# It4innovations/hyperqueue

Hardware: AMD Instinct MI355X
Metric: tasks_assigned_per_sec (higher is better)
Workload: dtype u64

## Files before the change

hyperqueue_amd/csrc/debug_capi.cpp:

```cpp
#include "../../include/hqtick_debug.h"

#include <algorithm>
#include <cstring>

#include "hb_order.h"
#include "milp.h"
#include "price_emul.h"

static thread_local int g_last_canonical = 0;
static thread_local long g_last_hull[2] = {0, 0};
extern "C" int hqtick_debug_milp_was_canonical(void) { return g_last_canonical; }
extern "C" void hqtick_debug_milp_last_hull(long *solves, long *nonpacking) {
    if (solves) *solves = g_last_hull[0];
    if (nonpacking) *nonpacking = g_last_hull[1];
}

extern "C" int hqtick_debug_milp_solve(int ncols, const double *obj, const uint8_t *col_kind, int nrows, const uint8_t *row_type,
                                       const double *rhs, const int *row_off, const int *row_col, const double *row_coef,
                                       double time_limit_s, int canonical, double *x_out, double *obj_out, int *is_optimal,
                                       long *nodes_out) {
    hqmilp::Model m;
    m.obj.assign(obj, obj + ncols);
    m.kind.assign(col_kind, col_kind + ncols);
    m.rtype.assign(row_type, row_type + nrows);
// ... 13 lines not shown
    return 1;
}

extern "C" void hqtick_debug_map_order_u32(const uint32_t *keys, uint32_t n, uint32_t *out_pos) {
    std::vector<uint32_t> order;
    hqhb::insertion_order_u32(keys, n, order);
    for (uint32_t i = 0; i < n; i++) out_pos[i] = order[i];
}

extern "C" int hqtick_debug_milp_solve_priced(int ncols, const double *obj, const uint8_t *col_kind, const int32_t *col_group, int nrows, const uint8_t *row_type,
                                              const uint8_t *row_implied, const double *rhs, const int *row_off, const int *row_col, const double *row_coef,
                                              double time_limit_s, int use_sweeps, uint32_t min_cols, double *x_out, double *obj_out, int *is_optimal, double *stats_out) {
    hqmilp::Model m;
    m.obj.assign(obj, obj + ncols);
    m.kind.assign(col_kind, col_kind + ncols);
    m.rtype.assign(row_type, row_type + nrows);
    m.rhs.assign(rhs, rhs + nrows);
    m.roff.assign(row_off, row_off + nrows + 1);
    int nnz = nrows ? row_off[nrows] : 0;
    m.rcol.assign(row_col, row_col + nnz);
    m.rcoef.assign(row_coef, row_coef + nnz);
    if (col_group) m.col_group.assign(col_group, col_group + ncols);
    if (row_implied) m.row_implied.assign(row_implied, row_implied + nrows);
    hqprice::EmulatedSweeper emu;
    if (min_cols) emu.min_cols = min_cols;
    hqmilp::Result r = hqmilp::solve(m, time_limit_s, true, hqmilp::REFERENCE_MIP_REL_GAP, use_sweeps ? &emu : nullptr);
    g_last_canonical = r.canonical ? 1 : 0;
    g_last_hull[0] = r.hull_solves; g_last_hull[1] = r.hull_solves_nonpacking;
    if (stats_out) { stats_out[0] = r.price_sweeps; stats_out[1] = r.price_rounds; stats_out[2] = r.price_total_us; stats_out[3] = r.canonical ? 1.0 : 0.0; }
    if (!r.feasible) return 0;
    for (int j = 0; j < ncols; j++) x_out[j] = r.x[j];
    *obj_out = r.objective;
    *is_optimal = r.optimal ? 1 : 0;
    return 1;
}

static thread_local hqmilp::Probe g_block_run_probe;
extern "C" void hqtick_debug_set_block_runs(int on) {
    hqmilp::g_probe = on < 0 ? nullptr : &g_block_run_probe; hqmilp::set_block_runs(on);
    if (on >= 0) { g_block_run_probe.model = g_block_run_probe.tables = g_block_run_probe.runs = g_block_run_probe.covered = 0; }
}
extern "C" void hqtick_debug_corrupt_block_runs(int on) { g_block_run_probe.corrupt_runs = on != 0; }
extern "C" void hqtick_debug_last_coupled_digest(uint64_t out[4]) {
    out[0] = g_block_run_probe.model; out[1] = g_block_run_probe.tables; out[2] = g_block_run_probe.runs; out[3] = g_block_run_probe.covered;
}
extern "C" void hqtick_debug_set_early_sweep(int on) { hqprice::set_early_sweep(on); }
extern "C" uint32_t hqtick_debug_early_sweeps(void) { return hqprice::early_sweeps(); }
extern "C" void hqtick_debug_capture_first_cut(int on) { hqprice::capture_first_cut(on != 0); }
extern "C" uint32_t hqtick_debug_first_cut(unsigned char *out, uint32_t cap) {
    const std::vector<unsigned char> &b = hqprice::first_cut_bytes();
    if (out && cap) memcpy(out, b.data(), std::min<size_t>(cap, b.size()));
    return (uint32_t)b.size();
}
```

hyperqueue_amd/csrc/host_model.cpp:

```cpp
#include "host_model.h"

#include <algorithm>
#include <chrono>
#include <cmath>
#include <cstring>
#include <string>
#include <unordered_map>

#include "hb_order.h"

namespace hqhost {

namespace {

struct OrderEntry { uint64_t hash = 0; bool used = false; std::vector<uint32_t> ids, order; };
thread_local OrderEntry order_cache[32];
thread_local unsigned order_next = 0;
const std::vector<uint32_t> &cached_worker_order(const std::vector<uint32_t> &ids) {
    typedef OrderEntry Entry;
    Entry (&cache)[32] = order_cache;
    unsigned &next = order_next;
    uint64_t h = 0x9E3779B97F4A7C15ull ^ ids.size();
    for (uint32_t v : ids) { h ^= v; h *= 0xFF51AFD7ED558CCDull; h ^= h >> 29; }
    for (Entry &e : cache) if (e.used && e.hash == h && e.ids.size() == ids.size() && (ids.empty() || memcmp(e.ids.data(), ids.data(), ids.size() * 4) == 0)) return e.order;
// ... 1181 lines not shown
                        if (runs_on) for (auto &wg : pm.with_gap) pm.max_excess = std::max(pm.max_excess, (int64_t)bcols_ub[wg.first] - (int64_t)wg.second);
                    }
                    no_gap = pm.whole ? &bcols : &pm.no_gap; no_gap_id = pm.lhs_id;
                    auto gap_rows = [&](const uint32_t w, const uint32_t gap) {
                        const int *wc = bcols.data() + bcols_off[w]; const size_t nwc = bcols_end[w] - bcols_off[w];
                        const uint64_t cols_ub = bcols_ub[w];
                        if (bounded && fl_cached == -2) fl_cached = short_flag(brq, bl.second);
                        const int fl = bounded ? fl_cached : -1;
                        if (cols_ub <= (uint64_t)cut.size + gap) return;
                        if (bounded && fl >= 0) { cols.assign(wc, wc + nwc); emit_plus(hqmilp::ROW_MAX, (double)cut.size + bsize + (double)gap, cols, fl, bsize); }
                        else if (!bounded) { m.begin_row(hqmilp::ROW_MAX, (double)cut.size + (double)gap); for (size_t k = 0; k < nwc; k++) m.term(wc[k], 1.0); m.end_row(); }
                    };
                    if (runs_on && (pm.all_gap || !pm.with_gap.empty()) && pm.max_excess <= (int64_t)cut.size) {
                        if (bounded) fl_cached = short_flag(brq, bl.second);
                        n_decided_once++;
                    } else if (pm.all_gap) for (uint32_t w : solver_workers) gap_rows(w, pm.gap_all);
                    else for (auto &wg : pm.with_gap) gap_rows(wg.first, wg.second);
                }
                if (no_gap->empty()) continue;
                int fl;
                if (bounded && (fl = short_flag(brq, bl.second)) >= 0) list_row(hqmilp::ROW_MAX, bsize + (double)cut.size, no_gap_id, *no_gap, fl, bsize);
                else if (!bounded && std::find(capped_by.begin(), capped_by.end(), brq) == capped_by.end()) {
                    capped_by.push_back(brq);
                    list_row(hqmilp::ROW_MAX, (double)cut.size, no_gap_id, *no_gap, -1, 0.0);
                }
            }
        }
    }

    if (!seq_start.empty()) {
        m.start.assign(m.ncols(), 0.0);
        for (const SeqStart &ss : seq_start) {
            const int pc = place_get(ss.w, batches[ss.batch].rq, ss.variant);
            if (pc < 0) { m.start.clear(); break; }
            m.start[pc] = ss.count;
        }
    }
    m.row_implied.resize(m.nrows(), 0);
    m.row_lhs.resize((size_t)m.nrows(), -1); m.row_lhs_len.resize((size_t)m.nrows(), 0); m.row_block.resize((size_t)m.nrows(), -1);
    m.col_ub = col_ub; m.col_ub.resize((size_t)m.ncols(), UINT32_MAX);
    if (hqmilp::g_probe) {
        using hqmilp::fnv1a_vec;
        uint64_t h = hqmilp::FNV_BASIS;
        h = fnv1a_vec(h, m.obj); h = fnv1a_vec(h, m.kind); h = fnv1a_vec(h, m.rtype); h = fnv1a_vec(h, m.rhs); h = fnv1a_vec(h, m.roff); h = fnv1a_vec(h, m.rcol); h = fnv1a_vec(h, m.rcoef);
        h = fnv1a_vec(h, m.start); h = fnv1a_vec(h, m.col_group); h = fnv1a_vec(h, m.row_implied); h = fnv1a_vec(h, m.row_lhs); h = fnv1a_vec(h, m.row_lhs_len);
        h = fnv1a_vec(h, m.list_off); h = fnv1a_vec(h, m.list_col); h = fnv1a_vec(h, m.row_block); h = fnv1a_vec(h, m.col_ub);
        hqmilp::g_probe->model = h; hqmilp::g_probe->runs = m.block_runs.size(); hqmilp::g_probe->tables = 0; hqmilp::g_probe->covered = 0;
    }
    const double t_model1 = clock_us();
    if (trace_model) {
        size_t run_blocks = 0; for (const auto &br : m.block_runs) run_blocks += (size_t)br.n_blocks;
        fprintf(stderr, "[model] cuts done at %.3f ms: %d columns, %d rows, %zu terms, %zu worker signatures, %zu (batch, cut, blocker) passes over the workers; %zu equal-block runs over %zu blocks, %zu (cut, blocker) passes decided once\n", (t_model1 - t_model0) / 1e3, m.ncols(), m.nrows(), m.rcol.size(), sig_rep.size(), n_triples, m.block_runs.size(), run_blocks, n_decided_once);
    }
    hqmilp::Result sol = hqmilp::solve(m, pb.time_limit_s, !pb.certificate_only, hqmilp::REFERENCE_MIP_REL_GAP, pb.pricer);
    if (trace_model) fprintf(stderr, "[model] solve done %.3f ms after the model\n", (clock_us() - t_model1) / 1e3);
    out.pre_us = t_model0 - t_enter; out.model_us = t_model1 - t_model0; out.milp_us = clock_us() - t_model1; out.price_sweeps = sol.price_sweeps; out.price_rounds = sol.price_rounds; out.price_us = sol.price_total_us;
    out.milp_nodes = sol.nodes; out.milp_cols = m.ncols(); out.milp_rows = m.nrows(); out.milp_components = sol.n_components;
    if (!sol.feasible) return out;
    out.is_optimal = sol.optimal;
    out.is_canonical = sol.canonical && sol.optimal;

    std::vector<uint64_t> key_hash; std::vector<std::pair<uint32_t, uint8_t>> key_list; std::vector<std::vector<std::pair<uint32_t, uint32_t>>> key_counts;
    std::vector<uint64_t> mn_hash; std::vector<uint32_t> mn_list; std::vector<std::vector<std::vector<uint32_t>>> mn_sets;
    std::vector<uint32_t> dec_ids, dec_widx, dec_cnt;
    for (const TaskBatch &batch : batches) {
        const RequestView &rv = pb.rqs[batch.rq];
        if (pb.rq_multi_node(batch.rq)) {
            size_t n_nodes = pb.variants[rv.first_variant].n_nodes;
            std::vector<std::vector<uint32_t>> sets;
            for (uint32_t w : solver_workers) {
                const int pc = place_get(w, batch.rq, 0);
                if (pc < 0 || (uint32_t)std::round(sol.x[pc]) == 0) continue;
                if (!sets.empty() && sets.back().size() < n_nodes) sets.back().push_back(w); else sets.push_back({w});
            }
            if (!sets.empty()) { mn_hash.push_back(hqhb::hash_rq_variant(batch.rq, 0)); mn_list.push_back(batch.rq); mn_sets.push_back(sets); }
        } else {
            for (uint8_t v = 0; v < rv.n_variants; v++) {
                const size_t nsw = solver_workers.size();
                dec_ids.resize(nsw + 1); dec_widx.resize(nsw + 1); dec_cnt.resize(nsw + 1);
                uint32_t *idp = dec_ids.data(), *wxp = dec_widx.data(), *cp = dec_cnt.data(); size_t nk = 0;
                const int *pcol = place_col.data() + rv.first_variant + v;
                const double *xs = sol.x.data();
                for (size_t i = 0; i < nsw; i++) {
                    const uint32_t w = solver_workers[i];
                    const int pc = pcol[(size_t)w * NVS];
                    const double xv = pc >= 0 ? xs[pc] : 0.0;
                    const uint32_t c = xv > 0.0 ? (uint32_t)(xv + 0.5) : 0u;
                    idp[nk] = ws.id[w]; wxp[nk] = w; cp[nk] = c; nk += c > 0 ? 1 : 0;
                }
                if (nk == 0) continue;
                dec_ids.resize(nk);
                const std::vector<uint32_t> &ids = dec_ids, &widx = dec_widx, &cnt = dec_cnt;
                const std::vector<uint32_t> &word = cached_worker_order(ids);
                std::vector<std::pair<uint32_t, uint32_t>> ordered; ordered.reserve(word.size());
                for (uint32_t k : word) ordered.push_back({widx[k], cnt[k]});
                key_hash.push_back(hqhb::hash_rq_variant(batch.rq, v)); key_list.push_back({batch.rq, v}); key_counts.push_back(std::move(ordered));
            }
        }
    }
    std::vector<uint32_t> ord;
    hqhb::insertion_order(key_hash.data(), (uint32_t)key_hash.size(), ord);
    for (uint32_t k : ord) { out.keys.push_back(key_list[k]); out.per_key.push_back(std::move(key_counts[k])); }
    hqhb::insertion_order(mn_hash.data(), (uint32_t)mn_hash.size(), ord);
    for (uint32_t k : ord) { out.mn_rq.push_back(mn_list[k]); out.mn_sets.push_back(std::move(mn_sets[k])); }
    if (trace_model) fprintf(stderr, "[model] decoded %.3f ms after the model, %.3f ms after the solver was entered\n", (clock_us() - t_model1) / 1e3, (clock_us() - t_enter) / 1e3);
    return out;
}

}
```

hyperqueue_amd/csrc/host_model.h:

```cpp
#pragma once
#include <cstdint>
#include <map>
#include <string>
#include <tuple>
#include <vector>

#include "../../include/hqtick.h"
#include "block_core.h"
#include "price.h"
#include "milp.h"

namespace hqhost {

struct VariantView {
    const uint32_t *res;
    const uint8_t *kind;
    const uint64_t *amount;
    uint32_t n_entries, n_nodes, weight;
    uint64_t min_time_ns;
    bool multi_node() const { return n_nodes > 0; }
};

struct RequestView {
    uint32_t first_variant, n_variants;
// ... 26 lines not shown
    const float *min_util = nullptr;
    const uint8_t *flags = nullptr;
    const uint32_t *group = nullptr;
    const uint8_t *vflags = nullptr;
    const uint32_t *vtmc = nullptr;
    uint32_t n_variant_slots = 0;
    std::vector<std::vector<std::pair<uint32_t, uint8_t>>> blocked;
    uint32_t n_blocked_lists = 0;
    const uint32_t *assigned_off = nullptr, *assigned_rq = nullptr; const uint8_t *assigned_variant = nullptr;
    const uint32_t *agg_off = nullptr, *agg_rq = nullptr, *agg_cnt = nullptr; const uint8_t *agg_variant = nullptr;
    uint32_t n_assigned(uint32_t w) const { return assigned_off ? assigned_off[w + 1] - assigned_off[w] : agg_off ? agg_off[w + 1] - agg_off[w] : 0; }
    bool is_sn(uint32_t w) const { return flags ? (flags[w] & HQ_WORKER_SN) != 0 : true; }
    bool stopping(uint32_t w) const { return flags ? (flags[w] & HQ_WORKER_STOPPING) != 0 : false; }
    bool is_free(uint32_t w) const { return is_sn(w) && n_assigned(w) == 0 && !stopping(w); }
    uint8_t vf(uint32_t w, uint32_t slot) const { return vflags[(size_t)w * n_variant_slots + slot]; }
    uint32_t tmc(uint32_t w, uint32_t slot) const { return vtmc[(size_t)w * n_variant_slots + slot]; }
};

struct BlockSolver {
    virtual ~BlockSolver() {}
    virtual bool solve(const hqblock::ColTable &cols, const hqblock::ClassTable &classes, const hqblock::Output &out) = 0;
    virtual bool begin(const hqblock::ColTable &cols, const hqblock::ClassTable &classes, const hqblock::Output &out) { begun_ok = solve(cols, classes, out); return begun_ok; }
    virtual bool finish() { return begun_ok; }
    virtual bool overlaps() const { return false; }
    bool begun_ok = false;
};

void flush_tick_caches();

struct BlockMemo {
    struct Entry { uint64_t hash = 0; std::vector<unsigned char> key; std::vector<double> x; long nodes = 0; int n_components = 0; };
    static constexpr size_t CAP = 64;
    std::vector<Entry> entries;
    size_t next = 0;
    std::vector<unsigned char> scratch;
    uint64_t scratch_hash = 0;
    const Entry *find(const hqmilp::Model &m);
    void put(const hqmilp::Result &r);
};

struct Problem {
    BlockMemo *memo = nullptr;
    BlockSolver *blocks = nullptr;
    hqprice::Sweeper *pricer = nullptr;
    uint32_t block_min_classes = 1;
    uint32_t block_verify = 2;
    uint32_t tick_seq = 0;
    uint32_t R = 0, n_groups = 0;
    std::vector<RequestView> rqs;
    std::vector<VariantView> variants;
    WorkerSet real;
    const WorkerSet *custom = nullptr;
    double time_limit_s = 5.0;
    bool certificate_only = false;
    bool rq_multi_node(uint32_t rq) const { return variants[rqs[rq].first_variant].multi_node(); }
    bool capable_rqv(const WorkerSet &ws, uint32_t w, uint32_t rq) const {
        for (uint32_t v = 0; v < rqs[rq].n_variants; v++) {
            uint32_t slot = rqs[rq].first_variant + v;
            uint8_t f = ws.vf(w, slot);
            if ((f & 4) && (variants[slot].multi_node() || (f & 2))) return true;
        }
        return false;
    }
};

void group_equal_rows(WorkerSet &ws, bool all_solver);

std::vector<TaskBatch> create_task_batches(const Problem &pb, const std::vector<QueueLevels> &queues);

struct Counts {
    std::vector<std::pair<uint32_t, uint8_t>> keys;
    std::vector<std::vector<std::pair<uint32_t, uint32_t>>> per_key;
    std::vector<uint32_t> mn_rq;
    std::vector<std::vector<std::vector<uint32_t>>> mn_sets;
    struct WorkerList { std::vector<uint32_t> widx; };
    bool by_class = false;
    bool one_class = false;
    uint32_t n_cols = 0;
    std::vector<uint32_t> wclass, class_x, key_col, key_list;
    std::vector<WorkerList> lists;
    bool pairs_built = true;
    void pairs() {
        if (pairs_built) return;
        per_key.assign(keys.size(), {});
        for (size_t k = 0; k < keys.size(); k++) {
            const std::vector<uint32_t> &wi = lists[key_list[k]].widx;
            auto &out = per_key[k]; out.resize(wi.size());
            for (size_t i = 0; i < wi.size(); i++) out[i] = {wi[i], class_x[(size_t)wclass[wi[i]] * n_cols + key_col[k]]};
        }
        pairs_built = true;
    }
    size_t key_size(size_t k) const { return pairs_built ? per_key[k].size() : lists[key_list[k]].widx.size(); }
    bool is_optimal = true;
    bool is_canonical = true;
    bool empty() const {
        if (!pairs_built) { for (size_t k = 0; k < keys.size(); k++) if (key_size(k)) return false; }
        for (auto &k : per_key) if (!k.empty()) return false;
        for (auto &k : mn_sets) if (!k.empty()) return false;
        return true;
    }
    uint32_t checksum() const {
        uint32_t h = 2166136261u;
        auto mix = [&](uint32_t v) { for (int i = 0; i < 4; i++) { h ^= (v >> (8 * i)) & 0xFFu; h *= 16777619u; } };
        mix(is_optimal ? 1u : 0u);
        for (size_t k = 0; k < keys.size(); k++) {
            mix(keys[k].first); mix(keys[k].second);
            if (pairs_built) for (auto &wc : per_key[k]) { mix(wc.first); mix(wc.second); }
            else for (uint32_t w : lists[key_list[k]].widx) { mix(w); mix(class_x[(size_t)wclass[w] * n_cols + key_col[k]]); }
        }
        for (size_t k = 0; k < mn_rq.size(); k++) { mix(mn_rq[k]); for (auto &set : mn_sets[k]) { mix(0xFFFFFFFFu); for (uint32_t w : set) mix(w); } }
        return h;
    }
    int error = 0; std::string errmsg;
    long milp_nodes = 0; int milp_cols = 0, milp_rows = 0, milp_components = 0;
    int price_sweeps = 0, price_rounds = 0; double price_us = 0, milp_us = 0, model_us = 0, pre_us = 0;
    uint32_t blocks_device = 0, blocks_host = 0, block_steps_max = 0, n_classes = 0;
    uint32_t blocks_verified = 0, blocks_mismatch = 0, blocks_rejected = 0;
    uint32_t blocks_memo = 0;
    double t_classify_us = 0, t_blocks_us = 0, t_decode_us = 0;
};

Counts run_scheduling_solver(const Problem &pb, const std::vector<TaskBatch> &batches);

}
```

hyperqueue_amd/csrc/hqtick.cpp:

```cpp
#include "../../include/hqtick.h"
#ifdef HQTICK_TEST_HOOKS
#include "../../include/hqtick_debug.h"
#endif

#include <dlfcn.h>
#include <hip/hip_runtime.h>
#include <rccl/rccl.h>

#include <algorithm>
#include <chrono>
#include <cstdio>
#include <cstdlib>
#include <cstring>
#include <functional>
#include <map>
#include <string>
#include <vector>

#include "block_solve.h"
#include "price_dev.h"
#ifdef HQTICK_TEST_HOOKS
#include "price_emul.h"
#endif
#include "devbuf.h"
// ... 43 lines not shown
    uint64_t max_id = 0; bool max_id_valid = false;
    uint32_t n_appends = 0;
    bool consumed_unconfirmed = false;
    hqhost::BlockMemo block_memo;
    uint64_t add_staged_n = 0;
    DevBuf d_set, d_flags, d_levels, d_nlevels, d_wave_tab, d_hist, d_gkey;
    DevBuf d_ord_hist, d_ord_tab, d_perm, d_perm2, d_ord_tiles, d_inv; PinBuf h_ord, h_ordh;
    bool force_ordered = false;
    bool ordered_sticky = false;
    bool last_ordered = false;
    hqk::OrderSelect last_os{};
    uint32_t dbg_order_runs = 0, dbg_order_levels = 0; bool dbg_order = false; double dbg_order_us = 0;
    uint32_t dbg_scan_L = 0, dbg_scan_G = 0, dbg_scan_shape[4] = {0, 0, 0, 0}; bool dbg_scan = false, dbg_census = false;
    uint32_t lv_seq = 0; bool set_clean = false; bool no_spec_scan = getenv("HQTICK_NO_SPEC_SCAN") != nullptr; bool levels_valid = false; uint32_t cached_L = 0; std::vector<uint64_t> h_levels; bool timing = true, timing_k1 = false;
    PinBuf h_up, h_up2, h_q, h_a, h_plan, h_rec, h_sinkhdr, h_add, h_addp, h_retr, h_blk, h_k5a, h_lv;
    PinBuf h_blkprof; uint32_t n_blkprof = 0; bool block_profile = false;
    hqprice::DeviceSweeper *pricer = nullptr;
    uint32_t block_budget = 4096, block_min_classes = 12;
    DevBuf d_up, d_vflags, d_vtmc, d_blk;
    DevBuf d_cluster; PinBuf h_cl, h_cld; bool cluster_valid = false, cluster_check = false, cl_pending = false; uint32_t cl_W = 0, cl_R = 0;
    std::vector<unsigned char> cl_rt;
    hipEvent_t cl_ev = nullptr;
    struct ClusterMirror {
        bool valid = false; uint32_t n_groups = 1;
        std::vector<uint32_t> id, group; std::vector<uint64_t> total, free_; std::vector<int64_t> rem; std::vector<float> min_util; std::vector<uint8_t> flags;
        std::map<uint32_t, std::vector<std::pair<uint32_t, uint8_t>>> blocked;
        std::vector<uint32_t> blk_worker, blk_rq; std::vector<uint8_t> blk_variant; bool blk_dirty = true;
    } mirror;
    DevBuf d_cluster2;
    struct RetrEntry { uint32_t old_id; bool in_queue; bool has_redirect; uint32_t target_id; uint8_t variant; };
    std::map<uint64_t, RetrEntry> retr;
    std::vector<uint64_t> retr_task, resp_task; std::vector<uint32_t> retr_worker, retr_red_worker, resp_worker; std::vector<uint8_t> retr_red_variant, resp_variant;
    bool sweep_inflight = false;
    bool wait_on_kernel = true;
    DevBuf d_sel_task, d_sel_level, d_map, d_rec, d_tsweep, d_bits, d_pre;
    hqhost::Problem pb;
    PlanScratch plan;
    std::vector<uint32_t> b_rq, b_size, b_limit, b_cut_off, c_size, c_bl_off, bl_rq, bl_size; std::vector<uint8_t> b_lr, b_blk;
    std::vector<uint32_t> cnt_rq, cnt_worker, cnt_value; std::vector<uint8_t> cnt_variant;
    std::vector<uint32_t> rec_off, retract_off, red_worker, mn_off, mn_worker, mn_rq; std::vector<uint64_t> rec_task, retract_task, red_task, mn_task, new_free;
    std::vector<uint8_t> rec_variant, rec_kind, red_variant, red_kind, q_loaded;
    hqtick_kernel_stats stats{};
    uint32_t tpw_hint = 0;
    uint32_t shard_index = 0, shard_count = 1;
    void *sink = nullptr; size_t sink_bytes = 0;
    hqk::WaveGeom last_geom{}; uint32_t last_L = 0, last_Q = 0, last_G = 0; size_t last_tb = 0, last_plan_bytes = 0, last_hist_off = 0; bool last_valid = false;
    hqgraph::Graph graph;
    hqasg::Ledger asg;
    hqtick_ctx *qctx = nullptr;
    ncclComm_t comm = nullptr; uint32_t comm_rank = 0, comm_world = 0;
    hqtick_exchange_fn xfn = nullptr; void *xuser = nullptr;
    DevBuf d_xsend, d_xrecv; PinBuf h_xsend, h_xrecv;
    uint32_t shard_min_blocks = 1025, shard_min_classes = 1025; bool shard_solve = true;
    uint32_t block_verify = 2, tick_seq = 0;
    uint64_t x_calls = 0, x_bytes = 0; double x_us = 0;
    double tl[32] = {}; int ntl = 0;
};

namespace {

#define HQ_HIP(call)                                                                                          \
    do {                                                                                                      \
        hipError_t e_ = (call);                                                                               \
        if (e_ != hipSuccess) { ctx->err = std::string(#call) + ": " + hipGetErrorString(e_); return HQTICK_E_DEVICE; } \
    } while (0)

#define HQ_HIP_TIMED(call)                                                                                    \
    do {                                                                                                      \
        hipError_t e_ = (call);                                                                               \
        hqk::take_launch_timer();                                                                             \
        if (e_ != hipSuccess) { ctx->err = std::string(#call) + ": " + hipGetErrorString(e_); return HQTICK_E_DEVICE; } \
    } while (0)

#define HQ_HIP_LAST(call, launched)                                                                           \
    do {                                                                                                      \
        hipError_t e_ = (call);                                                                               \
        (launched) = hqk::take_launch_timer().stop == nullptr && ctx->wait_on_kernel;                        \
        if (e_ != hipSuccess) { ctx->err = std::string(#call) + ": " + hipGetErrorString(e_); return HQTICK_E_DEVICE; } \
    } while (0)

int fail(hqtick_ctx *ctx, int code, const std::string &msg) { ctx->err = msg; return code; }

double elapsed_us(hipEvent_t a, hipEvent_t b) {
    float ms = 0;
    if (hipEventElapsedTime(&ms, a, b) == hipSuccess) return (double)ms * 1000.0;
    (void)hipGetLastError();
    return -1.0;
}

int validate(hqtick_ctx *ctx, const hqtick_snapshot *s, bool need_tasks) {
    if (!s) return fail(ctx, HQTICK_E_INVALID, "null snapshot");
    if (s->n_workers && (!s->worker_id || !s->worker_total || !s->worker_free)) return fail(ctx, HQTICK_E_INVALID, "worker arrays missing");
    for (uint32_t w = 1; w < s->n_workers; w++) if (s->worker_id[w - 1] >= s->worker_id[w]) return fail(ctx, HQTICK_E_INVALID, "worker ids not ascending");
    if (s->n_requests && (!s->rq_variant_off || !s->variant_entry_off)) return fail(ctx, HQTICK_E_INVALID, "request arrays missing");
    for (uint32_t q = 0; q < s->n_requests; q++) {
        if (s->rq_variant_off[q + 1] <= s->rq_variant_off[q]) return fail(ctx, HQTICK_E_INVALID, "request without variants");
        if (s->rq_variant_off[q + 1] - s->rq_variant_off[q] > 32) return fail(ctx, HQTICK_E_INVALID, "more than 32 variants");
    }
    uint32_t nv = s->n_requests ? s->rq_variant_off[s->n_requests] : 0;
    for (uint32_t e = 0; e < (nv ? s->variant_entry_off[nv] : 0); e++) {
        if (s->entry_resource[e] >= s->n_resources) return fail(ctx, HQTICK_E_INVALID, "entry resource id out of range");
        if (s->entry_kind[e] == HQ_ENTRY_AMOUNT && s->entry_amount[e] == 0) return fail(ctx, HQTICK_E_INVALID, "zero amount request");
    }
    if (need_tasks && s->n_ready) {
        if (!s->task_id || !s->task_priority || !s->task_rq) return fail(ctx, HQTICK_E_INVALID, "ready-set columns missing");
        for (uint64_t i = 1; i < s->n_ready; i++) if (s->task_id[i - 1] >= s->task_id[i]) return fail(ctx, HQTICK_E_INVALID, "ready set not sorted by task id");
// ... 493 lines not shown
    bool allgather(const void *send, void *recv, size_t bytes) override {
        if (ctx->xfn) return ctx->xfn(ctx->xuser, send, recv, bytes) == 0;
        return rccl_allgather_host(ctx, send, recv, bytes);
    }
    ~CtxExchange() override { ctx->x_calls += n_calls; ctx->x_bytes += n_bytes; ctx->x_us += us; }
};

struct ShardedBlocks : hqhost::BlockSolver {
    hqhost::BlockSolver &inner; hqprice::Exchange &ex; uint32_t min_classes;
    hqblock::Output p_out{}; uint32_t p_nd = 0, p_nc = 0, p_nm = 0; bool p_pass = false, p_inner_ok = false, p_pending = false;
    std::vector<uint64_t> cfree, ctot, celig; std::vector<uint32_t> dx, dst, dsteps; std::vector<unsigned char> send, recv;
    ShardedBlocks(hqhost::BlockSolver &in, hqprice::Exchange &e, uint32_t mc) : inner(in), ex(e), min_classes(mc) {}
    bool overlaps() const override { return inner.overlaps(); }
    bool solve(const hqblock::ColTable &ct, const hqblock::ClassTable &cl, const hqblock::Output &out) override { return begin(ct, cl, out) && finish(); }
    bool begin(const hqblock::ColTable &ct, const hqblock::ClassTable &cl, const hqblock::Output &out) override {
        p_pass = ex.world <= 1 || cl.n_classes < min_classes;
        if (p_pass) return inner.begin(ct, cl, out);
        const uint32_t nd = cl.n_classes, R = ct.R, NC = ct.n_cols, W = ex.world, me = ex.rank;
        const uint32_t nm = nd > me ? (nd - me + W - 1) / W : 0;
        cfree.resize((size_t)nm * R); ctot.resize((size_t)nm * R); celig.resize(nm);
        for (uint32_t j = 0; j < nm; j++) {
            const size_t i = (size_t)me + (size_t)j * W;
            memcpy(cfree.data() + (size_t)j * R, cl.free_ + i * R, (size_t)R * 8); memcpy(ctot.data() + (size_t)j * R, cl.total + i * R, (size_t)R * 8); celig[j] = cl.elig[i];
        }
        dx.assign((size_t)nm * NC, 0); dst.assign(nm, hqblock::ST_UNSUPPORTED); dsteps.assign(nm, 0);
        p_out = out; p_nd = nd; p_nc = NC; p_nm = nm; p_pending = true;
        p_inner_ok = nm == 0 || inner.begin(ct, hqblock::ClassTable{nm, cfree.data(), ctot.data(), celig.data()}, hqblock::Output{dx.data(), dst.data(), dsteps.data(), nullptr});
        return true;
    }
    bool finish() override {
        if (p_pass) return inner.finish();
        if (!p_pending) return false;
        p_pending = false;
        if (p_nm && !(p_inner_ok && inner.finish())) { std::fill(dst.begin(), dst.end(), (uint32_t)hqblock::ST_UNSUPPORTED); std::fill(dx.begin(), dx.end(), 0u); }
        const uint32_t W = ex.world, NC = p_nc, mx = (p_nd + W - 1) / W;
        const size_t o_st = (size_t)mx * NC * 4, o_steps = o_st + (size_t)mx * 4, bytes = (o_steps + (size_t)mx * 4 + 7) & ~(size_t)7;
        send.assign(bytes, 0); recv.resize(bytes * W);
        if (p_nm) { memcpy(send.data(), dx.data(), (size_t)p_nm * NC * 4); memcpy(send.data() + o_st, dst.data(), (size_t)p_nm * 4); memcpy(send.data() + o_steps, dsteps.data(), (size_t)p_nm * 4); }
        const double t0 = now_us();
        if (!ex.allgather(send.data(), recv.data(), bytes)) return false;
        ex.us += now_us() - t0; ex.n_calls++; ex.n_bytes += bytes * W;
        for (uint32_t r = 0; r < W; r++) {
            const unsigned char *b = recv.data() + (size_t)r * bytes;
            const uint32_t nr = p_nd > r ? (p_nd - r + W - 1) / W : 0;
            for (uint32_t j = 0; j < nr; j++) {
                const size_t i = (size_t)r + (size_t)j * W;
                memcpy(p_out.x + i * NC, b + (size_t)j * NC * 4, (size_t)NC * 4); memcpy(p_out.status + i, b + o_st + (size_t)j * 4, 4); memcpy(p_out.steps + i, b + o_steps + (size_t)j * 4, 4);
            }
        }
        return true;
    }
};

struct TickRun {
    hqtick_ctx *ctx; const hqtick_snapshot *s; hqtick_result *out; const bool use_resident;
    PlanScratch &ps; hqhost::Problem &pb;
    const uint32_t W, R, Q;
    static constexpr uint32_t NONE = 0xFFFFFFFFu;
    WorkerEval ev; Scan sc; hqhost::Counts cnt;
    uint64_t N = 0; uint32_t L = 0; int status = HQTICK_DONE;
    uint32_t nkeys = 0, max_count = 0, max_nk = 0, n_bit_words = 0, n_sel = 0, n_pfq = 0, n_rec = 0, max_items = 0;
    std::vector<uint32_t> pfq_rq;
    std::vector<std::pair<uint32_t, uint32_t>> retr_pos;
    std::vector<std::vector<uint32_t>> key_T;
    size_t o_rv = 0, o_rk = 0, o_mn = 0, o_fl = 0;
    bool sweep_launched = false;
    uint32_t n_tr = 0;
    const bool transpose_on = !(getenv("HQTICK_TRANSPOSE") && atoi(getenv("HQTICK_TRANSPOSE")) == 0);
    bool may_reorder = false;
    bool compact = false, delta16 = false; size_t o_rs = 0, o_rf = 0; uint32_t max_out = 0;
    uint64_t *h_rec_task = nullptr, *mn_ids = nullptr; uint8_t *h_rec_var = nullptr, *h_rec_kind = nullptr;
    bool assembled = false;
    double t0 = 0;

    TickRun(hqtick_ctx *c, const hqtick_snapshot *snap, hqtick_result *o, bool resident)
        : ctx(c), s(snap), out(o), use_resident(resident), ps(c->plan), pb(c->pb), W(snap->n_workers), R(snap->n_resources), Q(snap->n_requests) {}

    void mark() { if (ctx->ntl < 32) ctx->tl[ctx->ntl++] = now_us() - t0; }
    uint32_t n_groups() const { return sc.ordered ? (uint32_t)sc.run_cnt.size() : sc.G; }

    uint32_t worker_of(uint32_t k, uint32_t idx) {
        cnt.pairs();
        const auto &pk = cnt.per_key[k];
        std::vector<uint32_t> &T = key_T[k];
        if (T.empty()) {
            uint32_t maxc = 0; for (auto &wc : pk) maxc = std::max(maxc, wc.second);
            std::vector<uint32_t> ge(maxc + 2, 0);
            for (auto &wc : pk) ge[wc.second]++;
            uint32_t more = (uint32_t)pk.size(), acc = 0;
            for (uint32_t sw = 0; sw <= maxc; sw++) { T.push_back(acc); more -= ge[sw]; acc += more; }
        }
        uint32_t sw = (uint32_t)(std::upper_bound(T.begin(), T.end(), idx) - T.begin()) - 1, nth = idx - T[sw];
        for (auto &wc : pk) if (wc.second > sw) { if (nth == 0) return wc.first; nth--; }
        return HQ_NO_WORKER;
    }

    int load_ready_set() {
        if (!use_resident) {
            uint64_t N = s->n_ready;
            if (!ctx->d_tid.ensure(N * 8 + 8) || !ctx->d_tprio.ensure(N * 8 + 8) || !ctx->d_trq.ensure(N * 4 + 8)) return fail(ctx, HQTICK_E_DEVICE, "hipMalloc ready set");
            if (N) {
                HQ_HIP(hipMemcpyAsync(ctx->d_tid.p, s->task_id, N * 8, hipMemcpyHostToDevice, ctx->stream));
                HQ_HIP(hipMemcpyAsync(ctx->d_tprio.p, s->task_priority, N * 8, hipMemcpyHostToDevice, ctx->stream));
                HQ_HIP(hipMemcpyAsync(ctx->d_trq.p, s->task_rq, N * 4, hipMemcpyHostToDevice, ctx->stream));
            }
            ctx->n_ready = N; ctx->resident = false; ctx->levels_valid = false;
        } else if (!ctx->resident) return fail(ctx, HQTICK_E_INVALID, "hqtick_run_resident without hqtick_upload_ready");
        N = ctx->n_ready;
        return 0;
    }

    int plan_keys() {
        L = sc.L;
        ps.q_total.assign(Q, 0); ps.pf_n.assign(Q, 0); ps.pf_start.assign(Q, 0); ps.seq_taken.assign(Q, 0);
        for (uint32_t q = 0; q < Q; q++) {
            const uint32_t r0 = sc.run_off[q], r1 = sc.run_off[q + 1];
            for (uint32_t r = r0; r < r1; r++) ps.q_total[q] += sc.run_cnt[r];
            ps.pf_n[q] = s->prefill_off ? s->prefill_off[q + 1] - s->prefill_off[q] : 0;
            if (ps.pf_n[q]) ps.pf_start[q] = (r0 < r1 && sc.run_prio[r0] == s->prefill_priority[q]) ? sc.run_cnt[r0] : 0;
        }
        nkeys = (uint32_t)cnt.keys.size();
        ps.key_seg.assign(nkeys, 0); ps.key_sum.assign(nkeys, 0); ps.key_rq.assign(nkeys, 0); ps.key_var_w.assign((nkeys + 3) / 4 + 1, 0);
        ps.key_ord_off.assign(nkeys + 1, 0); ps.key_t_off.assign(nkeys + 1, 0); ps.key_bits_off.assign(nkeys + 1, 0);
        const bool by_class = cnt.by_class && cnt.wclass.size() == W && cnt.key_col.size() == nkeys;
        ctx->last_valid = false;
// ... 257 lines not shown
        ctx->rec_off = ps.out_off;
        ctx->retract_off.assign(W + 1, 0); ctx->retract_task.assign(ps.retract_pairs.size(), 0);
        {
            for (auto &rp : ps.retract_pairs) if (rp.first < W) ctx->retract_off[rp.first + 1]++;
            for (uint32_t w = 0; w < W; w++) ctx->retract_off[w + 1] += ctx->retract_off[w];
            std::vector<uint32_t> cur(ctx->retract_off.begin(), ctx->retract_off.end() - 1);
            for (auto &rp : ps.retract_pairs) if (rp.first < W) ctx->retract_task[cur[rp.first]++] = rp.second;
        }
        ctx->new_free.assign(s->worker_free, s->worker_free + (size_t)W * R);
        for (uint32_t k = 0; k < nkeys; k++) {
            const hqhost::VariantView &vv = pb.variants[pb.rqs[cnt.keys[k].first].first_variant + cnt.keys[k].second];
            const uint32_t *wcn = ps.wcnt + (size_t)k * W;
            for (uint32_t w = 0; w < W; w++) {
                const uint32_t c = wcn[w];
                if (!c) continue;
                for (uint32_t e = 0; e < vv.n_entries; e++) {
                    uint64_t &f = ctx->new_free[(size_t)w * R + vv.res[e]];
                    if (vv.kind[e] == HQ_ENTRY_ALL) f = 0; else { uint64_t d = vv.amount[e] * (uint64_t)c; f = f > d ? f - d : 0; }
                }
            }
        }
        for (auto &fr : ps.freed) {
            const hqhost::VariantView &vv = pb.variants[fr.second];
            for (uint32_t e = 0; e < vv.n_entries; e++) {
                uint64_t &f = ctx->new_free[(size_t)fr.first * R + vv.res[e]];
                f = vv.kind[e] == HQ_ENTRY_ALL ? s->worker_total[(size_t)fr.first * R + vv.res[e]] : f + vv.amount[e];
            }
        }
    }

    int launch_sweep_early() {
        sweep_launched = false;
        if (nkeys == 0 || n_bit_words == 0 || max_nk > hqk::SWEEP_MAX_WORKERS) return 0;
        if (n_tr == nkeys) { sweep_launched = true; return 0; }
        if (ctx->sweep_inflight) { HQ_HIP(hipStreamSynchronize(ctx->stream)); ctx->sweep_inflight = false; }
        const size_t n_ord = ps.ord_cnt.size(), words = 4 * (size_t)(nkeys + 1) + n_ord;
        if (!ctx->h_k5a.ensure(words * 4 + 64) || !ctx->d_tsweep.ensure((size_t)ps.key_t_off[nkeys] * 4 + 16) || !ctx->d_bits.ensure((size_t)n_bit_words * 8 + 16) ||
            !ctx->d_pre.ensure((size_t)n_bit_words * 4 + 16))
            return fail(ctx, HQTICK_E_DEVICE, "hipMalloc mapping");
        uint32_t *h = ctx->h_k5a.as<uint32_t>();
        const uint32_t *d = ctx->h_k5a.dev<uint32_t>();
        const size_t o_toff = 0, o_ordoff = nkeys + 1, o_boff = 2 * (size_t)(nkeys + 1), o_tr = 3 * (size_t)(nkeys + 1), o_ord = 4 * (size_t)(nkeys + 1);
        memcpy(h + o_toff, ps.key_t_off.data(), (size_t)(nkeys + 1) * 4); memcpy(h + o_ordoff, ps.key_ord_off.data(), (size_t)(nkeys + 1) * 4);
        memcpy(h + o_boff, ps.key_bits_off.data(), (size_t)(nkeys + 1) * 4); memcpy(h + o_tr, ps.key_tr.data(), (size_t)nkeys * 4); if (n_ord) memcpy(h + o_ord, ps.ord_cnt.data(), n_ord * 4);
        hqk::MapKeys mk{};
        mk.n_keys = nkeys; mk.key_t_off = d + o_toff; mk.key_ord_off = d + o_ordoff; mk.key_bits_off = d + o_boff; mk.ord_cnt = d + o_ord; mk.key_tr = d + o_tr;
        mk.t_sweep = ctx->d_tsweep.as<uint32_t>(); mk.bits = ctx->d_bits.as<uint64_t>(); mk.pre = ctx->d_pre.as<uint32_t>();
        if (ctx->timing) hqk::time_next_launch(ctx->ev[1], ctx->ev[6]);
        HQ_HIP_TIMED(hqk::sweep_bits(mk, max_count, max_nk, ctx->stream));
        sweep_launched = true; ctx->sweep_inflight = true;
        return 0;
    }

    int phase_c() {
        size_t n_mn_ids = 0; for (auto &sets : cnt.mn_sets) n_mn_ids += sets.size();
        delta16 = compact && (ctx->cfg.flags & HQTICK_FLAG_COMPACT_DELTA16) != 0;
        if (compact) {
            o_rs = delta16 ? (size_t)n_rec * 8 : (((size_t)n_rec * 4 + 7) & ~(size_t)7); o_rf = o_rs + (size_t)W * 8;
            o_rv = o_rk = 0; o_mn = (o_rf + (size_t)n_rec * (delta16 ? 16 : 12) + 7) & ~(size_t)7;
        } else { o_rv = (size_t)n_rec * 8; o_rk = o_rv + n_rec; o_mn = (o_rk + n_rec + 7) & ~(size_t)7; }
        o_fl = o_mn + n_mn_ids * 8;
        const size_t rec_bytes = o_fl + 64;
        if (!ctx->h_rec.ensure(rec_bytes)) return fail(ctx, HQTICK_E_DEVICE, "hipHostMalloc records");
        h_rec_task = ctx->h_rec.as<uint64_t>(); h_rec_var = ctx->h_rec.as<uint8_t>() + o_rv; h_rec_kind = ctx->h_rec.as<uint8_t>() + o_rk;
        mn_ids = reinterpret_cast<uint64_t *>(ctx->h_rec.as<uint8_t>() + o_mn);
        if (n_sel) {
            if (!ctx->d_sel_task.ensure((size_t)n_sel * 8) || !ctx->d_sel_level.ensure((size_t)n_sel * (sc.ordered ? 4 : 2) + 4))
                return fail(ctx, HQTICK_E_DEVICE, "hipMalloc selection");
            uint32_t *hp = ctx->h_plan.as<uint32_t>();
            size_t cur = ps.plan_head_words;
            auto put = [&](const std::vector<uint32_t> &v) { const size_t o = cur; if (!v.empty()) memcpy(hp + cur, v.data(), v.size() * 4); cur += v.size(); if (v.empty()) hp[cur++] = 0; return o; };
            const size_t o_wpos = 0, o_wcnt = (size_t)nkeys * W, o_pflj = (size_t)2 * nkeys * W;
            size_t o_rq = put(ps.key_rq), o_var = put(ps.key_var_w), o_seg = put(ps.key_seg), o_ordoff = put(ps.key_ord_off), o_ord = put(ps.ord_cnt), o_toff = put(ps.key_t_off),
                   o_boff = put(ps.key_bits_off), o_tr = put(ps.key_tr), o_base = put(ps.rq_sel_base), o_pfs = put(ps.pf_start), o_pfn = put(ps.pf_n),
                   o_pqs = put(ps.pfq_src), o_pqz = put(ps.pfq_size), o_out = put(ps.out_off);
            const size_t o_pqr = ctx->asg.on ? put(pfq_rq) : 0;
            size_t o_tb = put(ps.take_base);
            size_t o_roff = 0, o_qtnc = 0, o_rst = 0, o_rrk = 0;
            if (sc.ordered) { o_roff = put(sc.run_off); o_qtnc = put(ps.q_tnc); o_rst = put(sc.run_start); o_rrk = put(sc.run_level); }
            if (cur & 1) hp[cur++] = 0;
            const size_t o_holes = cur;
            for (uint64_t hk : ps.holes) { hp[cur++] = (uint32_t)(hk & 0xFFFFFFFFu); hp[cur++] = (uint32_t)(hk >> 32); }
            if (ps.holes.empty()) { hp[cur++] = 0; hp[cur++] = 0; }
            const size_t plan_words = cur;
            if (plan_words * 4 + 16 > ctx->h_plan.cap) return fail(ctx, HQTICK_E_DEVICE, "mapping plan larger than its buffer");
            if (!ctx->d_map.ensure(plan_words * 4 + 16) ||
                !ctx->d_tsweep.ensure((size_t)ps.key_t_off[nkeys] * 4 + 16) || !ctx->d_bits.ensure((size_t)n_bit_words * 8 + 16) || !ctx->d_pre.ensure((size_t)n_bit_words * 4 + 16))
                return fail(ctx, HQTICK_E_DEVICE, "hipMalloc mapping");
            mark();
            const uint32_t *d = ctx->d_map.as<uint32_t>();
            hqk::MapKeys mk{};
            mk.n_keys = nkeys; mk.key_rq = d + o_rq; mk.key_variant = reinterpret_cast<const uint8_t *>(d + o_var); mk.key_seg_start = d + o_seg;
            mk.key_ord_off = d + o_ordoff; mk.ord_cnt = d + o_ord; mk.key_t_off = d + o_toff; mk.key_bits_off = d + o_boff; mk.key_tr = d + o_tr;
            mk.t_sweep = ctx->d_tsweep.as<uint32_t>(); mk.bits = ctx->d_bits.as<uint64_t>(); mk.pre = ctx->d_pre.as<uint32_t>();
            mk.wpos = d + o_wpos; mk.wcnt = d + o_wcnt; mk.rq_sel_base = d + o_base; mk.rq_pf_start = d + o_pfs; mk.rq_pf_n = d + o_pfn;
            mk.n_holes = (uint32_t)ps.holes.size(); mk.holes = reinterpret_cast<const uint64_t *>(d + o_holes);
            mk.n_pfq = n_pfq; mk.pfq_src = d + o_pqs; mk.pfq_size = d + o_pqz; mk.pfl_j = d + o_pflj; mk.out_off = d + o_out;
            uint32_t *flags = reinterpret_cast<uint32_t *>(ctx->h_rec.as<uint8_t>() + o_fl);
            flags[0] = 0;
            ctx->last_n_sel = n_sel; ctx->last_consumed = false;
            const bool consume_in_tick = use_resident && (ctx->cfg.flags & HQTICK_FLAG_CONSUME_IN_TICK) != 0;
            if (consume_in_tick && ctx->asg.on && s->n_retracting) {
                uint32_t *saved = ctx->asg.saved_rq(N);
                if (!saved) return fail(ctx, HQTICK_E_DEVICE, "hipMalloc ledger request ids");
                HQ_HIP(hipMemcpyAsync(saved, ctx->d_trq.p, N * 4, hipMemcpyDeviceToDevice, ctx->stream));
            }
            ctx->last_geom = sc.geom; ctx->last_L = L; ctx->last_Q = Q; ctx->last_G = sc.G; ctx->last_tb = o_tb; ctx->last_plan_bytes = plan_words * 4; ctx->last_valid = true;
// ... 15 lines not shown
                                consume_in_tick ? ctx->d_trq.as<uint32_t>() : nullptr, ctx->stream, consume_in_tick ? 1u : 0u));
            }
            if (consume_in_tick) { ctx->n_live -= n_sel; ctx->last_consumed = true; ctx->consumed_unconfirmed = true; }
            if (!sweep_launched && n_tr < nkeys) {
                if (ctx->timing) hqk::time_next_launch(ctx->ev[1], ctx->ev[6]);
                HQ_HIP_TIMED(hqk::sweep_bits(mk, max_count, max_nk, ctx->stream));
            }
            uint8_t *drec = ctx->h_rec.dev<uint8_t>();
            uint64_t *k_task = reinterpret_cast<uint64_t *>(drec); uint8_t *k_var = drec + o_rv, *k_kind = drec + o_rk;
            if (ctx->sink) {
                const uint32_t cap = hqtick_sink_capacity_records(W, ctx->sink_bytes);
                if (n_rec > cap || hqtick_sink_bytes(W, cap) > ctx->sink_bytes) return fail(ctx, HQTICK_E_CAPACITY, "record sink too small for this tick");
                uint8_t *sk = reinterpret_cast<uint8_t *>(ctx->sink);
                const size_t so_off = 16, so_task = (so_off + (size_t)(W + 1) * 4 + 7) & ~(size_t)7, so_var = so_task + (size_t)cap * 8, so_kind = so_var + cap;
                std::vector<uint32_t> &hdr = ps.sink_hdr; hdr.assign(4 + W + 1, 0);
                hdr[0] = n_rec; hdr[1] = cnt.checksum(); hdr[2] = HQTICK_SINK_MAGIC; hdr[3] = cap;
                memcpy(hdr.data() + 4, ps.out_off.data(), (size_t)(W + 1) * 4);
                if (!ctx->h_sinkhdr.ensure(hdr.size() * 4)) return fail(ctx, HQTICK_E_DEVICE, "hipHostMalloc sink header");
                memcpy(ctx->h_sinkhdr.p, hdr.data(), hdr.size() * 4);
                HQ_HIP(hipMemcpyAsync(sk, ctx->h_sinkhdr.p, hdr.size() * 4, hipMemcpyHostToDevice, ctx->stream));
                k_task = reinterpret_cast<uint64_t *>(sk + so_task); k_var = sk + so_var; k_kind = sk + so_kind;
            }
            hqk::time_next_launch(ctx->timing ? ctx->ev[7] : nullptr, ctx->ev[11]);
            hqk::CompactOut co{};
            if (compact) co = hqk::CompactOut{reinterpret_cast<uint32_t *>(drec), reinterpret_cast<uint2 *>(drec + o_rs), reinterpret_cast<uint32_t *>(drec + o_rf),
                                              delta16 ? reinterpret_cast<uint16_t *>(drec) : nullptr};
            hqk::Stage stg{};
            if (ctx->asg.on && n_rec) {
                hqasg::StageCols c{};
                if (!ctx->asg.stage_for(n_rec, sc.ordered, sc.L, &c)) return fail(ctx, HQTICK_E_DEVICE, "hipMalloc ledger staging");
                stg = hqk::Stage{c.task, c.rq, c.row, c.level, c.meta};
                stg.pfq_rq = ctx->d_map.as<uint32_t>() + o_pqr;
            }
            bool expand_is_last = false;
            if (sc.ordered) HQ_HIP_LAST(hqk::expand_mapping_wide(mk, W, ctx->d_sel_task.as<uint64_t>(), ctx->d_sel_level.as<uint32_t>(), max_items, k_task, k_var, k_kind,
                                                           reinterpret_cast<uint32_t *>(drec + o_fl), co, max_out, may_reorder, ctx->stream, stg), expand_is_last);
            else HQ_HIP_LAST(hqk::expand_mapping(mk, W, ctx->d_sel_task.as<uint64_t>(), ctx->d_sel_level.as<uint16_t>(), Q, max_items, k_task, k_var, k_kind,
                                reinterpret_cast<uint32_t *>(drec + o_fl), co, max_out, may_reorder, ctx->stream, stg), expand_is_last);
            if (!cnt.mn_rq.empty()) expand_is_last = false;
            if (sc.ordered) {
                HQ_HIP(hipMemcpyAsync(ctx->h_ordh.as<uint32_t>() + hqk::ORDER_DIGITS * 256 + 2, ctx->d_ord_hist.as<uint32_t>() + hqk::ORDER_DIGITS * 256 + 2, 4, hipMemcpyDeviceToHost, ctx->stream));
                expand_is_last = false;
            }
            {
                size_t pos = 0;
                for (size_t i = 0; i < cnt.mn_rq.size(); i++) {
                    size_t n = cnt.mn_sets[i].size();
                    HQ_HIP(hipMemcpyAsync(mn_ids + pos, ctx->d_sel_task.as<uint64_t>() + ps.rq_sel_base[cnt.mn_rq[i]] + ps.mn_first[i], n * 8, hipMemcpyDeviceToHost, ctx->stream));
                    pos += n;
                }
            }
            mark();
            assemble_host_part();
            if (expand_is_last) HQ_HIP(hipEventSynchronize(ctx->ev[11])); else HQ_HIP(hipStreamSynchronize(ctx->stream));
            ctx->sweep_inflight = false;
            if (flags[0]) return fail(ctx, HQTICK_E_CAPACITY, "mapping kernel capacity exceeded");
            if (sc.ordered && ctx->h_ordh.as<uint32_t>()[hqk::ORDER_DIGITS * 256 + 2]) return fail(ctx, HQTICK_E_DEVICE, "ordered view: the selection left its request's segment");
            if (ctx->timing) { const double us_ = elapsed_us(ctx->ev[4], ctx->ev[5]); if (us_ >= 0) ctx->stats.select_us = us_; }
            if (ctx->timing) { const double us_ = elapsed_us(ctx->ev[1], ctx->ev[6]); if (us_ >= 0) ctx->stats.sweep_us = us_; }
            if (ctx->timing) { const double us_ = elapsed_us(ctx->ev[7], ctx->ev[11]); if (us_ >= 0) ctx->stats.other_us = us_; }
        }
        if (!n_sel) { ctx->last_n_sel = 0; ctx->last_consumed = true; }
        if (!n_sel && ctx->sink) {
            if (hqtick_sink_bytes(W, 0) > ctx->sink_bytes) return fail(ctx, HQTICK_E_CAPACITY, "record sink too small for this tick");
            std::vector<uint32_t> &hdr = ps.sink_hdr; hdr.assign(4 + W + 1, 0);
            hdr[1] = cnt.checksum(); hdr[2] = HQTICK_SINK_MAGIC; hdr[3] = hqtick_sink_capacity_records(W, ctx->sink_bytes);
            HQ_HIP(hipMemcpy(ctx->sink, hdr.data(), hdr.size() * 4, hipMemcpyHostToDevice));
        }
        return 0;
    }

    void finish(double t1, double t2, double t3) {
        if (!assembled) assemble_host_part();
        ctx->mn_task.clear(); ctx->mn_off.assign(1, 0); ctx->mn_worker.clear(); ctx->mn_rq.clear();
        {
            size_t pos = 0;
            for (size_t i = 0; i < cnt.mn_rq.size(); i++) for (auto &set : cnt.mn_sets[i]) {
                ctx->mn_task.push_back(mn_ids[pos++]); ctx->mn_rq.push_back(cnt.mn_rq[i]);
                for (uint32_t w : set) ctx->mn_worker.push_back(w);
                ctx->mn_off.push_back((uint32_t)ctx->mn_worker.size());
            }
        }
        out->status = status;
        out->n_counts = (uint32_t)ctx->cnt_rq.size(); out->count_rq = ctx->cnt_rq.data(); out->count_variant = ctx->cnt_variant.data();
        out->count_worker = ctx->cnt_worker.data(); out->count_value = ctx->cnt_value.data();
        out->rec_off = ctx->rec_off.data();
        if (compact && n_sel) {
            const uint8_t *hb = ctx->h_rec.as<uint8_t>();
            out->run_span = reinterpret_cast<const hqtick_run_span *>(hb + o_rs);
            if (delta16) { out->rec_delta16 = reinterpret_cast<const uint16_t *>(hb); out->runs16 = reinterpret_cast<const hqtick_rec_run16 *>(hb + o_rf); }
            else { out->rec_task_lo = reinterpret_cast<const uint32_t *>(hb); out->runs = reinterpret_cast<const hqtick_rec_run *>(hb + o_rf); }
        } else if (!ctx->sink) { out->rec_task = h_rec_task; out->rec_variant = h_rec_var; out->rec_kind = h_rec_kind; }
        out->retract_off = ctx->retract_off.data(); out->retract_task = ctx->retract_task.data();
        out->n_redirects = (uint32_t)ctx->red_task.size(); out->redirect_task = ctx->red_task.data(); out->redirect_worker = ctx->red_worker.data(); out->redirect_variant = ctx->red_variant.data(); out->redirect_kind = ctx->red_kind.data();
        out->n_mn = (uint32_t)ctx->mn_task.size(); out->mn_task = ctx->mn_task.data(); out->mn_worker_off = ctx->mn_off.data(); out->mn_worker = ctx->mn_worker.data();
        out->new_free = ctx->new_free.data();
        mark();
        double t5 = now_us();
        out->t_total_us = t5 - t0; out->t_scan_us = t1 - t0; out->t_batches_us = t2 - t1; out->t_solve_us = t3 - t2; out->t_mapping_us = t5 - t3;
        uint64_t n_pref = 0; for (uint32_t q = 0; q < Q; q++) n_pref += ps.new_pf_total[q];
        uint64_t n_asg = 0; for (uint32_t w = 0; w < W; w++) n_asg += ps.n_assign[w];
        uint32_t nv = Q ? s->rq_variant_off[Q] : 0;
        ctx->stats.n_assigned = n_asg; ctx->stats.n_prefilled = n_pref;
        ctx->stats.algorithmic_bytes = N * 20 + (uint64_t)W * R * 16 + (uint64_t)nv * R * 9 + n_asg * 13 + n_pref * 12;
        ctx->stats.tick_gpu_us = ctx->stats.distinct_us + ctx->stats.level_hist_us + ctx->stats.scan_us + ctx->stats.block_solve_us + ctx->stats.select_us + ctx->stats.sweep_us + ctx->stats.other_us;
    }

    int run() {
        t0 = now_us();
        ctx->ntl = 0;
        if (ctx->cfg.flags & HQTICK_FLAG_NO_TICK_CACHES) { ctx->levels_valid = false; hqhost::flush_tick_caches(); }
        memset(out, 0, sizeof(*out));
        ctx->stats = hqtick_kernel_stats{};
        int rc = validate(ctx, s, !use_resident);
        if (rc) return rc;
        HQ_HIP(hipSetDevice(ctx->device));
        if ((rc = load_ready_set())) return rc;
        const std::function<void()> prep = [&]() {
            fill_problem(pb, s, ctx->cfg, ev);
            if (ctx->asg.on && !s->assigned_off) {
                const hqasg::Agg g = ctx->asg.agg();
                pb.real.agg_off = g.off; pb.real.agg_rq = g.rq; pb.real.agg_cnt = g.cnt; pb.real.agg_variant = g.var;
            }
            if (pb.certificate_only && (ctx->shard_count > 1 || ctx->sink || ctx->xfn || ctx->comm)) pb.certificate_only = false;
        };
        if ((rc = phase_a(ctx, s, &ev, &sc, &prep))) return rc;
        mark();
        const double t1 = now_us();
        std::vector<hqhost::QueueLevels> qlv = queue_levels(sc, s);
        std::vector<hqhost::TaskBatch> batches = hqhost::create_task_batches(pb, qlv);
        export_batches(ctx, batches, out);
        mark();
        const double t2 = now_us();
        DeviceBlocks dev_blocks(ctx);
        pb.blocks = &dev_blocks; pb.block_min_classes = ctx->block_min_classes; pb.pricer = ctx->pricer;
        pb.block_verify = ctx->block_verify; pb.tick_seq = ctx->tick_seq++;
        pb.memo = (ctx->cfg.flags & (HQTICK_FLAG_NO_BLOCK_MEMO | HQTICK_FLAG_NO_TICK_CACHES)) ? nullptr : &ctx->block_memo;
        double shard_sweep_us = -1.0;
        ctx->x_calls = 0; ctx->x_bytes = 0; ctx->x_us = 0;
        if (CtxExchange::available(ctx)) {
            CtxExchange xch(ctx);
            ShardedBlocks sh_blocks(dev_blocks, xch, ctx->shard_min_classes);
            pb.blocks = &sh_blocks;
            if (ctx->pricer) {
                hqprice::ShardedSweeper sh_sweeps(*ctx->pricer, xch, ctx->shard_min_blocks);
                pb.pricer = &sh_sweeps;
                cnt = hqhost::run_scheduling_solver(pb, batches);
                shard_sweep_us = sh_sweeps.stat_sweep_us;
            } else cnt = hqhost::run_scheduling_solver(pb, batches);
        } else cnt = hqhost::run_scheduling_solver(pb, batches);
        pb.blocks = nullptr; pb.pricer = nullptr;
        ctx->stats.price_sweeps = (uint32_t)cnt.price_sweeps; ctx->stats.price_rounds = (uint32_t)cnt.price_rounds; ctx->stats.price_us = cnt.price_us; ctx->stats.milp_us = cnt.milp_us; ctx->stats.model_us = cnt.model_us; ctx->stats.solve_pre_us = cnt.pre_us;
        ctx->stats.price_sweep_us = shard_sweep_us >= 0.0 ? shard_sweep_us : (ctx->pricer ? ctx->pricer->stat_sweep_us : 0.0); ctx->stats.milp_cols = (uint32_t)cnt.milp_cols; ctx->stats.milp_rows = (uint32_t)cnt.milp_rows;
        ctx->stats.n_classes_verified = cnt.blocks_verified; ctx->stats.n_classes_mismatch = cnt.blocks_mismatch; ctx->stats.n_classes_rejected = cnt.blocks_rejected; ctx->stats.n_classes_memo = cnt.blocks_memo;
        ctx->stats.exchange_calls = (uint32_t)ctx->x_calls; ctx->stats.exchange_bytes = ctx->x_bytes; ctx->stats.exchange_us = ctx->x_us;
        if (cnt.error) return fail(ctx, cnt.error, cnt.errmsg);
        ctx->stats.n_classes_device = cnt.blocks_device; ctx->stats.n_classes_host = cnt.blocks_host; ctx->stats.block_steps_max = cnt.block_steps_max; ctx->stats.n_classes = cnt.n_classes;
        ctx->stats.solve_classify_us = cnt.t_classify_us; ctx->stats.solve_blocks_us = cnt.t_blocks_us; ctx->stats.solve_decode_us = cnt.t_decode_us;
        mark();
        const double t3 = now_us();
        out->is_optimal = cnt.is_optimal;
        out->is_canonical = cnt.is_canonical && cnt.is_optimal;
        status = HQTICK_DONE;
        if (!cnt.is_optimal) status = cnt.empty() ? HQTICK_NO_PROGRESS : HQTICK_NEED_MORE_COMPUTE;
        if ((rc = plan_keys())) return rc;
        if ((rc = launch_sweep_early())) return rc;
        if ((rc = plan_redirects())) return rc;
        mark();
        if ((rc = plan_prefill())) return rc;
        mark();
        if ((rc = plan_outputs())) return rc;
        mark();
        if ((rc = phase_c())) return rc;
        mark();
        finish(t1, t2, t3);
        return status;
    }
};

bool ledger_replica(const hqtick_ctx *ctx) { return ctx->shard_count > 1 || ctx->xfn || ctx->comm; }
hqasg::Env ledger_env(hqtick_ctx *ctx) {
    return hqasg::Env{ctx->device, ctx->stream, ctx->d_cluster.as<unsigned char>(), ctx->cl_W, ctx->cl_R, ctx->d_tid.as<uint64_t>(), ctx->d_tprio.as<uint64_t>(), ctx->d_trq.as<uint32_t>(), ctx->n_ready,
                      ctx->d_levels.as<uint64_t>(), &ctx->mirror.id, &ctx->mirror.flags, &ctx->mirror.free_};
}
int ledger_fail(hqtick_ctx *ctx, int rc) { if (rc < 0) ctx->err = ctx->asg.err; return rc; }
bool ledger_pending_live(hqtick_ctx *ctx) { return ctx->asg.pending_live(ctx->last_valid && !ctx->last_consumed); }
int ledger_guard(hqtick_ctx *ctx) {
    if (ctx->asg.on && ledger_pending_live(ctx)) return fail(ctx, HQTICK_E_INVALID, "assignment ledger: the last tick's placement is pending (hqtick_ready_consume_last first)");
    return 0;
}

int run_tick(hqtick_ctx *ctx, const hqtick_snapshot *s, hqtick_result *out, bool use_resident) {
    hqtick_snapshot full;
    bool copied = false;
    if (ctx->asg.on && s) {
        if (ledger_replica(ctx)) return fail(ctx, HQTICK_E_UNSUPPORTED, "assignment ledger on a sharded or replica context");
        if (s->worker_id || !(ctx->cluster_valid && ctx->mirror.valid)) return fail(ctx, HQTICK_E_INVALID, "assignment ledger on: the tick runs on the resident worker set (HQ_WORKERS_RESIDENT, no worker arrays)");
        if (s->assigned_off) return fail(ctx, HQTICK_E_INVALID, "assignment ledger on: the snapshot must not carry an assigned CSR as well");
        if (ctx->asg.tracking() && s->prefilled_off) return fail(ctx, HQTICK_E_INVALID, "prefilled tracking on: the snapshot must not carry a prefilled CSR as well");
        HQ_HIP(hipSetDevice(ctx->device));
        ctx->asg.abandon_tick();
        ctx->asg.take_requests(s);
        if (ctx->asg.tracking() && ctx->asg.max_variants() >= hqasg::PF_VARIANT) return fail(ctx, HQTICK_E_UNSUPPORTED, "prefilled tracking: a request has 254 or more variants");
        if (int rc = ctx->asg.sync_mirror(ledger_env(ctx))) return ledger_fail(ctx, rc);
    }
    if (s && s->n_workers == HQ_WORKERS_RESIDENT && !(s->worker_id == nullptr && ctx->cluster_valid && ctx->mirror.valid))
        return fail(ctx, HQTICK_E_INVALID, s->worker_id ? "n_workers == HQ_WORKERS_RESIDENT with worker arrays in the snapshot"
                                                         : "n_workers == HQ_WORKERS_RESIDENT without a resident worker set (hqtick_cluster_upload; dropped by hqtick_cluster_drop)");
    if (s && s->worker_id == nullptr && ctx->cluster_valid && ctx->mirror.valid) {
        hqtick_ctx::ClusterMirror &m = ctx->mirror;
        const uint32_t W = (uint32_t)m.id.size();
        if (s->n_workers != 0 && s->n_workers != HQ_WORKERS_RESIDENT && s->n_workers != W) return fail(ctx, HQTICK_E_INVALID, "snapshot without worker arrays: n_workers must be HQ_WORKERS_RESIDENT, 0 or the resident worker count");
        if (s->n_resources != ctx->cl_R) return fail(ctx, HQTICK_E_INVALID, "snapshot without worker arrays: n_resources differs from the resident tables");
        if (m.blk_dirty) {
            m.blk_worker.clear(); m.blk_rq.clear(); m.blk_variant.clear();
            for (uint32_t w = 0; w < W; w++) { auto it = m.blocked.find(m.id[w]); if (it == m.blocked.end()) continue; for (auto &p : it->second) { m.blk_worker.push_back(w); m.blk_rq.push_back(p.first); m.blk_variant.push_back(p.second); } }
            m.blk_dirty = false;
        }
        full = *s; copied = true;
        full.n_workers = W; full.worker_id = m.id.data(); full.worker_total = m.total.data(); full.worker_free = m.free_.data(); full.worker_remaining_ns = m.rem.data();
        full.worker_min_utilization = m.min_util.data(); full.worker_flags = m.flags.data(); full.worker_group = m.group.data(); full.n_groups = m.n_groups; full.worker_map_rank = nullptr;
        full.n_blocked = (uint32_t)m.blk_worker.size(); full.blocked_worker = m.blk_worker.data(); full.blocked_rq = m.blk_rq.data(); full.blocked_variant = m.blk_variant.data();
        s = &full;
    }
    const bool retr_resident = s && s->n_retracting == HQ_RETRACTING_RESIDENT;
    if (retr_resident) {
        if (!s->worker_id) return fail(ctx, HQTICK_E_INVALID, "resident retracting table without worker ids (hqtick_cluster_upload, or worker arrays in the snapshot)");
        const uint32_t W = s->n_workers;
        auto index_of = [&](uint32_t id) -> uint32_t { const uint32_t *b = s->worker_id, *e = b + W, *it = std::lower_bound(b, e, id); return (it != e && *it == id) ? (uint32_t)(it - b) : HQ_NO_WORKER; };
        ctx->retr_task.clear(); ctx->retr_worker.clear(); ctx->retr_red_worker.clear(); ctx->retr_red_variant.clear();
        for (auto &kv : ctx->retr) {
            if (!kv.second.in_queue) continue;
            const uint32_t oi = index_of(kv.second.old_id);
            if (oi == HQ_NO_WORKER) return fail(ctx, HQTICK_E_INVALID, "a Retracting task's worker is not in the worker set");
            ctx->retr_task.push_back(kv.first); ctx->retr_worker.push_back(oi);
            ctx->retr_red_worker.push_back(kv.second.has_redirect ? index_of(kv.second.target_id) : HQ_NO_WORKER); ctx->retr_red_variant.push_back(kv.second.variant);
        }
        if (!copied) { full = *s; copied = true; s = &full; }
        full.n_retracting = (uint32_t)ctx->retr_task.size();
        full.retracting_task = ctx->retr_task.data(); full.retracting_worker = ctx->retr_worker.data();
        full.retracting_redirect_worker = ctx->retr_red_worker.data(); full.retracting_redirect_variant = ctx->retr_red_variant.data();
    }
    int rc;
    {
        TickRun run(ctx, s, out, use_resident);
        rc = run.run();
    }
    if (ctx->consumed_unconfirmed) {
        ctx->consumed_unconfirmed = false;
        if (rc < 0) {
            const std::string why = ctx->err;
            bool restored = false;
            const bool synced = hipStreamSynchronize(ctx->stream) == hipSuccess;
            if (synced && ctx->last_valid && ctx->last_ordered) {
                hqk::OrderSelect os = ctx->last_os;
                os.mark_rq = ctx->d_trq.as<uint32_t>(); os.mark_value = 0; os.mark_and_select = 0;
                if (hqk::order_select(os, ctx->last_n_sel, ctx->stream) == hipSuccess && hipStreamSynchronize(ctx->stream) == hipSuccess) { ctx->n_live += ctx->last_n_sel; restored = true; }
            } else if (synced && ctx->last_valid && !ctx->last_ordered && ctx->last_Q && ctx->h_q.ensure(64)) {
                uint32_t *cntp = ctx->h_q.as<uint32_t>();
                cntp[0] = 0;
                if (hqk::ready_restore_consumed(ctx->d_gkey.as<uint16_t>(), ctx->d_trq.as<uint32_t>(), ctx->n_ready, ctx->last_Q, ctx->h_q.dev<uint32_t>(), ctx->stream) == hipSuccess &&
                    hipStreamSynchronize(ctx->stream) == hipSuccess && cntp[0] <= ctx->last_n_sel) {
                    ctx->n_live += ctx->last_n_sel;
                    restored = true;
                }
            }
            ctx->last_valid = false; ctx->last_consumed = true; ctx->last_n_sel = 0;
            ctx->err = why;
            if (restored) ctx->err += " (HQTICK_FLAG_CONSUME_IN_TICK: what the tick had taken is back in the resident ready set)";
            else { ctx->resident = false; ctx->err += " (HQTICK_FLAG_CONSUME_IN_TICK: the tick had already taken its tasks and they could not be put back; the resident ready set is dropped, upload it again)"; }
        }
    }
    if (rc >= 0 && retr_resident) {
        const uint32_t W = s->n_workers;
        for (uint32_t w = 0; w < W && w + 1 < ctx->retract_off.size(); w++)
            for (uint32_t i = ctx->retract_off[w]; i < ctx->retract_off[w + 1]; i++) ctx->retr[ctx->retract_task[i]] = hqtick_ctx::RetrEntry{s->worker_id[w], false, false, 0, 0};
        for (size_t i = 0; i < ctx->red_task.size(); i++) {
            auto it = ctx->retr.find(ctx->red_task[i]);
            if (it == ctx->retr.end()) continue;
            hqtick_ctx::RetrEntry &e = it->second;
            const uint8_t kind = i < ctx->red_kind.size() ? ctx->red_kind[i] : (uint8_t)HQ_REDIRECT_FROM_PREFILL;
            e.in_queue = false;
            if (kind == HQ_REDIRECT_SAME_WORKER) continue;
            if (ctx->red_worker[i] < W) { e.has_redirect = true; e.target_id = s->worker_id[ctx->red_worker[i]]; e.variant = ctx->red_variant[i]; }
        }
    }
    if (rc >= 0 && ctx->asg.on) {
        const bool in_tick = use_resident && (ctx->cfg.flags & HQTICK_FLAG_CONSUME_IN_TICK) != 0;
        ctx->asg.collect_tick(s, out, ctx->new_free, ctx->mn_rq, in_tick && s->n_retracting != 0);
        if (!use_resident || in_tick) {
            if (int r2 = ledger_fail(ctx, ctx->asg.apply_tick(ledger_env(ctx)))) {
                ctx->asg.on = false; ctx->asg.pending = false;
                ctx->err += " (the assignment ledger is switched off: upload the worker set and enable it again)";
                return r2;
            }
        }
    }
    return rc;
}

}

extern "C" {

uint32_t hqtick_abi_version(void) { return HQTICK_ABI_VERSION; }
const char *hqtick_build_arch(void) { return "gfx950"; }

int hqtick_create(const hqtick_config *config, hqtick_ctx **out_ctx) {
    if (!config || !out_ctx || (config->abi_version != HQTICK_ABI_VERSION && config->abi_version != 10u && config->abi_version != 11u)) return HQTICK_E_INVALID;
    int n = 0;
    if (hipGetDeviceCount(&n) != hipSuccess || n <= 0 || config->device_index < 0 || config->device_index >= n) return HQTICK_E_NO_DEVICE;
    hipDeviceProp_t prop;
    if (hipGetDeviceProperties(&prop, config->device_index) != hipSuccess) return HQTICK_E_NO_DEVICE;
    if (std::string(prop.gcnArchName).rfind("gfx950", 0) != 0) return HQTICK_E_NO_DEVICE;
    if (hipSetDevice(config->device_index) != hipSuccess) return HQTICK_E_NO_DEVICE;
    hqtick_ctx *ctx = new hqtick_ctx();
    ctx->cfg = *config; ctx->device = config->device_index;
    ctx->timing = (config->flags & HQTICK_FLAG_NO_KERNEL_TIMING) == 0;
    if (const char *e = getenv("HQTICK_TPW")) { long v = atol(e); if (v >= 256 && v <= (1 << 20) && v % 256 == 0) ctx->tpw_hint = (uint32_t)v; }
    if (const char *e = getenv("HQTICK_BLOCK_PROFILE")) ctx->block_profile = atoi(e) != 0;
// ... 936 lines not shown
    for (auto &k : cnt.per_key) for (auto &wc : k) if (wc.second > 0) q->q_loaded[wc.first] = 1;
    out->n_workers = fake->n_workers; out->is_loaded = q->q_loaded.data(); out->is_optimal = cnt.is_optimal;
    return 0;
}

#ifdef HQTICK_TEST_HOOKS
namespace {
struct EmulatedBlocks : hqhost::BlockSolver {
    uint32_t budget;
    explicit EmulatedBlocks(uint32_t b) : budget(b) {}
    bool solve(const hqblock::ColTable &ct, const hqblock::ClassTable &cl, const hqblock::Output &out) override {
        static thread_local hqblock::Shared *S = new hqblock::Shared();
        hqblock::HostWave wv;
        const uint32_t NC = ct.n_cols, R = ct.R, ne = ct.ent_off[NC];
        auto al8 = [](size_t v) { return (v + 7) & ~(size_t)7; };
        const size_t o_res = al8((size_t)(NC + 1) * 4), o_w = al8(o_res + (size_t)ne * 4), o_kind = al8(o_w + (size_t)NC * 4), o_amt = al8(o_kind + ne), o_pool = o_amt + (size_t)ne * 8,
                     bytes = (o_pool + (size_t)R * 8 + 15) & ~(size_t)15;
        std::vector<hqblock::V16> store(bytes / 16 + 1);
        unsigned char *b = reinterpret_cast<unsigned char *>(store.data());
        memcpy(b, ct.ent_off, (size_t)(NC + 1) * 4); memcpy(b + o_res, ct.ent_res, (size_t)ne * 4); memcpy(b + o_w, ct.weight, (size_t)NC * 4);
        memcpy(b + o_kind, ct.ent_kind, ne); memcpy(b + o_amt, ct.ent_amount, (size_t)ne * 8); memcpy(b + o_pool, ct.pool, (size_t)R * 8);
        hqblock::ColTable bt{NC, R, (const uint32_t *)b, (const uint32_t *)(b + o_res), b + o_kind, (const uint64_t *)(b + o_amt), (const uint32_t *)(b + o_w), (const double *)(b + o_pool), b, (uint32_t)bytes};
        for (uint32_t c = 0; c < cl.n_classes; c++) hqblock::solve_block(wv, *S, (c & 1) ? ct : bt, cl, c, out, budget);
        if (corrupt_mode && corrupt_class < cl.n_classes && out.status[corrupt_class] == hqblock::ST_OK) {
            uint32_t *x = out.x + (size_t)corrupt_class * NC;
            if (corrupt_mode == 1) { for (uint32_t g = 0; g < NC; g++) if (x[g]) { x[g]--; break; } }
            else if (corrupt_mode == 2) { for (uint32_t g = NC; g-- > 0;) if (x[g]) { x[g] += 1000; break; } }
            else if (corrupt_mode == 3) {
                const uint32_t col = corrupt_fill >> 16, n = corrupt_fill & 0xFFFFu;
                if (col < NC) { for (uint32_t g = 0; g < NC; g++) x[g] = 0; x[col] = n; }
            }
        }
        return true;
    }
    int corrupt_mode = 0; uint32_t corrupt_class = 0, corrupt_fill = 0;
};
thread_local int g_block_emulation = 0, g_price_emulation = 0; thread_local uint32_t g_price_min_cols = 0, g_last_price_sweeps = 0, g_last_price_rounds = 0;
thread_local uint32_t g_block_budget = 4096, g_last_blocks_device = 0, g_last_blocks_host = 0;
thread_local uint32_t g_block_verify = 2, g_tick_seq = 0, g_last_guard[3] = {0, 0, 0}; thread_local int g_corrupt_mode = 0; thread_local uint32_t g_corrupt_class = 0, g_corrupt_fill = 0;
thread_local double g_last_stage_us[3] = {0, 0, 0};
}

void hqtick_debug_set_block_guard(uint32_t verify, uint32_t tick_seq, int corrupt_mode, uint32_t corrupt_class, uint32_t corrupt_fill) {
    g_block_verify = verify; g_tick_seq = tick_seq; g_corrupt_mode = corrupt_mode; g_corrupt_class = corrupt_class; g_corrupt_fill = corrupt_fill;
}
void hqtick_debug_last_block_guard(uint32_t *verified, uint32_t *mismatch, uint32_t *rejected) {
    if (verified) *verified = g_last_guard[0]; if (mismatch) *mismatch = g_last_guard[1]; if (rejected) *rejected = g_last_guard[2];
}
thread_local hqhost::BlockMemo *g_memo = nullptr; thread_local uint32_t g_last_memo = 0;
void hqtick_debug_set_block_memo(int on) { if (on && !g_memo) g_memo = new hqhost::BlockMemo(); if (!on) { delete g_memo; g_memo = nullptr; } }
uint32_t hqtick_debug_last_block_memo(void) { return g_last_memo; }
void hqtick_debug_set_price_emulation(int on, uint32_t min_cols) { g_price_emulation = on; g_price_min_cols = min_cols; }
void hqtick_debug_set_fast_path(int on) { hqmilp::set_fast_path(on); }
void hqtick_debug_check_model_hints(int on) { hqprice::set_check_hints(on != 0); }
int hqtick_debug_model_hint_mismatches(void) { return hqprice::hint_mismatches(); }
thread_local int g_price_fault = -1;
void hqtick_debug_set_price_fault(int fail_at) { g_price_fault = fail_at; }
thread_local hqtick_exchange_fn g_xfn = nullptr; thread_local void *g_xuser = nullptr; thread_local uint32_t g_xrank = 0, g_xworld = 1, g_xmin_blocks = 1, g_xmin_classes = 1, g_xcalls = 0;
void hqtick_debug_set_exchange(hqtick_exchange_fn fn, void *user, uint32_t rank, uint32_t world, uint32_t min_blocks, uint32_t min_classes) {
    g_xfn = fn; g_xuser = user; g_xrank = rank; g_xworld = world ? world : 1; g_xmin_blocks = min_blocks; g_xmin_classes = min_classes;
}
uint32_t hqtick_debug_last_exchange_calls(void) { return g_xcalls; }
void hqtick_debug_last_stage_us(double *out3) { if (out3) for (int i = 0; i < 3; i++) out3[i] = g_last_stage_us[i]; }
void hqtick_debug_last_price(uint32_t *sweeps, uint32_t *rounds) { if (sweeps) *sweeps = g_last_price_sweeps; if (rounds) *rounds = g_last_price_rounds; }
static thread_local std::vector<uint32_t> g_last_mn_rq, g_last_mn_off{0}, g_last_mn_worker;
uint32_t hqtick_debug_last_mn(const uint32_t **rq, const uint32_t **off, const uint32_t **worker) {
    if (rq) *rq = g_last_mn_rq.data();
    if (off) *off = g_last_mn_off.data();
    if (worker) *worker = g_last_mn_worker.data();
    return (uint32_t)g_last_mn_rq.size();
}
int hqtick_debug_last_order(const hqtick_ctx *ctx, uint32_t *n_runs, uint32_t *n_levels, double *order_us) {
    if (!ctx) return HQTICK_E_INVALID;
    if (n_runs) *n_runs = ctx->dbg_order ? ctx->dbg_order_runs : 0;
    if (n_levels) *n_levels = ctx->dbg_order ? ctx->dbg_order_levels : 0;
    if (order_us) *order_us = ctx->dbg_order ? ctx->dbg_order_us : 0.0;
    return ctx->dbg_order ? 1 : 0;
}
int hqtick_debug_last_scan(const hqtick_ctx *ctx, int which, uint32_t *n_levels, uint32_t *n_groups, uint32_t shape[4], uint64_t *levels, uint32_t cap_levels, uint32_t *hist,
                           uint32_t cap_groups) {
    if (!ctx || (which != 0 && which != 1)) return HQTICK_E_INVALID;
    const hqtick_ctx *c = which == 0 ? ctx : ctx->qctx;
    if (!c || !(which == 0 ? c->dbg_scan : c->dbg_census)) return 0;
    const uint32_t L = c->dbg_scan_L, G = c->dbg_scan_G;
    const uint64_t *lv = which == 0 ? c->h_levels.data() : c->h_lv.as<uint64_t>() + 2;
    const uint32_t *hs = reinterpret_cast<const uint32_t *>(c->h_a.as<unsigned char>() + 16);
    if (n_levels) *n_levels = L;
    if (n_groups) *n_groups = G;
    if (shape) for (int i = 0; i < 4; i++) shape[i] = which == 0 ? c->dbg_scan_shape[i] : 0u;
    if (levels) for (uint32_t i = 0; i < L && i < cap_levels; i++) levels[i] = lv[i];
    if (hist) for (uint32_t i = 0; i < G && i < cap_groups; i++) hist[i] = hs[i];
    return 1;
}
void hqtick_debug_set_block_emulation(int on, uint32_t budget) { g_block_emulation = on; if (budget) g_block_budget = budget; }
void hqtick_debug_last_blocks(uint32_t *n_emulated, uint32_t *n_host) { if (n_emulated) *n_emulated = g_last_blocks_device; if (n_host) *n_host = g_last_blocks_host; }

int hqtick_debug_block_solve_host(uint32_t n_cols, uint32_t n_resources, const uint32_t *ent_off, const uint32_t *ent_res, const uint8_t *ent_kind, const uint64_t *ent_amount,
                                  const uint32_t *weight, const double *pool, uint32_t n_classes, const uint64_t *free_, const uint64_t *total, const uint64_t *elig,
                                  uint32_t budget, uint32_t *x, uint32_t *status, uint32_t *steps) {
    hqblock::ColTable ct{n_cols, n_resources, ent_off, ent_res, ent_kind, ent_amount, weight, pool, nullptr, 0};
    hqblock::ClassTable cl{n_classes, free_, total, elig};
    hqblock::Output out{x, status, steps, nullptr};
    EmulatedBlocks emu(budget ? budget : 4096);
    return emu.solve(ct, cl, out) ? 0 : HQTICK_E_DEVICE;
}

int hqtick_debug_host_stages(const hqtick_config *config, const hqtick_snapshot *s, const uint8_t *vflags, const uint32_t *vtmc, uint32_t n_levels,
                             const uint64_t *levels, const uint32_t *hist, hqtick_result *out) {
    if (!config || !s || !out) return HQTICK_E_INVALID;
    static thread_local hqtick_ctx *holder = nullptr;
    if (!holder) holder = new hqtick_ctx();
    hqtick_ctx *ctx = holder;
    ctx->cfg = *config;
    if (int rc = validate(ctx, s, false)) return rc;
    WorkerEval ev; ev.flags = vflags; ev.tmc = vtmc;
    hqhost::Problem pb;
    fill_problem(pb, s, ctx->cfg, ev);
    Scan sc; sc.Q = s->n_requests; sc.L = n_levels; sc.G = n_levels * s->n_requests;
    sc.levels.assign(levels, levels + n_levels); sc.hist.assign(hist, hist + (size_t)n_levels * s->n_requests);
    runs_from_hist(sc);
    std::vector<hqhost::QueueLevels> qlv = queue_levels(sc, s);
    std::vector<hqhost::TaskBatch> batches = hqhost::create_task_batches(pb, qlv);
    memset(out, 0, sizeof(*out));
    g_last_mn_rq.clear(); g_last_mn_off.assign(1, 0); g_last_mn_worker.clear();
    export_batches(ctx, batches, out);
    EmulatedBlocks emu(g_block_budget);
    emu.corrupt_mode = g_corrupt_mode; emu.corrupt_class = g_corrupt_class; emu.corrupt_fill = g_corrupt_fill;
    if (g_block_emulation) { pb.blocks = &emu; pb.block_min_classes = 1; }
    pb.block_verify = g_block_verify; pb.tick_seq = g_tick_seq; pb.memo = g_memo;
    hqprice::EmulatedSweeper pemu;
    if (g_price_emulation) { pemu.fail_at = g_price_fault; pemu.budget = g_block_budget; if (g_price_min_cols) pemu.min_cols = g_price_min_cols; pb.pricer = &pemu; }
    hqhost::Counts cnt;
    if (g_xfn && g_xworld > 1) {
        struct FnExchange : hqprice::Exchange { bool allgather(const void *snd, void *rcv, size_t bytes) override { return g_xfn(g_xuser, snd, rcv, bytes) == 0; } } xch;
        xch.rank = g_xrank; xch.world = g_xworld;
        ShardedBlocks sh_blocks(emu, xch, g_xmin_classes);
        hqprice::ShardedSweeper sh_sweeps(pemu, xch, g_xmin_blocks);
        if (pb.blocks) pb.blocks = &sh_blocks;
        if (pb.pricer) pb.pricer = &sh_sweeps;
        cnt = hqhost::run_scheduling_solver(pb, batches);
        g_xcalls = (uint32_t)xch.n_calls;
    } else cnt = hqhost::run_scheduling_solver(pb, batches);
    if (cnt.error) return fail(ctx, cnt.error, cnt.errmsg);
    g_last_guard[0] = cnt.blocks_verified; g_last_guard[1] = cnt.blocks_mismatch; g_last_guard[2] = cnt.blocks_rejected;
    g_last_memo = cnt.blocks_memo;
    g_last_blocks_device = cnt.blocks_device; g_last_blocks_host = cnt.blocks_host; g_last_price_sweeps = (uint32_t)cnt.price_sweeps; g_last_price_rounds = (uint32_t)cnt.price_rounds;
    g_last_stage_us[0] = cnt.t_classify_us; g_last_stage_us[1] = cnt.t_blocks_us; g_last_stage_us[2] = cnt.t_decode_us;
    for (size_t i = 0; i < cnt.mn_rq.size(); i++)
        for (auto &set : cnt.mn_sets[i]) { g_last_mn_rq.push_back(cnt.mn_rq[i]); g_last_mn_worker.insert(g_last_mn_worker.end(), set.begin(), set.end()); g_last_mn_off.push_back((uint32_t)g_last_mn_worker.size()); }
    ctx->cnt_rq.clear(); ctx->cnt_variant.clear(); ctx->cnt_worker.clear(); ctx->cnt_value.clear();
    cnt.pairs();
    for (size_t k = 0; k < cnt.keys.size(); k++)
        for (auto &wc : cnt.per_key[k]) { ctx->cnt_rq.push_back(cnt.keys[k].first); ctx->cnt_variant.push_back(cnt.keys[k].second); ctx->cnt_worker.push_back(wc.first); ctx->cnt_value.push_back(wc.second); }
    out->n_counts = (uint32_t)ctx->cnt_rq.size(); out->count_rq = ctx->cnt_rq.data(); out->count_variant = ctx->cnt_variant.data();
    out->count_worker = ctx->cnt_worker.data(); out->count_value = ctx->cnt_value.data();
    out->is_optimal = cnt.is_optimal; out->is_canonical = cnt.is_canonical && cnt.is_optimal;
    out->status = cnt.is_optimal ? HQTICK_DONE : (cnt.empty() ? HQTICK_NO_PROGRESS : HQTICK_NEED_MORE_COMPUTE);
    return out->status;
}

int hqtick_debug_host_query(const hqtick_config *config, const hqtick_snapshot *s, const hqtick_query_workers *fake, const uint8_t *vflags, const uint32_t *vtmc,
                            const uint8_t *fake_vflags, const uint32_t *fake_vtmc, uint32_t n_levels, const uint64_t *levels, const uint32_t *hist,
                            hqtick_query_result *out) {
    if (!config || !s || !fake || !out) return HQTICK_E_INVALID;
    static thread_local hqtick_ctx *holder = nullptr;
    if (!holder) holder = new hqtick_ctx();
    hqtick_ctx *ctx = holder;
    ctx->cfg = *config;
    if (int rc = validate(ctx, s, false)) return rc;
    const uint32_t R = s->n_resources, Q = s->n_requests;
    WorkerEval ev; ev.flags = vflags; ev.tmc = vtmc;
    hqhost::Problem pb;
    fill_problem(pb, s, ctx->cfg, ev);
    hqhost::WorkerSet fw;
    fw.n = fake->n_workers; fw.R = R; fw.id = fake->worker_id; fw.total = fake->worker_total; fw.free_ = fake->worker_total;
    fw.remaining_ns = fake->worker_remaining_ns; fw.min_util = fake->worker_min_utilization; fw.flags = nullptr; fw.group = nullptr;
    fw.vflags = fake_vflags; fw.vtmc = fake_vtmc; fw.n_variant_slots = Q ? s->rq_variant_off[Q] : 0;
    fw.blocked.assign(fw.n, {});
    hqhost::group_equal_rows(fw, true);
    pb.custom = &fw;
    Scan sc; sc.Q = Q; sc.L = n_levels; sc.G = n_levels * Q;
    sc.levels.assign(levels, levels + n_levels); sc.hist.assign(hist, hist + (size_t)n_levels * Q);
    runs_from_hist(sc);
    std::vector<hqhost::QueueLevels> qlv = queue_levels(sc, s);
    std::vector<hqhost::TaskBatch> batches = hqhost::create_task_batches(pb, qlv);
    EmulatedBlocks emu(g_block_budget);
    if (g_block_emulation) { pb.blocks = &emu; pb.block_min_classes = 1; }
    hqhost::Counts cnt = hqhost::run_scheduling_solver(pb, batches);
    if (cnt.error) return fail(ctx, cnt.error, cnt.errmsg);
    ctx->q_loaded.assign(fake->n_workers, 0);
    for (auto &k : cnt.per_key) for (auto &wc : k) if (wc.second > 0) ctx->q_loaded[wc.first] = 1;
    out->n_workers = fake->n_workers; out->is_loaded = ctx->q_loaded.data(); out->is_optimal = cnt.is_optimal;
    return 0;
}

#endif

int hqtick_set_shard(hqtick_ctx *ctx, uint32_t shard_index, uint32_t shard_count) {
    if (!ctx) return HQTICK_E_INVALID;
    if (shard_count > 1 && shard_index >= shard_count) return fail(ctx, HQTICK_E_INVALID, "shard_index >= shard_count");
    if (shard_count > 1 && ctx->asg.on) return fail(ctx, HQTICK_E_UNSUPPORTED, "hqtick_set_shard: the assignment ledger is on (hqtick_assigned_disable first)");
    ctx->shard_index = shard_count > 1 ? shard_index : 0; ctx->shard_count = shard_count > 1 ? shard_count : 1;
    return 0;
}

int hqtick_set_exchange(hqtick_ctx *ctx, hqtick_exchange_fn fn, void *user) {
    if (!ctx) return HQTICK_E_INVALID;
    ctx->xfn = fn; ctx->xuser = fn ? user : nullptr;
    return 0;
}

// ... 201 lines not shown
```

hyperqueue_amd/csrc/milp.cpp:

```cpp
#include "milp.h"
#include "lp_tab.h"
#include "price.h"

#include <algorithm>
#include <chrono>
#include <cstdio>
#include <cstdlib>
#include <cmath>
#include <climits>
#include <cstring>
#include <functional>
#include <numeric>
#include <string>
#include <unordered_map>

namespace hqmilp {
namespace {

using namespace lp;

struct DSUlite {
    std::vector<int> p;
    explicit DSUlite(int n) : p(n) { std::iota(p.begin(), p.end(), 0); }
    int find(int a) { while (p[a] != a) { p[a] = p[p[a]]; a = p[a]; } return a; }
// ... 1252 lines not shown
    auto row_ok = [&](int i, double a) {
        const double tol = 1e-7 * (1.0 + std::fabs(mdl.rhs[i]));
        return mdl.rtype[i] == ROW_MAX ? a <= mdl.rhs[i] + tol : (mdl.rtype[i] == ROW_MIN ? a >= mdl.rhs[i] - tol : std::fabs(a - mdl.rhs[i]) <= tol);
    };
    for (int i = 0; i < m; i++) if (!row_ok(i, act[i])) return false;
    std::vector<int> order;
    order_by_cost_desc(mdl.obj.data(), n, order);
    for (int pass = 0; pass < 64; pass++) {
        bool changed = false;
        for (int j : order) {
            if (mdl.obj[j] <= 0.0) break;
            double step = ub[j] - x[j];
            for (int k = coff[j]; k < coff[j + 1] && step >= 1.0; k++) {
                const int i = crow[k]; const double a = ccoef[k];
                if (mdl.rtype[i] == ROW_EQ) { step = 0.0; break; }
                if (a > 0.0 && mdl.rtype[i] == ROW_MAX) { const double room = mdl.rhs[i] - act[i]; if (room < 0.5 * a) { step = 0.0; break; } step = std::min(step, std::floor(room / a + 1e-9)); }
                else if (a < 0.0 && mdl.rtype[i] == ROW_MIN) { const double room = act[i] - mdl.rhs[i]; if (room < -0.5 * a) { step = 0.0; break; } step = std::min(step, std::floor(room / -a + 1e-9)); }
            }
            if (step < 1.0) continue;
            x[j] += step; changed = true;
            for (int k = coff[j]; k < coff[j + 1]; k++) act[crow[k]] += ccoef[k] * step;
        }
        bool dropped = false;
        for (int j = 0; j < n; j++) {
            if (mdl.kind[j] != COL_BOOL || mdl.obj[j] != 0.0 || x[j] != 1.0) continue;
            bool ok = true;
            for (int k = coff[j]; k < coff[j + 1] && ok; k++) ok = row_ok(crow[k], act[crow[k]] - ccoef[k]);
            if (!ok) continue;
            x[j] = 0.0; dropped = true;
            for (int k = coff[j]; k < coff[j + 1]; k++) act[crow[k]] -= ccoef[k];
        }
        if (!changed && !dropped) break;
        if (!dropped) break;
    }
    return true;
}

}

void columns_by_cost_desc(const double *c, int n, std::vector<int> &out) { order_by_cost_desc(c, n, out); }

thread_local int g_fast_path = -1;
void set_fast_path(int on) { g_fast_path = on; }
thread_local int g_block_runs = -1;
thread_local Probe *g_probe = nullptr;
void set_block_runs(int on) { g_block_runs = on; }
bool block_runs_on() {
    static const bool env_on = !(getenv("HQMILP_BLOCK_RUNS") && atoi(getenv("HQMILP_BLOCK_RUNS")) == 0);
    return g_block_runs < 0 ? env_on : g_block_runs != 0;
}

const double ROW_TOL = 1e-6;

namespace {
bool solve_fast(const Model &mdl_in, double time_limit_s, double rel_gap, hqprice::Sweeper *sweeper, const double ts0, Result &res_out) {
    static const bool tracing_solve = getenv("HQMILP_TRACE") != nullptr;
    auto tmark = [&](const char *what) { if (tracing_solve && mdl_in.ncols() > 1000) fprintf(stderr, "[milp] solve(): %s at %.3f ms\n", what, (wall() - ts0) * 1e3); };
    static const bool fast_env = !(getenv("HQMILP_FAST") && atoi(getenv("HQMILP_FAST")) == 0);
    const bool fast_on = g_fast_path < 0 ? fast_env : g_fast_path != 0;
    const int FAST_MIN_COLS = 2048;
    const bool hints_there = (int)mdl_in.col_group.size() == mdl_in.ncols() && (int)mdl_in.row_lhs.size() == mdl_in.nrows() && (int)mdl_in.row_lhs_len.size() == mdl_in.nrows();
    const bool takes_it = fast_on && sweeper && rel_gap > 0.0 && mdl_in.ncols() >= FAST_MIN_COLS && mdl_in.ncols() >= (int)sweeper->min_cols && hints_there && (int)mdl_in.start.size() != mdl_in.ncols();
    if (takes_it || (g_probe && hints_there)) {
        const int n = mdl_in.ncols(), m = mdl_in.nrows();
        hqprice::ModelView mv;
        mv.n = n; mv.m = m; mv.obj = mdl_in.obj.data(); mv.kind = mdl_in.kind.data(); mv.rtype = mdl_in.rtype.data(); mv.rhs = mdl_in.rhs.data();
        mv.roff = mdl_in.roff.data(); mv.rcol = mdl_in.rcol.data(); mv.rcoef = mdl_in.rcoef.data(); mv.col_group = mdl_in.col_group.data();
        mv.row_implied = (int)mdl_in.row_implied.size() == m ? mdl_in.row_implied.data() : nullptr; mv.row_lhs = mdl_in.row_lhs.data(); mv.row_lhs_len = mdl_in.row_lhs_len.data(); mv.list_off = mdl_in.list_off.data(); mv.list_col = mdl_in.list_col.data(); mv.n_lists = (int)mdl_in.list_off.size() - 1;
        if ((int)mdl_in.row_block.size() == m && (int)mdl_in.col_ub.size() == n) { mv.row_block = mdl_in.row_block.data(); mv.col_ub = mdl_in.col_ub.data(); }
        static_assert(sizeof(Model::BlockRun) == 7 * sizeof(int32_t), "ModelView::block_runs reads seven int32 per run");
        if (!mdl_in.block_runs.empty()) { mv.block_runs = &mdl_in.block_runs[0].col0; mv.n_block_runs = (int)mdl_in.block_runs.size(); }
        mv.run_stats = g_probe ? &g_probe->covered : nullptr; mv.tables_digest = g_probe ? &g_probe->tables : nullptr;
        if (!takes_it) { hqprice::flatten_for_probe(mv, tracing_solve); return false; }
        double cost_scale = 1.0;
        const double tf0 = wall();
        hqprice::Answer pa = hqprice::solve_model(mv, rel_gap, time_limit_s, ts0 + (time_limit_s > 0 ? time_limit_s : 1e18), tracing_solve, *sweeper, &cost_scale);
        if (tracing_solve) fprintf(stderr, "[milp] fast path: ran %d (%s) sweeps %u rounds %u bound %.9f point %.9f, %.3f ms of which %.3f ms inside the sweeps\n", (int)pa.ran, pa.why, pa.sweeps, pa.rounds, pa.ran ? pa.bound : -1.0, pa.x.empty() ? -1.0 : pa.x_value, (wall() - tf0) * 1e3, sweeper->stat_sweep_us / 1e3);
        if (pa.ran && (int)pa.x.size() == n && pa.bound * (1.0 + 1e-9) + 1e-12 <= pa.x_value + rel_gap * std::fabs(pa.x_value)) {
            bool ok = true;
            for (int j = 0; j < n && ok; j++) { const double v = pa.x[(size_t)j]; if (v < -1e-9 || std::fabs(v - std::floor(v + 0.5)) > 1e-9 || (mdl_in.kind[j] == COL_BOOL && v > 1.0 + 1e-9)) ok = false; }
            std::vector<double> lhs_act; std::vector<uint8_t> lhs_seen;
            for (int i = 0; i < m && ok; i++) {
                double a = 0.0;
                int k0 = mdl_in.roff[i];
                const int L = mdl_in.row_lhs[i];
                if (L >= 0) {
                    if ((size_t)L >= lhs_seen.size()) { lhs_seen.resize((size_t)L + 1, 0); lhs_act.resize((size_t)L + 1, 0.0); }
                    if (!lhs_seen[(size_t)L]) { double s = 0.0; for (int k = mdl_in.list_off[L]; k < mdl_in.list_off[L + 1]; k++) s += pa.x[(size_t)mdl_in.list_col[k]]; lhs_act[(size_t)L] = s; lhs_seen[(size_t)L] = 1; }
                    a = lhs_act[(size_t)L];
                }
                for (int k = k0; k < mdl_in.roff[i + 1]; k++) a += mdl_in.rcoef[k] * pa.x[(size_t)mdl_in.rcol[k]];
                const double tol = std::max(ROW_TOL, 1e-9 * std::max(1.0, std::fabs(mdl_in.rhs[i])));
                if (mdl_in.rtype[i] != ROW_MIN && a > mdl_in.rhs[i] + tol) ok = false;
                if (mdl_in.rtype[i] != ROW_MAX && a < mdl_in.rhs[i] - tol) ok = false;
            }
            double z_pt = 0.0;
            if (ok) {
                for (int j = 0; j < n; j++) z_pt += mdl_in.obj[j] * std::floor(pa.x[(size_t)j] + 0.5);
                const double zs = cost_scale > 0.0 ? z_pt / cost_scale : z_pt;
                if (!(pa.bound * (1.0 + 1e-9) + 1e-12 <= zs + rel_gap * std::fabs(zs))) ok = false;
            }
            if (ok) {
                Result res;
                res.x = std::move(pa.x);
                for (double &v : res.x) v = std::floor(v + 0.5);
                res.feasible = true; res.optimal = true; res.canonical = false;
                res.n_components = 1; res.nodes = pa.sweeps; res.price_sweeps = (int)pa.sweeps; res.price_rounds = (int)pa.rounds; res.price_total_us = (wall() - tf0) * 1e6;
                res.objective = z_pt;
                tmark("fast path certified");
                res_out = std::move(res);
                return true;
            }
            if (tracing_solve) fprintf(stderr, "[milp] fast path: the certified point fails a row of the model (or its own objective misses the certificate): classic path\n");
        }
    }
    return false;
}
}

static Result solve_classic(const Model &mdl_in, double time_limit_s, bool canonical, double rel_gap, hqprice::Sweeper *sweeper, const double ts0);

Result solve(const Model &mdl_arg, double time_limit_s, bool canonical, double rel_gap, hqprice::Sweeper *sweeper) {
    const double ts_entry = wall();
    { Result r; if (solve_fast(mdl_arg, time_limit_s, rel_gap, sweeper, ts_entry, r)) return r; }
    if (mdl_arg.has_lists()) {
        Model plain = mdl_arg;
        plain.expand_lists();
        return solve_classic(plain, time_limit_s, canonical, rel_gap, sweeper, ts_entry);
    }
    return solve_classic(mdl_arg, time_limit_s, canonical, rel_gap, sweeper, ts_entry);
}

static Result solve_classic(const Model &mdl_in, double time_limit_s, bool canonical, double rel_gap, hqprice::Sweeper *sweeper, const double ts0) {
    static const bool tracing_solve = getenv("HQMILP_TRACE") != nullptr;
    auto tmark = [&](const char *what) { if (tracing_solve && mdl_in.ncols() > 1000) fprintf(stderr, "[milp] solve(): %s at %.3f ms\n", what, (wall() - ts0) * 1e3); };
    Model snapped;
    bool need_snap = false;
    for (size_t k = 0; k < mdl_in.rcoef.size() && !need_snap; k++) {
        if (mdl_in.kind[mdl_in.rcol[k]] != COL_BOOL) continue;
        const double c = mdl_in.rcoef[k], g = std::round(c * 10000.0) / 10000.0;
        if (g != c && std::fabs(g - c) <= ROW_TOL) need_snap = true;
    }
    if (need_snap) {
        snapped = mdl_in;
        for (size_t k = 0; k < snapped.rcoef.size(); k++) {
            if (snapped.kind[snapped.rcol[k]] != COL_BOOL) continue;
            const double c = snapped.rcoef[k], g = std::round(c * 10000.0) / 10000.0;
            if (g != c && std::fabs(g - c) <= ROW_TOL) snapped.rcoef[k] = g;
        }
    }
    {
        const Model &src = need_snap ? snapped : mdl_in;
        const double GRID = 10000.0;
        std::vector<long long> ci;
        std::vector<uint8_t> reach;
        struct Seen { std::vector<long long> ci; double rhs, new_rhs; };
        std::vector<Seen> seen_rows; size_t seen_next = 0; const size_t SEEN_CAP = 8;
        struct Cut { int row; long long d, rhs; };
        std::vector<Cut> cuts; std::vector<long long> cut_d;
        for (int i = 0; i < src.nrows(); i++) {
            if (src.rtype[i] != ROW_MAX) continue;
            const int a = src.roff[i], b = src.roff[i + 1];
            if (b - a < 1 || !(src.rhs[i] > 0.0) || src.rhs[i] > 1e11) continue;
            ci.clear();
            bool ok = true;
            for (int k = a; k < b && ok; k++) {
                const double c = src.rcoef[k] * GRID, r = std::round(c);
                if (!(src.rcoef[k] > 0.0) || r < 1.0 || std::fabs(c - r) > 1e-6 * std::max(1.0, r) || r > 9e15) ok = false; else ci.push_back((long long)r);
            }
            if (!ok) continue;
            double new_rhs;
            const Seen *hit = nullptr;
            for (const Seen &sr : seen_rows) if (sr.rhs == src.rhs[i] && sr.ci == ci) { hit = &sr; break; }
            if (hit) new_rhs = hit->new_rhs;
            else {
                long long g = 0;
                for (long long c : ci) { long long x = c, y = g; while (y) { const long long t = x % y; x = y; y = t; } g = x; }
// ... 228 lines not shown
```

hyperqueue_amd/csrc/milp.h:

```cpp
#pragma once
#include <cstddef>
#include <cstdint>
#include <algorithm>
#include <vector>

namespace hqprice { struct Sweeper; }

namespace hqmilp {

enum { COL_NAT = 0, COL_BOOL = 1 };
enum { ROW_MIN = 0, ROW_MAX = 1, ROW_EQ = 2 };

struct Model {
    std::vector<double> obj;
    std::vector<uint8_t> kind;
    std::vector<uint8_t> rtype;
    std::vector<double> rhs;
    std::vector<int> roff{0};
    std::vector<int> rcol;
    std::vector<double> rcoef;
    std::vector<double> start;
    std::vector<int32_t> col_group;
    std::vector<uint8_t> row_implied;
    std::vector<int32_t> row_lhs, row_lhs_len;
// ... 4 lines not shown
        if (!has_lists()) return;
        const int m = nrows();
        std::vector<int> noff; noff.reserve((size_t)m + 1); noff.push_back(0);
        size_t total = rcol.size();
        for (int i = 0; i < m; i++) if (i < (int)row_lhs.size() && row_lhs[i] >= 0) total += (size_t)(list_off[row_lhs[i] + 1] - list_off[row_lhs[i]]);
        std::vector<int> ncol; std::vector<double> ncoef; ncol.reserve(total); ncoef.reserve(total);
        for (int i = 0; i < m; i++) {
            if (i < (int)row_lhs.size() && row_lhs[i] >= 0) {
                const int l = row_lhs[i];
                ncol.insert(ncol.end(), list_col.begin() + list_off[l], list_col.begin() + list_off[l + 1]);
                ncoef.resize(ncol.size(), 1.0);
            }
            ncol.insert(ncol.end(), rcol.begin() + roff[i], rcol.begin() + roff[i + 1]);
            ncoef.insert(ncoef.end(), rcoef.begin() + roff[i], rcoef.begin() + roff[i + 1]);
            noff.push_back((int)ncol.size());
        }
        roff.swap(noff); rcol.swap(ncol); rcoef.swap(ncoef);
        list_off.assign(1, 0); list_col.clear();
        std::fill(row_lhs.begin(), row_lhs.end(), -1); std::fill(row_lhs_len.begin(), row_lhs_len.end(), 0);
    }
    std::vector<int32_t> row_block;
    std::vector<uint32_t> col_ub;
    struct BlockRun { int32_t col0, row0, term0, n_blocks, n_cols, n_rows, n_terms; };
    std::vector<BlockRun> block_runs;
    int ncols() const { return (int)obj.size(); }
    int nrows() const { return (int)rhs.size(); }
    int add_col(double w, uint8_t k) {
        obj.push_back(w);
        kind.push_back(k);
        return (int)obj.size() - 1;
    }
    void begin_row(uint8_t t, double b) {
        rtype.push_back(t);
        rhs.push_back(b);
    }
    void term(int c, double v) {
        rcol.push_back(c);
        rcoef.push_back(v);
    }
    void end_row() { roff.push_back((int)rcol.size()); }
};

struct Result {
    std::vector<double> x;
    double objective = 0.0;
    bool feasible = false;
    bool optimal = false;
    bool canonical = true;
    long nodes = 0, lp_iters = 0;
    int n_components = 0;
    int price_sweeps = 0, price_rounds = 0;
    double price_bound_us = 0, price_total_us = 0;
    long hull_solves = 0, hull_solves_nonpacking = 0;
};

const double REFERENCE_MIP_REL_GAP = 1e-4;

Result solve(const Model &m, double time_limit_s, bool canonical = true, double rel_gap = REFERENCE_MIP_REL_GAP, hqprice::Sweeper *sweeper = nullptr);

void columns_by_cost_desc(const double *c, int n, std::vector<int> &out);
void set_fast_path(int on);
void set_block_runs(int on);
bool block_runs_on();
struct Probe { uint64_t model = 0, tables = 0, runs = 0, covered = 0; bool corrupt_runs = false; };
extern thread_local Probe *g_probe;
inline uint64_t fnv1a(uint64_t h, const void *p, size_t bytes) { const unsigned char *b = (const unsigned char *)p; for (size_t i = 0; i < bytes; i++) h = (h ^ b[i]) * 1099511628211ull; return h; }
template <class T> inline uint64_t fnv1a_vec(uint64_t h, const std::vector<T> &v) { const uint64_t n = v.size(); h = fnv1a(h, &n, 8); return v.empty() ? h : fnv1a(h, v.data(), v.size() * sizeof(T)); }
const uint64_t FNV_BASIS = 1469598103934665603ull;

}
```

hyperqueue_amd/csrc/price.hip:

```cpp
#include <hip/hip_runtime.h>

#include <algorithm>
#include <chrono>
#include <cstdio>
#include <cstdlib>
#include <cstring>
#include <type_traits>
#include <vector>

#include "dev_wave.h"
#include "price_core.h"
#include "price_dev.h"

namespace hqprice {

static_assert(PARTS == ASLOTS, "the master's parts are the kernel's activity slots");
constexpr int ASUB = 4;

namespace {

struct SweepResult {
    double cx, rc, bnd;
    uint32_t n_budget, max_steps;
    long long act[KMAX];
    double part_cx[ASLOTS];
    long long part_act[ASLOTS * KMAX];
    uint32_t seq;
};

struct PartVal { uint32_t nbud, mx; };

struct SweepArgs {
    Tables t;
    SweepOut out;
    uint32_t budget, seq;
    uint32_t *tickets;
    long long *tact;
    PartVal *pval;
    SweepResult *res;
    uint32_t first, local;
    double *lv_cx, *lv_rc, *lv_bnd; uint32_t *lv_steps;
    double pi[KMAX];
};

__device__ __forceinline__ double ld_dev(const double *p) { return __longlong_as_double((long long)__hip_atomic_load(reinterpret_cast<const unsigned long long *>(p), __ATOMIC_RELAXED, __HIP_MEMORY_SCOPE_AGENT)); }
__device__ __forceinline__ long long ld_dev(const long long *p) { return (long long)__hip_atomic_load(reinterpret_cast<const unsigned long long *>(p), __ATOMIC_RELAXED, __HIP_MEMORY_SCOPE_AGENT); }
__device__ __forceinline__ uint32_t ld_dev(const uint32_t *p) { return __hip_atomic_load(p, __ATOMIC_RELAXED, __HIP_MEMORY_SCOPE_AGENT); }
__device__ __forceinline__ void st_dev(long long *p, long long v) { __hip_atomic_store(reinterpret_cast<unsigned long long *>(p), (unsigned long long)v, __ATOMIC_RELAXED, __HIP_MEMORY_SCOPE_AGENT); }
__device__ __forceinline__ void st_dev(uint32_t *p, uint32_t v) { __hip_atomic_store(p, v, __ATOMIC_RELAXED, __HIP_MEMORY_SCOPE_AGENT); }
__device__ __forceinline__ void st_host(double *p, double v) { __hip_atomic_store(reinterpret_cast<unsigned long long *>(p), (unsigned long long)__double_as_longlong(v), __ATOMIC_RELAXED, __HIP_MEMORY_SCOPE_SYSTEM); }
__device__ __forceinline__ void st_host(long long *p, long long v) { __hip_atomic_store(reinterpret_cast<unsigned long long *>(p), (unsigned long long)v, __ATOMIC_RELAXED, __HIP_MEMORY_SCOPE_SYSTEM); }
__device__ __forceinline__ void st_host(uint32_t *p, uint32_t v) { __hip_atomic_store(p, v, __ATOMIC_RELAXED, __HIP_MEMORY_SCOPE_SYSTEM); }
__device__ __forceinline__ void acked() { __builtin_amdgcn_fence(__ATOMIC_RELEASE, "workgroup"); }

template <class SH, int NW>
__global__ __launch_bounds__(WAVE * NW) void k_price_sweep(const SweepArgs a) {
    __shared__ SH S;
    using WV = typename std::conditional<NW == 1, hqblock::DevWave, hqblock::DevGroup<NW>>::type;
    WV wv;
    if (NW > 1 && threadIdx.x >= WAVE) { hqblock::pool_helper(wv, S); return; }
    const uint32_t lane = threadIdx.x;
    const uint32_t nb = a.t.n_blocks, K = a.t.K, per = part_size(nb), b = a.first + blockIdx.x, p = b / per;
    solve_priced_block(wv, S, a.t, a.pi, b, a.out, a.budget);
    uint64_t *prof = a.out.prof ? a.out.prof + (size_t)b * PSLOTS : nullptr;
    const uint32_t r0 = a.first, r1 = a.first + gridDim.x;
    const uint32_t pb0 = p * per > r0 ? p * per : r0, pe = p * per + per < nb ? p * per + per : nb, pb1 = pe < r1 ? pe : r1;
    acked();
    if (prof && lane == 0) prof[11] = wv.now();
    uint32_t last = 0;
    if (lane == 0) last = __hip_atomic_fetch_add(&a.tickets[1 + p], 1u, __ATOMIC_RELAXED, __HIP_MEMORY_SCOPE_AGENT) == pb1 - pb0 - 1 ? 1u : 0u;
    last = (uint32_t)__builtin_amdgcn_readfirstlane((int)last);
    if (prof && lane == 0) prof[12] = wv.now();
    if (!last) return;
    {
        long long vs[2][ASUB];
#pragma unroll
        for (int u = 0; u < 2; u++) {
            const uint32_t k = lane + (uint32_t)u * WAVE;
#pragma unroll
            for (int sub = 0; sub < ASUB; sub++) vs[u][sub] = k < K ? ld_dev(&a.out.act[((size_t)p * ASUB + sub) * K + k]) : 0;
        }
        double *scr = &S.py[0][0];
        static_assert(sizeof(S.py) >= 256 * sizeof(double), "a round of the part's c.x values is staged in the dual pool's storage");
        uint32_t nbud = 0, mx = 0;
        double s4 = 0.0;
        for (uint32_t c0 = p * per; c0 < pe; c0 += 256) {
            double v[4]; uint32_t vst[4];
#pragma unroll
            for (int u = 0; u < 4; u++) { const uint32_t q = c0 + lane + (uint32_t)u * WAVE; v[u] = (q < pe && !a.local) ? ld_dev(&a.out.blk_cx[q]) : 0.0; vst[u] = (q >= pb0 && q < pb1) ? ld_dev(&a.out.blk_steps[q]) : 0u; }
#pragma unroll
            for (int u = 0; u < 4; u++) { scr[lane + (uint32_t)u * WAVE] = v[u]; nbud += vst[u] >> 31; const uint32_t st = vst[u] & 0x7FFFFFFFu; mx = st > mx ? st : mx; }
            wv.sync();
            const uint32_t cnt = pe - c0 < 256u ? pe - c0 : 256u;
            if (lane < 4 && !a.local) for (uint32_t i = lane; i < cnt; i += 4) s4 += scr[i];
            wv.sync();
        }
#pragma unroll
        for (int off = 32; off >= 1; off >>= 1) { nbud += __shfl_xor(nbud, off, 64); const uint32_t om = __shfl_xor(mx, off, 64); mx = om > mx ? om : mx; }
        const double s1 = __shfl(s4, 1, 64), s2 = __shfl(s4, 2, 64), s3 = __shfl(s4, 3, 64);
        const double pcx = ((s4 + s1) + s2) + s3;
#pragma unroll
        for (int u = 0; u < 2; u++) {
            const uint32_t k = lane + (uint32_t)u * WAVE;
            if (k >= K) continue;
            long long v = 0;
#pragma unroll
            for (int sub = 0; sub < ASUB; sub++) { v += vs[u][sub]; st_dev(&a.out.act[((size_t)p * ASUB + sub) * K + k], 0); }
            st_host(&a.res->part_act[(size_t)p * K + k], v);
            if (v != 0 && !a.local) atomicAdd(reinterpret_cast<unsigned long long *>(&a.tact[k]), (unsigned long long)v);
        }
        if (lane == 0) {
            st_dev(&a.pval[p].nbud, nbud); st_dev(&a.pval[p].mx, mx);
            if (!a.local) st_host(&a.res->part_cx[p], pcx);
            st_dev(&a.tickets[1 + p], 0u);
        }
        __threadfence_system();
    }
    const uint32_t p_first = r0 / per, p_last = (r1 - 1) / per;
    if (lane == 0) last = __hip_atomic_fetch_add(&a.tickets[0], 1u, __ATOMIC_RELAXED, __HIP_MEMORY_SCOPE_AGENT) == p_last - p_first ? 1u : 0u;
    last = (uint32_t)__builtin_amdgcn_readfirstlane((int)last);
    if (!last) return;
    if (a.local) {
        for (uint32_t b0 = r0 + lane; b0 < r1; b0 += WAVE * 8) {
            double vcx[8], vrc[8], vbd[8]; uint32_t vst[8];
#pragma unroll
            for (int u = 0; u < 8; u++) { const uint32_t q = b0 + (uint32_t)u * WAVE; const bool in = q < r1; vcx[u] = in ? ld_dev(&a.out.blk_cx[q]) : 0.0; vrc[u] = in ? ld_dev(&a.out.blk_rc[q]) : 0.0; vbd[u] = in ? ld_dev(&a.out.blk_bnd[q]) : 0.0; vst[u] = in ? ld_dev(&a.out.blk_steps[q]) : 0u; }
#pragma unroll
            for (int u = 0; u < 8; u++) { const uint32_t q = b0 + (uint32_t)u * WAVE; if (q < r1) { st_host(&a.lv_cx[q], vcx[u]); st_host(&a.lv_rc[q], vrc[u]); st_host(&a.lv_bnd[q], vbd[u]); st_host(&a.lv_steps[q], vst[u]); } }
        }
    } else {
        const uint32_t n_parts = (nb + per - 1) / per;
        long long ta[2] = {0, 0};
#pragma unroll
        for (int u = 0; u < 2; u++) { const uint32_t k = lane + (uint32_t)u * WAVE; if (k < K) ta[u] = ld_dev(&a.tact[k]); }
        uint32_t pn = 0, pm = 0;
        if (lane < n_parts) { pn = ld_dev(&a.pval[lane].nbud); pm = ld_dev(&a.pval[lane].mx); }
        double cx = 0.0, rc = 0.0, bnd = 0.0;
        for (uint32_t b0 = lane; b0 < nb; b0 += WAVE * 8) {
            double vcx[8], vrc[8], vbd[8];
#pragma unroll
            for (int u = 0; u < 8; u++) { const uint32_t q = b0 + (uint32_t)u * WAVE; const bool in = q < nb; vcx[u] = in ? ld_dev(&a.out.blk_cx[q]) : 0.0; vrc[u] = in ? ld_dev(&a.out.blk_rc[q]) : 0.0; vbd[u] = in ? ld_dev(&a.out.blk_bnd[q]) : 0.0; }
#pragma unroll
            for (int u = 0; u < 8; u++) { if (b0 + (uint32_t)u * WAVE >= nb) break; cx += vcx[u]; rc += vrc[u]; bnd += vbd[u]; }
        }
        double *red = &S.py[0][0];
        red[lane] = cx; red[WAVE + lane] = rc; red[2 * WAVE + lane] = bnd;
#pragma unroll
        for (int off = 8; off >= 1; off >>= 1) { pn += __shfl_xor(pn, off, 64); const uint32_t om = __shfl_xor(pm, off, 64); pm = om > pm ? om : pm; }
        wv.sync();
        double tcx = 0.0, trc = 0.0, tb = 0.0;
        if (lane == 0) for (int l = 0; l < WAVE; l++) { tcx += red[l]; trc += red[WAVE + l]; tb += red[2 * WAVE + l]; }
#pragma unroll
        for (int u = 0; u < 2; u++) {
            const uint32_t k = lane + (uint32_t)u * WAVE;
            if (k >= K) continue;
            st_dev(&a.tact[k], 0);
            st_host(&a.res->act[k], ta[u]);
            for (uint32_t i = n_parts; i < (uint32_t)ASLOTS; i++) st_host(&a.res->part_act[(size_t)i * K + k], 0);
        }
        if (lane >= n_parts && lane < (uint32_t)ASLOTS) st_host(&a.res->part_cx[lane], 0.0);
        if (lane == 0) { st_host(&a.res->cx, tcx); st_host(&a.res->rc, trc); st_host(&a.res->bnd, tb); st_host(&a.res->n_budget, pn); st_host(&a.res->max_steps, pm); }
    }
    if (lane == 0) st_dev(&a.tickets[0], 0u);
    if (prof && lane == 0) prof[13] = wv.now();
    __threadfence_system();
    wv.sync();
    if (prof && lane == 0) prof[14] = wv.now();
    if (lane == 0) __hip_atomic_store(&a.res->seq, a.seq, __ATOMIC_RELEASE, __HIP_MEMORY_SCOPE_SYSTEM);
}

constexpr size_t SYNC_ACT = 128, SYNC_PACT = SYNC_ACT + (size_t)ASLOTS * ASUB * KMAX * 8, SYNC_PVAL = SYNC_PACT + (size_t)KMAX * 8, SYNC_BYTES = SYNC_PVAL + (size_t)ASLOTS * sizeof(PartVal);

constexpr int NPROF = 13;
const int PROF_FROM[NPROF] = {0, 1, 3, 4, 5, 5, 8, 9, 10, 6, 11, 12, 13};
const int PROF_TO[NPROF]   = {1, 2, 4, 5, 6, 8, 9, 10, 6, 11, 12, 13, 14};
const char *const PROF_NAME[NPROF] = {"reduced costs + compaction", "dual pool + order + greedy fills", "level lists + root bound", "walk", "results + activities", "[results: zero the sums", "pattern + sums in LDS", "atomics + cost loads", "values]",
                                      "acknowledgements before the ticket", "part ticket", "part sums + sweep ticket + totals (last block)", "system fence (last block)"};

size_t al16(size_t v) { return (v + 15) & ~(size_t)15; }
double now_us() { return std::chrono::duration<double, std::micro>(std::chrono::steady_clock::now().time_since_epoch()).count(); }

}

DeviceSweeper::~DeviceSweeper() { h_stage.release(); h_res.release(); h_pats.release(); h_pin.release(); h_blkv.release(); d_tab.release(); d_pats.release(); d_blk.release(); d_sync.release(); d_prof.release(); }

bool DeviceSweeper::size_buffers(const HostTables &t, uint32_t max_sweeps) {
    if (profile && (!h_prof.ensure((size_t)t.n_blocks * PSLOTS * 8 + 64) || !d_prof.ensure((size_t)t.n_blocks * PSLOTS * 8 + 64))) return false;
    T = &t; n_sweeps = 0; cap_sweeps = max_sweeps; blocks_only = false;
    max_block_cols = 0;
    for (uint32_t b = 0; b < t.n_blocks; b++) max_block_cols = std::max(max_block_cols, t.blk_off[b + 1] - t.blk_off[b]);
    if (force_nmax) max_block_cols = (uint32_t)hqblock::NMAX;
    o_off = 0; o_m = al16(o_off + (size_t)(t.n_blocks + 1) * 4); o_cap = al16(o_m + t.n_blocks); o_cost = al16(o_cap + (size_t)t.n_blocks * MMAX * 8);
    o_a = al16(o_cost + (size_t)t.n_cols * 8); o_ccap = al16(o_a + (size_t)t.n_cols * MMAX * 8); o_woff = al16(o_ccap + (size_t)t.n_cols * 4);
    o_wrow = al16(o_woff + (size_t)(t.n_cols + 1) * 4);
    if (!h_res.ensure(sizeof(SweepResult) + 64)) return false;
    if (!h_pin.ensure((size_t)std::min<uint32_t>(max_sweeps, PIN_SWEEPS) * t.n_cols * 2 + 64)) return false;
    in_flight = false;
    return d_pats.ensure((size_t)max_sweeps * t.n_cols * 2) && d_blk.ensure((size_t)t.n_blocks * 28 + 64) && d_sync.ensure(SYNC_BYTES);
}

void DeviceSweeper::stage_blocks(const HostTables &t) {
    unsigned char *h = h_stage.as<unsigned char>();
    memcpy(h + o_off, t.blk_off.data(), (size_t)(t.n_blocks + 1) * 4); memcpy(h + o_m, t.blk_m.data(), t.n_blocks); memcpy(h + o_cap, t.blk_cap.data(), (size_t)t.n_blocks * MMAX * 8);
    memcpy(h + o_cost, t.col_cost.data(), (size_t)t.n_cols * 8); memcpy(h + o_a, t.col_a.data(), (size_t)t.n_cols * MMAX * 8); memcpy(h + o_ccap, t.col_cap.data(), (size_t)t.n_cols * 4);
}

bool DeviceSweeper::begin(const HostTables &t, uint32_t max_sweeps) {
    if (t.K > (uint32_t)KMAX || t.n_blocks == 0) return false;
    if (!size_buffers(t, max_sweeps)) return false;
    const size_t nw = t.w_row.size();
    wide_room = std::max(wide_room, nw);
    o_wcoef = al16(o_wrow + nw * 2); tab_bytes = al16(o_wcoef + nw * 4);
    if (!h_stage.ensure(tab_bytes) || !d_tab.ensure(tab_bytes)) return false;
    unsigned char *h = h_stage.as<unsigned char>();
    stage_blocks(t);
    memcpy(h + o_woff, t.col_woff.data(), (size_t)(t.n_cols + 1) * 4);
    if (nw) { memcpy(h + o_wrow, t.w_row.data(), nw * 2); memcpy(h + o_wcoef, t.w_coef.data(), nw * 4); }
    if (hipMemcpyAsync(d_tab.p, h, tab_bytes, hipMemcpyHostToDevice, stream) != hipSuccess) return false;
    if (!sync_clean) { if (hipMemsetAsync(d_sync.p, 0, SYNC_BYTES, stream) != hipSuccess) return false; }
    SweepResult *r = h_res.as<SweepResult>();
    seq = r->seq;
    return true;
}

int DeviceSweeper::begin_blocks(const HostTables &t, uint32_t max_sweeps) {
    if (t.n_blocks == 0 || !size_buffers(t, max_sweeps)) return 0;
    const size_t room = std::max(wide_room, (size_t)t.n_cols * 4);
    o_wcoef = o_wrow; tab_bytes = o_wrow;
    const size_t dev_bytes = al16(al16(o_wrow + room * 2) + room * 4);
    if (!h_stage.ensure(o_wrow + (dev_bytes - o_woff)) || !d_tab.ensure(dev_bytes)) return 0;
    unsigned char *h = h_stage.as<unsigned char>();
    stage_blocks(t);
    memset(h + o_woff, 0, o_wrow - o_woff);
    if (hipMemcpyAsync(d_tab.p, h, o_wrow, hipMemcpyHostToDevice, stream) != hipSuccess) return 0;
    if (!sync_clean) { if (hipMemsetAsync(d_sync.p, 0, SYNC_BYTES, stream) != hipSuccess) return 0; }
    seq = h_res.as<SweepResult>()->seq;
    blocks_only = true;
    return 1;
}

bool DeviceSweeper::begin_wide() {
    if (!T || !blocks_only) return false;
    const HostTables &t = *T;
    if (t.K > (uint32_t)KMAX || t.col_woff.size() != (size_t)t.n_cols + 1) return false;
    const size_t nw = t.w_row.size();
    wide_room = std::max(wide_room, nw);
    o_wcoef = al16(o_wrow + nw * 2); tab_bytes = al16(o_wcoef + nw * 4);
    const size_t wide_bytes = tab_bytes - o_woff;
    if (o_wrow + wide_bytes > h_stage.cap || tab_bytes > d_tab.cap) {
        if (hipStreamSynchronize(stream) != hipSuccess) return false;
        if (!h_stage.ensure(o_wrow + wide_bytes) || !d_tab.ensure(tab_bytes)) return false;
        unsigned char *h = h_stage.as<unsigned char>();
        stage_blocks(t);
        memcpy(h + o_woff, t.col_woff.data(), (size_t)(t.n_cols + 1) * 4);
        if (nw) { memcpy(h + o_wrow, t.w_row.data(), nw * 2); memcpy(h + o_wcoef, t.w_coef.data(), nw * 4); }
        if (hipMemcpyAsync(d_tab.p, h, tab_bytes, hipMemcpyHostToDevice, stream) != hipSuccess) return false;
    } else {
        unsigned char *h = h_stage.as<unsigned char>() + o_wrow;
        memcpy(h, t.col_woff.data(), (size_t)(t.n_cols + 1) * 4);
        if (nw) { memcpy(h + (o_wrow - o_woff), t.w_row.data(), nw * 2); memcpy(h + (o_wcoef - o_woff), t.w_coef.data(), nw * 4); }
        if (hipMemcpyAsync(d_tab.as<unsigned char>() + o_woff, h, wide_bytes, hipMemcpyHostToDevice, stream) != hipSuccess) return false;
    }
    blocks_only = false;
    return true;
}

bool DeviceSweeper::set_caps(const int32_t *col_cap) {
    if (!T) return false;
    memcpy(h_stage.as<unsigned char>() + o_ccap, col_cap, (size_t)T->n_cols * 4);
    return hipMemcpyAsync(d_tab.as<unsigned char>() + o_ccap, h_stage.as<unsigned char>() + o_ccap, (size_t)T->n_cols * 4, hipMemcpyHostToDevice, stream) == hipSuccess;
}

bool DeviceSweeper::set_block_caps(const double *blk_cap) {
    if (!T) return false;
    const size_t bytes = (size_t)T->n_blocks * MMAX * 8;
    memcpy(h_stage.as<unsigned char>() + o_cap, blk_cap, bytes);
    return hipMemcpyAsync(d_tab.as<unsigned char>() + o_cap, h_stage.as<unsigned char>() + o_cap, bytes, hipMemcpyHostToDevice, stream) == hipSuccess;
}

bool DeviceSweeper::sweep(const double *pi, SweepTotals &out) { return launch(pi, 0, T ? T->n_blocks : 0, false, &out); }

bool DeviceSweeper::sweep_range(const double *pi, uint32_t b0, uint32_t b1, RangeValues &rv) {
    if (!T || b1 > T->n_blocks || b0 > b1) return false;
    const uint32_t nb = T->n_blocks;
    if (!h_blkv.ensure((size_t)nb * 28 + 64)) return false;
    if (b1 > b0) { if (!launch(pi, b0, b1, true, nullptr)) return false; }
    else {
        if (n_sweeps >= cap_sweeps) return false;
        SweepResult *r = h_res.as<SweepResult>();
        memset(r->part_act, 0, sizeof(r->part_act));
        n_sweeps++;
    }
    unsigned char *h = h_blkv.as<unsigned char>();
    rv = RangeValues{(const double *)h, (const double *)(h + (size_t)nb * 8), (const double *)(h + (size_t)nb * 16), (const uint32_t *)(h + (size_t)nb * 24), h_res.as<SweepResult>()->part_act};
    return true;
}

bool DeviceSweeper::launch(const double *pi, uint32_t b0, uint32_t b1, bool local, SweepTotals *outp) { return launch_only(pi, b0, b1, local) && wait_done(outp); }
bool DeviceSweeper::sweep_launch(const double *pi) { return launch_only(pi, 0, T ? T->n_blocks : 0, false); }
bool DeviceSweeper::sweep_finish(SweepTotals &out) { return wait_done(&out); }

bool DeviceSweeper::launch_only(const double *pi, uint32_t b0, uint32_t b1, bool local) {
    if (!T || n_sweeps >= cap_sweeps || b1 <= b0 || in_flight) return false;
    if (blocks_only && (n_sweeps != 0 || local)) return false;
    const HostTables &t = *T;
    const uint32_t K = blocks_only ? 0u : t.K;
    unsigned char *d = d_tab.as<unsigned char>();
    SweepArgs a;
    a.t = Tables{t.n_blocks, t.n_cols, K, (const uint32_t *)(d + o_off), (const uint8_t *)(d + o_m), (const double *)(d + o_cap), (const double *)(d + o_cost), (const double *)(d + o_a),
                 (const int32_t *)(d + o_ccap), (const uint32_t *)(d + o_woff), (const uint16_t *)(d + o_wrow), (const int32_t *)(d + o_wcoef)};
    unsigned char *blk = d_blk.as<unsigned char>();
    uint16_t *xdst = n_sweeps < PIN_SWEEPS ? h_pin.dev<uint16_t>() + (size_t)n_sweeps * t.n_cols : d_pats.as<uint16_t>() + (size_t)n_sweeps * t.n_cols;
    a.out = SweepOut{xdst, (double *)blk, (double *)(blk + (size_t)t.n_blocks * 8), (double *)(blk + (size_t)t.n_blocks * 16),
                     (long long *)(d_sync.as<unsigned char>() + SYNC_ACT), (uint32_t *)(blk + (size_t)t.n_blocks * 24), profile ? d_prof.as<uint64_t>() : nullptr, (uint32_t)ASUB, dbg};
    a.budget = budget; a.seq = ++seq; a.tickets = d_sync.as<uint32_t>(); a.tact = (long long *)(d_sync.as<unsigned char>() + SYNC_PACT); a.pval = (PartVal *)(d_sync.as<unsigned char>() + SYNC_PVAL); a.res = h_res.dev<SweepResult>();
    a.first = b0; a.local = local ? 1u : 0u;
    if (local) { unsigned char *lv = h_blkv.dev<unsigned char>(); a.lv_cx = (double *)lv; a.lv_rc = (double *)(lv + (size_t)t.n_blocks * 8); a.lv_bnd = (double *)(lv + (size_t)t.n_blocks * 16); a.lv_steps = (uint32_t *)(lv + (size_t)t.n_blocks * 24); }
    else { a.lv_cx = a.lv_rc = a.lv_bnd = nullptr; a.lv_steps = nullptr; }
    memset(a.pi, 0, sizeof(a.pi));
    if (K) memcpy(a.pi, pi, (size_t)K * 8);
    const double t0 = now_us();
    const uint32_t nblk = b1 - b0;
    const int nw = force_waves == 1 || force_waves == 2 ? force_waves : 4;
#define HQ_SWEEP(SH_, NW_) hipLaunchKernelGGL((k_price_sweep<SH_, NW_>), dim3(nblk), dim3(WAVE * NW_), 0, stream, a)
#define HQ_SWEEP_N(SH_) do { if (nw == 4) HQ_SWEEP(SH_, 4); else if (nw == 2) HQ_SWEEP(SH_, 2); else HQ_SWEEP(SH_, 1); } while (0)
    if (max_block_cols <= 8) HQ_SWEEP_N(hqblock::SharedN<8>);
    else if (max_block_cols <= 16) HQ_SWEEP_N(hqblock::SharedN<16>);
    else HQ_SWEEP_N(hqblock::SharedN<hqblock::NMAX>);
#undef HQ_SWEEP_N
#undef HQ_SWEEP
    if (hipGetLastError() != hipSuccess) return false;
    in_flight = true; sync_clean = false; flight_t0 = t0; flight_blocks = b1 - b0; flight_k = K;
    return true;
}

bool DeviceSweeper::wait_done(SweepTotals *outp) {
    if (!T || !in_flight) return false;
    in_flight = false;
    const HostTables &t = *T;
    const double t0 = flight_t0;
    volatile SweepResult *r = h_res.as<SweepResult>();
    for (uint64_t spins = 0;; spins++) {
        if (__atomic_load_n(&r->seq, __ATOMIC_ACQUIRE) == seq) break;
        if ((spins & 0xFFFF) == 0xFFFF && now_us() - t0 > 2.0e6) {
            if (hipStreamSynchronize(stream) != hipSuccess) return false;
            if (__atomic_load_n(&r->seq, __ATOMIC_ACQUIRE) != seq) return false;
            break;
        }
    }
    last_kernel_us = now_us() - t0;
    sync_clean = true;
    if (profile) {
        if (hipMemcpyAsync(h_prof.p, d_prof.p, (size_t)t.n_blocks * PSLOTS * 8, hipMemcpyDeviceToHost, stream) != hipSuccess || hipStreamSynchronize(stream) != hipSuccess) return false;
        const uint64_t *pr = h_prof.as<uint64_t>();
        for (int st = 0; st < NPROF; st++) {
            const int from = PROF_FROM[st], to = PROF_TO[st];
            std::vector<double> v; v.reserve(t.n_blocks);
            for (uint32_t b = 0; b < t.n_blocks; b++) { const uint64_t t0s = pr[(size_t)b * PSLOTS + from], t1s = pr[(size_t)b * PSLOTS + to]; if (t0s && t1s >= t0s) v.push_back((double)(t1s - t0s) / 100.0); }
            if (v.empty()) continue;
            std::sort(v.begin(), v.end()); prof_med[st] += v[v.size() / 2]; prof_max[st] += v.back();
        }
        uint64_t first = ~0ull, last_done = 0, seq_at = 0;
        for (uint32_t b = 0; b < t.n_blocks; b++) { const uint64_t *q = pr + (size_t)b * PSLOTS; if (q[0] && q[0] < first) first = q[0]; if (q[6] > last_done) last_done = q[6]; if (q[14] > seq_at) seq_at = q[14]; }
        if (first != ~0ull) { prof_span += (double)(last_done - first) / 100.0; if (seq_at) prof_tail += (double)(seq_at - last_done) / 100.0; }
        double smax = 0; for (uint32_t b = 0; b < t.n_blocks; b++) smax = std::max(smax, (double)pr[(size_t)b * PSLOTS + 7]);
        prof_steps += smax; prof_n++;
    }
    total_sweeps++; total_block_solves += flight_blocks; total_us += last_kernel_us;
    n_sweeps++;
    if (!outp) return true;
    SweepTotals &out = *outp;
    out.cx = r->cx; out.rc = r->rc; out.bnd = r->bnd; out.n_budget = r->n_budget; out.max_steps = r->max_steps;
    const uint32_t K = flight_k;
    out.act.resize(K);
    for (uint32_t k = 0; k < K; k++) out.act[k] = r->act[k];
    out.part_cx.assign(r->part_cx, r->part_cx + ASLOTS);
    out.part_act.resize((size_t)ASLOTS * K);
    for (size_t i = 0; i < (size_t)ASLOTS * K; i++) out.part_act[i] = r->part_act[i];
    return true;
}

const uint16_t *DeviceSweeper::patterns(uint32_t first, uint32_t count) {
    if (!T || first + count > n_sweeps || in_flight) return nullptr;
    const size_t nc = T->n_cols, bytes = (size_t)count * nc * 2;
    if (first + count <= PIN_SWEEPS) return h_pin.as<uint16_t>() + (size_t)first * nc;
    if (!h_pats.ensure(bytes + 64)) return nullptr;
    if (count == 0) return h_pats.as<uint16_t>();
    const uint32_t n_pin = first < PIN_SWEEPS ? PIN_SWEEPS - first : 0;
    if (n_pin) memcpy(h_pats.p, h_pin.as<uint16_t>() + (size_t)first * nc, (size_t)n_pin * nc * 2);
    if (hipMemcpyAsync(h_pats.as<uint16_t>() + (size_t)n_pin * nc, d_pats.as<uint16_t>() + (size_t)(first + n_pin) * nc, bytes - (size_t)n_pin * nc * 2, hipMemcpyDeviceToHost, stream) != hipSuccess) return nullptr;
    if (hipStreamSynchronize(stream) != hipSuccess) return nullptr;
    return h_pats.as<uint16_t>();
}

void DeviceSweeper::end() {
    if (in_flight) { hipStreamSynchronize(stream); in_flight = false; }
    if (profile && prof_n) {
        fprintf(stderr, "[price profile] %d sweeps, per block and sweep (us; median over blocks / slowest block, averaged over the sweeps):", prof_n);
        for (int st = 0; st < NPROF; st++) fprintf(stderr, "  %s %.1f / %.1f;", PROF_NAME[st], prof_med[st] / prof_n, prof_max[st] / prof_n);
        fprintf(stderr, "  first block's start -> last block's results %.1f, -> completion word stored %.1f more;", prof_span / prof_n, prof_tail / prof_n);
        fprintf(stderr, "  most search steps of a block %.0f; sweep as the host saw it %.1f us\n", prof_steps / prof_n, total_us / (double)std::max<uint64_t>(1, total_sweeps));
        for (int st = 0; st < NPROF; st++) prof_med[st] = prof_max[st] = 0; prof_steps = 0; prof_span = prof_tail = 0; prof_n = 0;
    }
    T = nullptr; blocks_only = false;
}

}
```

hyperqueue_amd/csrc/price_dev.h:

```cpp
#pragma once
#include <hip/hip_runtime.h>

#include <cstdlib>

#include "devbuf.h"
#include "price.h"

namespace hqprice {

struct DeviceSweeper : Sweeper {
    hipStream_t stream = nullptr;
    hqbuf::PinBuf h_stage, h_res, h_pats, h_pin, h_prof, h_blkv;
    static constexpr uint32_t PIN_SWEEPS = 64;
    bool sync_clean = false;
    bool in_flight = false; double flight_t0 = 0; uint32_t flight_blocks = 0;
    bool profile = getenv("HQTICK_PRICE_PROFILE") != nullptr; double prof_med[16] = {0}, prof_max[16] = {0}, prof_steps = 0, prof_span = 0, prof_tail = 0; int prof_n = 0;
    hqbuf::DevBuf d_tab, d_pats, d_blk, d_sync, d_prof;
    const HostTables *T = nullptr;
    size_t o_off = 0, o_m = 0, o_cap = 0, o_cost = 0, o_a = 0, o_ccap = 0, o_woff = 0, o_wrow = 0, o_wcoef = 0, tab_bytes = 0;
    bool blocks_only = false;
    uint32_t flight_k = 0;
    size_t wide_room = 0;
    uint32_t n_sweeps = 0, cap_sweeps = 0, seq = 0;
    uint32_t max_block_cols = 0;
    bool force_nmax = getenv("HQTICK_PRICE_NMAX") != nullptr;
    int force_waves = getenv("HQTICK_PRICE_WAVES") ? atoi(getenv("HQTICK_PRICE_WAVES")) : 0;
    uint32_t dbg = getenv("HQTICK_PRICE_DBG") ? (uint32_t)atoi(getenv("HQTICK_PRICE_DBG")) : 0u;
    double last_kernel_us = 0;
    uint64_t total_sweeps = 0, total_block_solves = 0; double total_us = 0;
    explicit DeviceSweeper(hipStream_t s) : stream(s) {}
    ~DeviceSweeper() override;
    bool begin(const HostTables &t, uint32_t max_sweeps) override;
    int begin_blocks(const HostTables &t, uint32_t max_sweeps) override;
    bool begin_wide() override;
    bool size_buffers(const HostTables &t, uint32_t max_sweeps);
    void stage_blocks(const HostTables &t);
    bool set_caps(const int32_t *col_cap) override;
    bool set_block_caps(const double *blk_cap) override;
    bool sweep(const double *pi, SweepTotals &out) override;
    bool sweep_range(const double *pi, uint32_t b0, uint32_t b1, RangeValues &out) override;
    bool launch(const double *pi, uint32_t b0, uint32_t b1, bool local, SweepTotals *out);
    bool launch_only(const double *pi, uint32_t b0, uint32_t b1, bool local);
    bool wait_done(SweepTotals *out);
    bool sweep_launch(const double *pi) override;
    bool sweep_finish(SweepTotals &out) override;
    const uint16_t *patterns(uint32_t first, uint32_t count) override;
    void end() override;
};

}
```

include/hqtick_debug.h:

```cpp
#ifndef HQTICK_DEBUG_H
#define HQTICK_DEBUG_H
#include <stdint.h>
#include "hqtick.h"
#ifdef __cplusplus
extern "C" {
#endif
#if defined(__GNUC__)
#pragma GCC visibility push(default)
#endif

int hqtick_debug_milp_solve(int ncols, const double *obj, const uint8_t *col_kind, int nrows, const uint8_t *row_type,
                            const double *rhs, const int *row_off, const int *row_col, const double *row_coef,
                            double time_limit_s, int canonical, double *x_out, double *obj_out, int *is_optimal,
                            long *nodes_out);

int hqtick_debug_last_order(const hqtick_ctx *ctx, uint32_t *n_runs, uint32_t *n_levels, double *order_us);

int hqtick_debug_last_scan(const hqtick_ctx *ctx, int which, uint32_t *n_levels, uint32_t *n_groups, uint32_t shape[4],
                           uint64_t *levels, uint32_t cap_levels, uint32_t *hist, uint32_t cap_groups);

int hqtick_debug_host_stages(const hqtick_config *config, const hqtick_snapshot *snapshot, const uint8_t *vflags, const uint32_t *vtmc,
                             uint32_t n_levels, const uint64_t *levels, const uint32_t *hist, hqtick_result *out);

int hqtick_debug_host_query(const hqtick_config *config, const hqtick_snapshot *snapshot, const hqtick_query_workers *fake,
                            const uint8_t *vflags, const uint32_t *vtmc, const uint8_t *fake_vflags, const uint32_t *fake_vtmc,
                            uint32_t n_levels, const uint64_t *levels, const uint32_t *hist, hqtick_query_result *out);

int hqtick_debug_milp_was_canonical(void);
void hqtick_debug_milp_last_hull(long *solves, long *nonpacking);

void hqtick_debug_map_order_u32(const uint32_t *keys, uint32_t n, uint32_t *out_pos);

int hqtick_debug_block_solve_host(uint32_t n_cols, uint32_t n_resources, const uint32_t *ent_off, const uint32_t *ent_res, const uint8_t *ent_kind,
                                  const uint64_t *ent_amount, const uint32_t *weight, const double *pool, uint32_t n_classes, const uint64_t *free_,
                                  const uint64_t *total, const uint64_t *elig, uint32_t budget, uint32_t *x, uint32_t *status, uint32_t *steps);
void hqtick_debug_set_block_emulation(int on, uint32_t budget);
void hqtick_debug_last_stage_us(double *out3);
void hqtick_debug_last_blocks(uint32_t *n_emulated, uint32_t *n_host);

int hqtick_time_kernel(hqtick_ctx *ctx, int which, int iters, double *avg_us);
int hqtick_timeline(const hqtick_ctx *ctx, double *out, int cap);
const uint64_t *hqtick_block_profile_last(const hqtick_ctx *ctx, uint32_t *n_classes);


void hqtick_debug_set_price_emulation(int on, uint32_t min_cols);
void hqtick_debug_set_price_fault(int fail_at);
void hqtick_debug_set_fast_path(int on);
void hqtick_debug_check_model_hints(int on);
int hqtick_debug_model_hint_mismatches(void);
void hqtick_debug_set_block_runs(int on);
void hqtick_debug_last_coupled_digest(uint64_t out[4]);
void hqtick_debug_set_early_sweep(int on);
uint32_t hqtick_debug_early_sweeps(void);
void hqtick_debug_capture_first_cut(int on);
uint32_t hqtick_debug_first_cut(unsigned char *out, uint32_t cap);
void hqtick_debug_corrupt_block_runs(int on);
void hqtick_debug_last_price(uint32_t *sweeps, uint32_t *rounds);
uint32_t hqtick_debug_last_mn(const uint32_t **rq, const uint32_t **off, const uint32_t **worker);
int hqtick_debug_milp_solve_priced(int ncols, const double *obj, const uint8_t *col_kind, const int32_t *col_group, int nrows, const uint8_t *row_type,
                                   const uint8_t *row_implied, const double *rhs, const int *row_off, const int *row_col, const double *row_coef,
                                   double time_limit_s, int use_sweeps, uint32_t min_cols, double *x_out, double *obj_out, int *is_optimal, double *stats_out);

struct hqwire_tables;
struct hqwire_records;
struct hqwire_output;
int hqwire_debug_encode_host(const struct hqwire_tables *tables, const struct hqwire_records *records, const struct hqwire_output *out);
int hqwire_debug_encode_host_order(const struct hqwire_tables *tables, const struct hqwire_records *records, const struct hqwire_output *out, int order);

void hqtick_debug_set_block_guard(uint32_t verify, uint32_t tick_seq, int corrupt_mode, uint32_t corrupt_class, uint32_t corrupt_fill);
void hqtick_debug_last_block_guard(uint32_t *verified, uint32_t *mismatch, uint32_t *rejected);
void hqtick_debug_set_block_memo(int on);
uint32_t hqtick_debug_last_block_memo(void);
void hqtick_debug_set_exchange(hqtick_exchange_fn fn, void *user, uint32_t rank, uint32_t world, uint32_t min_blocks, uint32_t min_classes);
uint32_t hqtick_debug_last_exchange_calls(void);
int hqtick_debug_exchange(hqtick_ctx *ctx, const void *send, void *recv, size_t bytes_per_rank);
#if defined(__GNUC__)
#pragma GCC visibility pop
#endif
#ifdef __cplusplus
}
#endif
#endif
```

Before: 70.00 million.

## Defer MILP solution row check to overlap with device work; host-side sweep totals

The row-feasibility check of the coupled MILP solution is moved out of the solver critical path into a pending check. That check runs while the device selection/expansion work is in flight, and the tick is retried without the fast path if it fails, including restoring consumed tasks. Separately, the device sweeper drops the last-block cross-part reduction. It now polls per-part sequence numbers and computes the totals on the host from per-block values. This adds retry complexity and rollback risk in exchange for overlapping the check with GPU work and shortening the kernel tail.

```diff
diff --git a/hyperqueue_amd/csrc/debug_capi.cpp b/hyperqueue_amd/csrc/debug_capi.cpp
--- a/hyperqueue_amd/csrc/debug_capi.cpp
+++ b/hyperqueue_amd/csrc/debug_capi.cpp
@@ -89,3 +89,5 @@
     if (out && cap) memcpy(out, b.data(), std::min<size_t>(cap, b.size()));
     return (uint32_t)b.size();
 }
+extern "C" void hqtick_debug_set_deferred_check(int on) { hqmilp::set_defer_check(on); }
+extern "C" void hqtick_debug_fail_deferred_checks(uint32_t n) { hqmilp::fail_next_deferred_checks(n); }
diff --git a/hyperqueue_amd/csrc/host_model.cpp b/hyperqueue_amd/csrc/host_model.cpp
--- a/hyperqueue_amd/csrc/host_model.cpp
+++ b/hyperqueue_amd/csrc/host_model.cpp
@@ -1257,7 +1257,8 @@
         size_t run_blocks = 0; for (const auto &br : m.block_runs) run_blocks += (size_t)br.n_blocks;
         fprintf(stderr, "[model] cuts done at %.3f ms: %d columns, %d rows, %zu terms, %zu worker signatures, %zu (batch, cut, blocker) passes over the workers; %zu equal-block runs over %zu blocks, %zu (cut, blocker) passes decided once\n", (t_model1 - t_model0) / 1e3, m.ncols(), m.nrows(), m.rcol.size(), sig_rep.size(), n_triples, m.block_runs.size(), run_blocks, n_decided_once);
     }
-    hqmilp::Result sol = hqmilp::solve(m, pb.time_limit_s, !pb.certificate_only, hqmilp::REFERENCE_MIP_REL_GAP, pb.pricer);
+    const unsigned solve_flags = (pb.deferred ? hqmilp::SOLVE_DEFER_CHECK : 0u) | (pb.no_fast_path ? hqmilp::SOLVE_NO_FAST_PATH : 0u);
+    hqmilp::Result sol = hqmilp::solve(m, pb.time_limit_s, !pb.certificate_only, hqmilp::REFERENCE_MIP_REL_GAP, pb.pricer, solve_flags);
     if (trace_model) fprintf(stderr, "[model] solve done %.3f ms after the model\n", (clock_us() - t_model1) / 1e3);
     out.pre_us = t_model0 - t_enter; out.model_us = t_model1 - t_model0; out.milp_us = clock_us() - t_model1; out.price_sweeps = sol.price_sweeps; out.price_rounds = sol.price_rounds; out.price_us = sol.price_total_us;
     out.milp_nodes = sol.nodes; out.milp_cols = m.ncols(); out.milp_rows = m.nrows(); out.milp_components = sol.n_components;
@@ -1309,6 +1310,11 @@
     hqhb::insertion_order(mn_hash.data(), (uint32_t)mn_hash.size(), ord);
     for (uint32_t k : ord) { out.mn_rq.push_back(mn_list[k]); out.mn_sets.push_back(std::move(mn_sets[k])); }
     if (trace_model) fprintf(stderr, "[model] decoded %.3f ms after the model, %.3f ms after the solver was entered\n", (clock_us() - t_model1) / 1e3, (clock_us() - t_enter) / 1e3);
+    if (sol.check_pending) {
+        hqmilp::PendingCheck &pc = *pb.deferred;
+        pc.model = std::move(m); pc.x = std::move(sol.x); pc.bound = sol.check_bound; pc.cost_scale = sol.check_cost_scale; pc.rel_gap = hqmilp::REFERENCE_MIP_REL_GAP; pc.pending = true;
+        out.check_pending = true;
+    }
     return out;
 }
 
diff --git a/hyperqueue_amd/csrc/host_model.h b/hyperqueue_amd/csrc/host_model.h
--- a/hyperqueue_amd/csrc/host_model.h
+++ b/hyperqueue_amd/csrc/host_model.h
@@ -102,6 +102,8 @@
     WorkerSet real;
     const WorkerSet *custom = nullptr;
     double time_limit_s = 5.0;
+    hqmilp::PendingCheck *deferred = nullptr;
+    bool no_fast_path = false;
     bool certificate_only = false;
     bool rq_multi_node(uint32_t rq) const { return variants[rqs[rq].first_variant].multi_node(); }
     bool capable_rqv(const WorkerSet &ws, uint32_t w, uint32_t rq) const {
@@ -143,6 +145,7 @@
     size_t key_size(size_t k) const { return pairs_built ? per_key[k].size() : lists[key_list[k]].widx.size(); }
     bool is_optimal = true;
     bool is_canonical = true;
+    bool check_pending = false;
     bool empty() const {
         if (!pairs_built) { for (size_t k = 0; k < keys.size(); k++) if (key_size(k)) return false; }
         for (auto &k : per_key) if (!k.empty()) return false;
diff --git a/hyperqueue_amd/csrc/hqtick.cpp b/hyperqueue_amd/csrc/hqtick.cpp
--- a/hyperqueue_amd/csrc/hqtick.cpp
+++ b/hyperqueue_amd/csrc/hqtick.cpp
@@ -119,6 +119,7 @@
     hqtick_exchange_fn xfn = nullptr; void *xuser = nullptr;
     DevBuf d_xsend, d_xrecv; PinBuf h_xsend, h_xrecv;
     uint32_t shard_min_blocks = 1025, shard_min_classes = 1025; bool shard_solve = true;
+    hqmilp::PendingCheck pending_check; uint32_t check_retries = 0;
     uint32_t block_verify = 2, tick_seq = 0;
     uint64_t x_calls = 0, x_bytes = 0; double x_us = 0;
     double tl[32] = {}; int ntl = 0;
@@ -718,6 +719,8 @@
     }
 };
 
+constexpr int CHECK_FAILED = -0x7fff0001;
+
 struct TickRun {
     hqtick_ctx *ctx; const hqtick_snapshot *s; hqtick_result *out; const bool use_resident;
     PlanScratch &ps; hqhost::Problem &pb;
@@ -737,6 +740,8 @@
     bool compact = false, delta16 = false; size_t o_rs = 0, o_rf = 0; uint32_t max_out = 0;
     uint64_t *h_rec_task = nullptr, *mn_ids = nullptr; uint8_t *h_rec_var = nullptr, *h_rec_kind = nullptr;
     bool assembled = false;
+    bool no_fast_path = false;
+    bool check_failed = false;
     double t0 = 0;
 
     TickRun(hqtick_ctx *c, const hqtick_snapshot *snap, hqtick_result *o, bool resident)
@@ -1100,7 +1105,13 @@
         return 0;
     }
 
+    bool settle_check() {
+        if (ctx->pending_check.pending && !ctx->pending_check.run()) check_failed = true;
+        return !check_failed;
+    }
+
     int phase_c() {
+        if (!n_sel && !settle_check()) return CHECK_FAILED;
         size_t n_mn_ids = 0; for (auto &sets : cnt.mn_sets) n_mn_ids += sets.size();
         delta16 = compact && (ctx->cfg.flags & HQTICK_FLAG_COMPACT_DELTA16) != 0;
         if (compact) {
@@ -1222,8 +1233,10 @@
             }
             mark();
             assemble_host_part();
+            settle_check();
             if (expand_is_last) HQ_HIP(hipEventSynchronize(ctx->ev[11])); else HQ_HIP(hipStreamSynchronize(ctx->stream));
             ctx->sweep_inflight = false;
+            if (check_failed) return CHECK_FAILED;
             if (flags[0]) return fail(ctx, HQTICK_E_CAPACITY, "mapping kernel capacity exceeded");
             if (sc.ordered && ctx->h_ordh.as<uint32_t>()[hqk::ORDER_DIGITS * 256 + 2]) return fail(ctx, HQTICK_E_DEVICE, "ordered view: the selection left its request's segment");
             if (ctx->timing) { const double us_ = elapsed_us(ctx->ev[4], ctx->ev[5]); if (us_ >= 0) ctx->stats.select_us = us_; }
@@ -1306,6 +1319,9 @@
         pb.blocks = &dev_blocks; pb.block_min_classes = ctx->block_min_classes; pb.pricer = ctx->pricer;
         pb.block_verify = ctx->block_verify; pb.tick_seq = ctx->tick_seq++;
         pb.memo = (ctx->cfg.flags & (HQTICK_FLAG_NO_BLOCK_MEMO | HQTICK_FLAG_NO_TICK_CACHES)) ? nullptr : &ctx->block_memo;
+        ctx->pending_check.pending = false;
+        pb.no_fast_path = no_fast_path;
+        pb.deferred = (!no_fast_path && !ctx->sink && !CtxExchange::available(ctx) && hqmilp::defer_check_on()) ? &ctx->pending_check : nullptr;
         double shard_sweep_us = -1.0;
         ctx->x_calls = 0; ctx->x_bytes = 0; ctx->x_us = 0;
         if (CtxExchange::available(ctx)) {
@@ -1319,7 +1335,7 @@
                 shard_sweep_us = sh_sweeps.stat_sweep_us;
             } else cnt = hqhost::run_scheduling_solver(pb, batches);
         } else cnt = hqhost::run_scheduling_solver(pb, batches);
-        pb.blocks = nullptr; pb.pricer = nullptr;
+        pb.blocks = nullptr; pb.pricer = nullptr; pb.deferred = nullptr; pb.no_fast_path = false;
         ctx->stats.price_sweeps = (uint32_t)cnt.price_sweeps; ctx->stats.price_rounds = (uint32_t)cnt.price_rounds; ctx->stats.price_us = cnt.price_us; ctx->stats.milp_us = cnt.milp_us; ctx->stats.model_us = cnt.model_us; ctx->stats.solve_pre_us = cnt.pre_us;
         ctx->stats.price_sweep_us = shard_sweep_us >= 0.0 ? shard_sweep_us : (ctx->pricer ? ctx->pricer->stat_sweep_us : 0.0); ctx->stats.milp_cols = (uint32_t)cnt.milp_cols; ctx->stats.milp_rows = (uint32_t)cnt.milp_rows;
         ctx->stats.n_classes_verified = cnt.blocks_verified; ctx->stats.n_classes_mismatch = cnt.blocks_mismatch; ctx->stats.n_classes_rejected = cnt.blocks_rejected; ctx->stats.n_classes_memo = cnt.blocks_memo;
@@ -1412,30 +1428,55 @@
         full.retracting_redirect_worker = ctx->retr_red_worker.data(); full.retracting_redirect_variant = ctx->retr_red_variant.data();
     }
     int rc;
+    bool check_failed = false;
     {
         TickRun run(ctx, s, out, use_resident);
         rc = run.run();
+        run.settle_check();
+        check_failed = run.check_failed;
+    }
+    auto restore_consumed = [&]() -> bool {
+        bool restored = false;
+        const bool synced = hipStreamSynchronize(ctx->stream) == hipSuccess;
+        if (synced && ctx->last_valid && ctx->last_ordered) {
+            hqk::OrderSelect os = ctx->last_os;
+            os.mark_rq = ctx->d_trq.as<uint32_t>(); os.mark_value = 0; os.mark_and_select = 0;
+            if (hqk::order_select(os, ctx->last_n_sel, ctx->stream) == hipSuccess && hipStreamSynchronize(ctx->stream) == hipSuccess) { ctx->n_live += ctx->last_n_sel; restored = true; }
+        } else if (synced && ctx->last_valid && !ctx->last_ordered && ctx->last_Q && ctx->h_q.ensure(64)) {
+            uint32_t *cntp = ctx->h_q.as<uint32_t>();
+            cntp[0] = 0;
+            if (hqk::ready_restore_consumed(ctx->d_gkey.as<uint16_t>(), ctx->d_trq.as<uint32_t>(), ctx->n_ready, ctx->last_Q, ctx->h_q.dev<uint32_t>(), ctx->stream) == hipSuccess &&
+                hipStreamSynchronize(ctx->stream) == hipSuccess && cntp[0] <= ctx->last_n_sel) {
+                ctx->n_live += ctx->last_n_sel;
+                restored = true;
+            }
+        }
+        ctx->last_valid = false; ctx->last_consumed = true; ctx->last_n_sel = 0;
+        return restored;
+    };
+    if (check_failed) {
+        ctx->check_retries++;
+        bool clean = hipStreamSynchronize(ctx->stream) == hipSuccess;
+        ctx->sweep_inflight = false;
+        if (clean && ctx->consumed_unconfirmed) clean = restore_consumed();
+        else { ctx->last_valid = false; ctx->last_consumed = true; ctx->last_n_sel = 0; }
+        if (ctx->asg.on) ctx->asg.abandon_tick();
+        if (!clean) {
+            if (ctx->consumed_unconfirmed) ctx->resident = false;
+            ctx->consumed_unconfirmed = false;
+            return fail(ctx, HQTICK_E_DEVICE, "the coupled solve's point failed its row check after the tick had taken its tasks, and they could not be put back; upload the ready set again");
+        }
+        ctx->consumed_unconfirmed = false;
+        ctx->tick_seq--;
+        TickRun again(ctx, s, out, use_resident);
+        again.no_fast_path = true;
+        rc = again.run();
     }
     if (ctx->consumed_unconfirmed) {
         ctx->consumed_unconfirmed = false;
         if (rc < 0) {
             const std::string why = ctx->err;
-            bool restored = false;
-            const bool synced = hipStreamSynchronize(ctx->stream) == hipSuccess;
-            if (synced && ctx->last_valid && ctx->last_ordered) {
-                hqk::OrderSelect os = ctx->last_os;
-                os.mark_rq = ctx->d_trq.as<uint32_t>(); os.mark_value = 0; os.mark_and_select = 0;
-                if (hqk::order_select(os, ctx->last_n_sel, ctx->stream) == hipSuccess && hipStreamSynchronize(ctx->stream) == hipSuccess) { ctx->n_live += ctx->last_n_sel; restored = true; }
-            } else if (synced && ctx->last_valid && !ctx->last_ordered && ctx->last_Q && ctx->h_q.ensure(64)) {
-                uint32_t *cntp = ctx->h_q.as<uint32_t>();
-                cntp[0] = 0;
-                if (hqk::ready_restore_consumed(ctx->d_gkey.as<uint16_t>(), ctx->d_trq.as<uint32_t>(), ctx->n_ready, ctx->last_Q, ctx->h_q.dev<uint32_t>(), ctx->stream) == hipSuccess &&
-                    hipStreamSynchronize(ctx->stream) == hipSuccess && cntp[0] <= ctx->last_n_sel) {
-                    ctx->n_live += ctx->last_n_sel;
-                    restored = true;
-                }
-            }
-            ctx->last_valid = false; ctx->last_consumed = true; ctx->last_n_sel = 0;
+            const bool restored = restore_consumed();
             ctx->err = why;
             if (restored) ctx->err += " (HQTICK_FLAG_CONSUME_IN_TICK: what the tick had taken is back in the resident ready set)";
             else { ctx->resident = false; ctx->err += " (HQTICK_FLAG_CONSUME_IN_TICK: the tick had already taken its tasks and they could not be put back; the resident ready set is dropped, upload it again)"; }
@@ -2478,6 +2519,8 @@
 uint32_t hqtick_debug_last_block_memo(void) { return g_last_memo; }
 void hqtick_debug_set_price_emulation(int on, uint32_t min_cols) { g_price_emulation = on; g_price_min_cols = min_cols; }
 void hqtick_debug_set_fast_path(int on) { hqmilp::set_fast_path(on); }
+thread_local uint32_t g_stage_retries = 0;
+uint32_t hqtick_debug_deferred_check_retries(const hqtick_ctx *ctx) { return ctx ? ctx->check_retries : g_stage_retries; }
 void hqtick_debug_check_model_hints(int on) { hqprice::set_check_hints(on != 0); }
 int hqtick_debug_model_hint_mismatches(void) { return hqprice::hint_mismatches(); }
 thread_local int g_price_fault = -1;
@@ -2557,6 +2600,9 @@
     hqprice::EmulatedSweeper pemu;
     if (g_price_emulation) { pemu.fail_at = g_price_fault; pemu.budget = g_block_budget; if (g_price_min_cols) pemu.min_cols = g_price_min_cols; pb.pricer = &pemu; }
     hqhost::Counts cnt;
+    hqmilp::PendingCheck pend;
+    g_stage_retries = 0;
+    if (!(g_xfn && g_xworld > 1) && hqmilp::defer_check_setting() == 1) pb.deferred = &pend;
     if (g_xfn && g_xworld > 1) {
         struct FnExchange : hqprice::Exchange { bool allgather(const void *snd, void *rcv, size_t bytes) override { return g_xfn(g_xuser, snd, rcv, bytes) == 0; } } xch;
         xch.rank = g_xrank; xch.world = g_xworld;
@@ -2566,7 +2612,10 @@
         if (pb.pricer) pb.pricer = &sh_sweeps;
         cnt = hqhost::run_scheduling_solver(pb, batches);
         g_xcalls = (uint32_t)xch.n_calls;
-    } else cnt = hqhost::run_scheduling_solver(pb, batches);
+    } else {
+        cnt = hqhost::run_scheduling_solver(pb, batches);
+        if (cnt.check_pending && !pend.run()) { g_stage_retries++; pb.deferred = nullptr; pb.no_fast_path = true; cnt = hqhost::run_scheduling_solver(pb, batches); }
+    }
     if (cnt.error) return fail(ctx, cnt.error, cnt.errmsg);
     g_last_guard[0] = cnt.blocks_verified; g_last_guard[1] = cnt.blocks_mismatch; g_last_guard[2] = cnt.blocks_rejected;
     g_last_memo = cnt.blocks_memo;
@@ -2583,6 +2632,66 @@
     out->is_optimal = cnt.is_optimal; out->is_canonical = cnt.is_canonical && cnt.is_optimal;
     out->status = cnt.is_optimal ? HQTICK_DONE : (cnt.empty() ? HQTICK_NO_PROGRESS : HQTICK_NEED_MORE_COMPUTE);
     return out->status;
+}
+
+int hqtick_debug_run_sweeps(hqtick_ctx *ctx, uint32_t n_blocks, uint32_t seed, int early, int abandon, uint32_t n_sweeps, double *out, uint32_t cap) {
+    const uint32_t K = 3, NC = 8, ROW = 5 + K + hqprice::PARTS + hqprice::PARTS * K;
+    if (!out || !n_blocks || (size_t)n_sweeps * ROW > cap) return HQTICK_E_INVALID;
+    if (ctx && !ctx->pricer) return fail(ctx, HQTICK_E_UNSUPPORTED, "no device sweeper on this context");
+    uint64_t state = 0x9E3779B97F4A7C15ull ^ ((uint64_t)seed << 17);
+    auto rnd = [&](uint32_t n) { state = state * 6364136223846793005ull + 1442695040888963407ull; return (uint32_t)((state >> 33) % n); };
+    hqprice::HostTables t;
+    t.n_blocks = n_blocks; t.n_cols = n_blocks * NC; t.K = K;
+    t.blk_off.resize((size_t)n_blocks + 1); t.blk_m.assign(n_blocks, 2); t.blk_cap.assign((size_t)n_blocks * hqblock::MMAX, 0.0);
+    t.col_cost.resize(t.n_cols); t.col_a.assign((size_t)t.n_cols * hqblock::MMAX, 0.0); t.col_cap.resize(t.n_cols); t.col_woff.assign(1, 0);
+    for (uint32_t b = 0; b <= n_blocks; b++) t.blk_off[b] = b * NC;
+    for (uint32_t b = 0; b < n_blocks; b++) {
+        t.blk_cap[(size_t)b * hqblock::MMAX] = 12.0 + rnd(12); t.blk_cap[(size_t)b * hqblock::MMAX + 1] = 8.0 + rnd(16);
+        for (uint32_t q = 0; q < NC; q++) {
+            const uint32_t j = b * NC + q;
+            t.col_cost[j] = (double)(1 + rnd(1000)) / 1000.0; t.col_cap[j] = 1 + (int32_t)rnd(6);
+            t.col_a[(size_t)j * hqblock::MMAX] = 1.0 + rnd(4); t.col_a[(size_t)j * hqblock::MMAX + 1] = (double)rnd(4);
+            const uint32_t first = rnd(K), ne = 1 + rnd(2);
+            for (uint32_t e = 0; e < ne; e++) { t.w_row.push_back((uint16_t)((first + e) % K)); t.w_coef.push_back(1 + (int32_t)rnd(2)); }
+            t.col_woff.push_back((uint32_t)t.w_row.size());
+        }
+    }
+    hqprice::EmulatedSweeper emu;
+    hqprice::Sweeper *sw = ctx ? static_cast<hqprice::Sweeper *>(ctx->pricer) : &emu;
+    if (ctx) HQ_HIP(hipSetDevice(ctx->device));
+    const double zero[K] = {0.0, 0.0, 0.0};
+    if (abandon) {
+        if (!sw->begin(t, 4)) return HQTICK_E_DEVICE;
+        sw->pending_k = K;
+        const bool ok = sw->sweep_launch(zero);
+        sw->end();
+        if (!ok) return HQTICK_E_DEVICE;
+    }
+    bool ok = true;
+    uint32_t s0 = 0;
+    hqprice::SweepTotals tot;
+    auto put = [&](uint32_t s_) {
+        double *o = out + (size_t)s_ * ROW;
+        o[0] = tot.cx; o[1] = tot.rc; o[2] = tot.bnd; o[3] = tot.n_budget; o[4] = tot.max_steps;
+        for (uint32_t k = 0; k < K; k++) o[5 + k] = k < tot.act.size() ? (double)tot.act[k] : -1.0;
+        for (int p_ = 0; p_ < hqprice::PARTS; p_++) o[5 + K + p_] = tot.part_cx[p_];
+        for (uint32_t i = 0; i < hqprice::PARTS * K; i++) o[5 + K + hqprice::PARTS + i] = i < tot.part_act.size() ? (double)tot.part_act[i] : -1.0;
+    };
+    if (early && n_sweeps) {
+        if (sw->begin_blocks(t, n_sweeps + 1) != 1) return HQTICK_E_DEVICE;
+        sw->pending_k = 0;
+        ok = sw->sweep_launch(zero) && sw->begin_wide() && sw->sweep_finish(tot);
+        if (ok) { put(0); s0 = 1; }
+    } else ok = sw->begin(t, n_sweeps + 1);
+    for (uint32_t s_ = s0; ok && s_ < n_sweeps; s_++) {
+        double pi[K];
+        for (uint32_t k = 0; k < K; k++) pi[k] = 0.013 * (double)(s_ * (k + 1)) + (s_ ? (double)rnd(100) / 5000.0 : 0.0);
+        ok = sw->sweep(pi, tot);
+        if (ok) put(s_);
+    }
+    sw->end();
+    if (!ok) return ctx ? fail(ctx, HQTICK_E_DEVICE, "hqtick_debug_run_sweeps: a sweep failed") : HQTICK_E_DEVICE;
+    return (int)ROW;
 }
 
 int hqtick_debug_host_query(const hqtick_config *config, const hqtick_snapshot *s, const hqtick_query_workers *fake, const uint8_t *vflags, const uint32_t *vtmc,
diff --git a/hyperqueue_amd/csrc/milp.cpp b/hyperqueue_amd/csrc/milp.cpp
--- a/hyperqueue_amd/csrc/milp.cpp
+++ b/hyperqueue_amd/csrc/milp.cpp
@@ -1328,12 +1328,54 @@
 
 const double ROW_TOL = 1e-6;
 
+bool check_certified_point(const Model &mdl_in, const std::vector<double> &x, const double bound, const double cost_scale, const double rel_gap, double *objective) {
+    const int n = mdl_in.ncols(), m = mdl_in.nrows();
+    if ((int)x.size() != n) return false;
+    bool ok = true;
+    for (int j = 0; j < n && ok; j++) { const double v = x[(size_t)j]; if (v < -1e-9 || std::fabs(v - std::floor(v + 0.5)) > 1e-9 || (mdl_in.kind[j] == COL_BOOL && v > 1.0 + 1e-9)) ok = false; }
+    std::vector<double> lhs_act; std::vector<uint8_t> lhs_seen;
+    for (int i = 0; i < m && ok; i++) {
+        double a = 0.0;
+        int k0 = mdl_in.roff[i];
+        const int L = mdl_in.row_lhs[i];
+        if (L >= 0) {
+            if ((size_t)L >= lhs_seen.size()) { lhs_seen.resize((size_t)L + 1, 0); lhs_act.resize((size_t)L + 1, 0.0); }
+            if (!lhs_seen[(size_t)L]) { double s = 0.0; for (int k = mdl_in.list_off[L]; k < mdl_in.list_off[L + 1]; k++) s += x[(size_t)mdl_in.list_col[k]]; lhs_act[(size_t)L] = s; lhs_seen[(size_t)L] = 1; }
+            a = lhs_act[(size_t)L];
+        }
+        for (int k = k0; k < mdl_in.roff[i + 1]; k++) a += mdl_in.rcoef[k] * x[(size_t)mdl_in.rcol[k]];
+        const double tol = std::max(ROW_TOL, 1e-9 * std::max(1.0, std::fabs(mdl_in.rhs[i])));
+        if (mdl_in.rtype[i] != ROW_MIN && a > mdl_in.rhs[i] + tol) ok = false;
+        if (mdl_in.rtype[i] != ROW_MAX && a < mdl_in.rhs[i] - tol) ok = false;
+    }
+    double z_pt = 0.0;
+    if (ok) {
+        for (int j = 0; j < n; j++) z_pt += mdl_in.obj[j] * std::floor(x[(size_t)j] + 0.5);
+        const double zs = cost_scale > 0.0 ? z_pt / cost_scale : z_pt;
+        if (!(bound * (1.0 + 1e-9) + 1e-12 <= zs + rel_gap * std::fabs(zs))) ok = false;
+    }
+    if (ok && objective) *objective = z_pt;
+    return ok;
+}
+
+thread_local int g_defer_check = -1;
+thread_local uint32_t g_fail_deferred = 0;
+void set_defer_check(int on) { g_defer_check = on; }
+int defer_check_setting() { return g_defer_check; }
+bool defer_check_on() {
+    static const bool env_on = !(getenv("HQMILP_DEFER_CHECK") && atoi(getenv("HQMILP_DEFER_CHECK")) == 0);
+    return g_defer_check < 0 ? env_on : g_defer_check != 0;
+}
+void fail_next_deferred_checks(uint32_t n) { g_fail_deferred = n; }
+bool PendingCheck::take_forced_failure() { if (!g_fail_deferred) return false; g_fail_deferred--; return true; }
+
 namespace {
-bool solve_fast(const Model &mdl_in, double time_limit_s, double rel_gap, hqprice::Sweeper *sweeper, const double ts0, Result &res_out) {
+bool solve_fast(const Model &mdl_in, double time_limit_s, double rel_gap, hqprice::Sweeper *sweeper, const double ts0, const unsigned flags, Result &res_out) {
     static const bool tracing_solve = getenv("HQMILP_TRACE") != nullptr;
     auto tmark = [&](const char *what) { if (tracing_solve && mdl_in.ncols() > 1000) fprintf(stderr, "[milp] solve(): %s at %.3f ms\n", what, (wall() - ts0) * 1e3); };
     static const bool fast_env = !(getenv("HQMILP_FAST") && atoi(getenv("HQMILP_FAST")) == 0);
-    const bool fast_on = g_fast_path < 0 ? fast_env : g_fast_path != 0;
+    const bool defer = (flags & SOLVE_DEFER_CHECK) != 0;
+    const bool fast_on = (flags & SOLVE_NO_FAST_PATH) ? false : g_fast_path < 0 ? fast_env : g_fast_path != 0;
     const int FAST_MIN_COLS = 2048;
     const bool hints_there = (int)mdl_in.col_group.size() == mdl_in.ncols() && (int)mdl_in.row_lhs.size() == mdl_in.nrows() && (int)mdl_in.row_lhs_len.size() == mdl_in.nrows();
     const bool takes_it = fast_on && sweeper && rel_gap > 0.0 && mdl_in.ncols() >= FAST_MIN_COLS && mdl_in.ncols() >= (int)sweeper->min_cols && hints_there && (int)mdl_in.start.size() != mdl_in.ncols();
@@ -1353,37 +1395,17 @@
         hqprice::Answer pa = hqprice::solve_model(mv, rel_gap, time_limit_s, ts0 + (time_limit_s > 0 ? time_limit_s : 1e18), tracing_solve, *sweeper, &cost_scale);
         if (tracing_solve) fprintf(stderr, "[milp] fast path: ran %d (%s) sweeps %u rounds %u bound %.9f point %.9f, %.3f ms of which %.3f ms inside the sweeps\n", (int)pa.ran, pa.why, pa.sweeps, pa.rounds, pa.ran ? pa.bound : -1.0, pa.x.empty() ? -1.0 : pa.x_value, (wall() - tf0) * 1e3, sweeper->stat_sweep_us / 1e3);
         if (pa.ran && (int)pa.x.size() == n && pa.bound * (1.0 + 1e-9) + 1e-12 <= pa.x_value + rel_gap * std::fabs(pa.x_value)) {
-            bool ok = true;
-            for (int j = 0; j < n && ok; j++) { const double v = pa.x[(size_t)j]; if (v < -1e-9 || std::fabs(v - std::floor(v + 0.5)) > 1e-9 || (mdl_in.kind[j] == COL_BOOL && v > 1.0 + 1e-9)) ok = false; }
-            std::vector<double> lhs_act; std::vector<uint8_t> lhs_seen;
-            for (int i = 0; i < m && ok; i++) {
-                double a = 0.0;
-                int k0 = mdl_in.roff[i];
-                const int L = mdl_in.row_lhs[i];
-                if (L >= 0) {
-                    if ((size_t)L >= lhs_seen.size()) { lhs_seen.resize((size_t)L + 1, 0); lhs_act.resize((size_t)L + 1, 0.0); }
-                    if (!lhs_seen[(size_t)L]) { double s = 0.0; for (int k = mdl_in.list_off[L]; k < mdl_in.list_off[L + 1]; k++) s += pa.x[(size_t)mdl_in.list_col[k]]; lhs_act[(size_t)L] = s; lhs_seen[(size_t)L] = 1; }
-                    a = lhs_act[(size_t)L];
-                }
-                for (int k = k0; k < mdl_in.roff[i + 1]; k++) a += mdl_in.rcoef[k] * pa.x[(size_t)mdl_in.rcol[k]];
-                const double tol = std::max(ROW_TOL, 1e-9 * std::max(1.0, std::fabs(mdl_in.rhs[i])));
-                if (mdl_in.rtype[i] != ROW_MIN && a > mdl_in.rhs[i] + tol) ok = false;
-                if (mdl_in.rtype[i] != ROW_MAX && a < mdl_in.rhs[i] - tol) ok = false;
-            }
             double z_pt = 0.0;
-            if (ok) {
-                for (int j = 0; j < n; j++) z_pt += mdl_in.obj[j] * std::floor(pa.x[(size_t)j] + 0.5);
-                const double zs = cost_scale > 0.0 ? z_pt / cost_scale : z_pt;
-                if (!(pa.bound * (1.0 + 1e-9) + 1e-12 <= zs + rel_gap * std::fabs(zs))) ok = false;
-            }
+            const bool ok = defer ? true : check_certified_point(mdl_in, pa.x, pa.bound, cost_scale, rel_gap, &z_pt);
             if (ok) {
                 Result res;
                 res.x = std::move(pa.x);
-                for (double &v : res.x) v = std::floor(v + 0.5);
+                if (defer) { res.check_pending = true; res.check_bound = pa.bound; res.check_cost_scale = cost_scale; }
+                else for (double &v : res.x) v = std::floor(v + 0.5);
                 res.feasible = true; res.optimal = true; res.canonical = false;
                 res.n_components = 1; res.nodes = pa.sweeps; res.price_sweeps = (int)pa.sweeps; res.price_rounds = (int)pa.rounds; res.price_total_us = (wall() - tf0) * 1e6;
                 res.objective = z_pt;
-                tmark("fast path certified");
+                tmark(defer ? "fast path certified, the row check deferred" : "fast path certified");
                 res_out = std::move(res);
                 return true;
             }
@@ -1396,9 +1418,9 @@
 
 static Result solve_classic(const Model &mdl_in, double time_limit_s, bool canonical, double rel_gap, hqprice::Sweeper *sweeper, const double ts0);
 
-Result solve(const Model &mdl_arg, double time_limit_s, bool canonical, double rel_gap, hqprice::Sweeper *sweeper) {
+Result solve(const Model &mdl_arg, double time_limit_s, bool canonical, double rel_gap, hqprice::Sweeper *sweeper, unsigned flags) {
     const double ts_entry = wall();
-    { Result r; if (solve_fast(mdl_arg, time_limit_s, rel_gap, sweeper, ts_entry, r)) return r; }
+    { Result r; if (solve_fast(mdl_arg, time_limit_s, rel_gap, sweeper, ts_entry, flags, r)) return r; }
     if (mdl_arg.has_lists()) {
         Model plain = mdl_arg;
         plain.expand_lists();
diff --git a/hyperqueue_amd/csrc/milp.h b/hyperqueue_amd/csrc/milp.h
--- a/hyperqueue_amd/csrc/milp.h
+++ b/hyperqueue_amd/csrc/milp.h
@@ -80,11 +80,27 @@
     int price_sweeps = 0, price_rounds = 0;
     double price_bound_us = 0, price_total_us = 0;
     long hull_solves = 0, hull_solves_nonpacking = 0;
+    bool check_pending = false;
+    double check_bound = 0.0, check_cost_scale = 1.0;
 };
 
 const double REFERENCE_MIP_REL_GAP = 1e-4;
 
-Result solve(const Model &m, double time_limit_s, bool canonical = true, double rel_gap = REFERENCE_MIP_REL_GAP, hqprice::Sweeper *sweeper = nullptr);
+enum { SOLVE_DEFER_CHECK = 1u, SOLVE_NO_FAST_PATH = 2u };
+Result solve(const Model &m, double time_limit_s, bool canonical = true, double rel_gap = REFERENCE_MIP_REL_GAP, hqprice::Sweeper *sweeper = nullptr, unsigned flags = 0);
+
+bool check_certified_point(const Model &m, const std::vector<double> &x, double bound, double cost_scale, double rel_gap, double *objective);
+struct PendingCheck {
+    Model model; std::vector<double> x;
+    double bound = 0.0, cost_scale = 1.0, rel_gap = 0.0;
+    bool pending = false;
+    bool run() { pending = false; const bool ok = check_certified_point(model, x, bound, cost_scale, rel_gap, nullptr); return ok && !take_forced_failure(); }
+    static bool take_forced_failure();
+};
+void set_defer_check(int on);
+int defer_check_setting();
+bool defer_check_on();
+void fail_next_deferred_checks(uint32_t n);
 
 void columns_by_cost_desc(const double *c, int n, std::vector<int> &out);
 void set_fast_path(int on);
diff --git a/hyperqueue_amd/csrc/price.hip b/hyperqueue_amd/csrc/price.hip
--- a/hyperqueue_amd/csrc/price.hip
+++ b/hyperqueue_amd/csrc/price.hip
@@ -20,23 +20,16 @@
 namespace {
 
 struct SweepResult {
-    double cx, rc, bnd;
-    uint32_t n_budget, max_steps;
-    long long act[KMAX];
-    double part_cx[ASLOTS];
     long long part_act[ASLOTS * KMAX];
+    alignas(64) uint32_t pseq[ASLOTS];
     uint32_t seq;
 };
-
-struct PartVal { uint32_t nbud, mx; };
 
 struct SweepArgs {
     Tables t;
     SweepOut out;
     uint32_t budget, seq;
     uint32_t *tickets;
-    long long *tact;
-    PartVal *pval;
     SweepResult *res;
     uint32_t first, local;
     double *lv_cx, *lv_rc, *lv_bnd; uint32_t *lv_steps;
@@ -80,25 +73,13 @@
 #pragma unroll
             for (int sub = 0; sub < ASUB; sub++) vs[u][sub] = k < K ? ld_dev(&a.out.act[((size_t)p * ASUB + sub) * K + k]) : 0;
         }
-        double *scr = &S.py[0][0];
-        static_assert(sizeof(S.py) >= 256 * sizeof(double), "a round of the part's c.x values is staged in the dual pool's storage");
-        uint32_t nbud = 0, mx = 0;
-        double s4 = 0.0;
-        for (uint32_t c0 = p * per; c0 < pe; c0 += 256) {
-            double v[4]; uint32_t vst[4];
-#pragma unroll
-            for (int u = 0; u < 4; u++) { const uint32_t q = c0 + lane + (uint32_t)u * WAVE; v[u] = (q < pe && !a.local) ? ld_dev(&a.out.blk_cx[q]) : 0.0; vst[u] = (q >= pb0 && q < pb1) ? ld_dev(&a.out.blk_steps[q]) : 0u; }
-#pragma unroll
-            for (int u = 0; u < 4; u++) { scr[lane + (uint32_t)u * WAVE] = v[u]; nbud += vst[u] >> 31; const uint32_t st = vst[u] & 0x7FFFFFFFu; mx = st > mx ? st : mx; }
-            wv.sync();
-            const uint32_t cnt = pe - c0 < 256u ? pe - c0 : 256u;
-            if (lane < 4 && !a.local) for (uint32_t i = lane; i < cnt; i += 4) s4 += scr[i];
-            wv.sync();
-        }
-#pragma unroll
-        for (int off = 32; off >= 1; off >>= 1) { nbud += __shfl_xor(nbud, off, 64); const uint32_t om = __shfl_xor(mx, off, 64); mx = om > mx ? om : mx; }
-        const double s1 = __shfl(s4, 1, 64), s2 = __shfl(s4, 2, 64), s3 = __shfl(s4, 3, 64);
-        const double pcx = ((s4 + s1) + s2) + s3;
+        if (!a.local) for (uint32_t c0 = pb0; c0 < pb1; c0 += 256) {
+            double vcx[4], vrc[4], vbd[4]; uint32_t vst[4];
+#pragma unroll
+            for (int u = 0; u < 4; u++) { const uint32_t q = c0 + lane + (uint32_t)u * WAVE; const bool in = q < pb1; vcx[u] = in ? ld_dev(&a.out.blk_cx[q]) : 0.0; vrc[u] = in ? ld_dev(&a.out.blk_rc[q]) : 0.0; vbd[u] = in ? ld_dev(&a.out.blk_bnd[q]) : 0.0; vst[u] = in ? ld_dev(&a.out.blk_steps[q]) : 0u; }
+#pragma unroll
+            for (int u = 0; u < 4; u++) { const uint32_t q = c0 + lane + (uint32_t)u * WAVE; if (q < pb1) { st_host(&a.lv_cx[q], vcx[u]); st_host(&a.lv_rc[q], vrc[u]); st_host(&a.lv_bnd[q], vbd[u]); st_host(&a.lv_steps[q], vst[u]); } }
+        }
 #pragma unroll
         for (int u = 0; u < 2; u++) {
             const uint32_t k = lane + (uint32_t)u * WAVE;
@@ -107,20 +88,16 @@
 #pragma unroll
             for (int sub = 0; sub < ASUB; sub++) { v += vs[u][sub]; st_dev(&a.out.act[((size_t)p * ASUB + sub) * K + k], 0); }
             st_host(&a.res->part_act[(size_t)p * K + k], v);
-            if (v != 0 && !a.local) atomicAdd(reinterpret_cast<unsigned long long *>(&a.tact[k]), (unsigned long long)v);
-        }
-        if (lane == 0) {
-            st_dev(&a.pval[p].nbud, nbud); st_dev(&a.pval[p].mx, mx);
-            if (!a.local) st_host(&a.res->part_cx[p], pcx);
-            st_dev(&a.tickets[1 + p], 0u);
-        }
+        }
+        if (lane == 0) st_dev(&a.tickets[1 + p], 0u);
+    }
+    uint32_t *done = &a.res->pseq[p];
+    if (a.local) {
         __threadfence_system();
-    }
-    const uint32_t p_first = r0 / per, p_last = (r1 - 1) / per;
-    if (lane == 0) last = __hip_atomic_fetch_add(&a.tickets[0], 1u, __ATOMIC_RELAXED, __HIP_MEMORY_SCOPE_AGENT) == p_last - p_first ? 1u : 0u;
-    last = (uint32_t)__builtin_amdgcn_readfirstlane((int)last);
-    if (!last) return;
-    if (a.local) {
+        const uint32_t p_first = r0 / per, p_last = (r1 - 1) / per;
+        if (lane == 0) last = __hip_atomic_fetch_add(&a.tickets[0], 1u, __ATOMIC_RELAXED, __HIP_MEMORY_SCOPE_AGENT) == p_last - p_first ? 1u : 0u;
+        last = (uint32_t)__builtin_amdgcn_readfirstlane((int)last);
+        if (!last) return;
         for (uint32_t b0 = r0 + lane; b0 < r1; b0 += WAVE * 8) {
             double vcx[8], vrc[8], vbd[8]; uint32_t vst[8];
 #pragma unroll
@@ -128,54 +105,23 @@
 #pragma unroll
             for (int u = 0; u < 8; u++) { const uint32_t q = b0 + (uint32_t)u * WAVE; if (q < r1) { st_host(&a.lv_cx[q], vcx[u]); st_host(&a.lv_rc[q], vrc[u]); st_host(&a.lv_bnd[q], vbd[u]); st_host(&a.lv_steps[q], vst[u]); } }
         }
-    } else {
-        const uint32_t n_parts = (nb + per - 1) / per;
-        long long ta[2] = {0, 0};
-#pragma unroll
-        for (int u = 0; u < 2; u++) { const uint32_t k = lane + (uint32_t)u * WAVE; if (k < K) ta[u] = ld_dev(&a.tact[k]); }
-        uint32_t pn = 0, pm = 0;
-        if (lane < n_parts) { pn = ld_dev(&a.pval[lane].nbud); pm = ld_dev(&a.pval[lane].mx); }
-        double cx = 0.0, rc = 0.0, bnd = 0.0;
-        for (uint32_t b0 = lane; b0 < nb; b0 += WAVE * 8) {
-            double vcx[8], vrc[8], vbd[8];
-#pragma unroll
-            for (int u = 0; u < 8; u++) { const uint32_t q = b0 + (uint32_t)u * WAVE; const bool in = q < nb; vcx[u] = in ? ld_dev(&a.out.blk_cx[q]) : 0.0; vrc[u] = in ? ld_dev(&a.out.blk_rc[q]) : 0.0; vbd[u] = in ? ld_dev(&a.out.blk_bnd[q]) : 0.0; }
-#pragma unroll
-            for (int u = 0; u < 8; u++) { if (b0 + (uint32_t)u * WAVE >= nb) break; cx += vcx[u]; rc += vrc[u]; bnd += vbd[u]; }
-        }
-        double *red = &S.py[0][0];
-        red[lane] = cx; red[WAVE + lane] = rc; red[2 * WAVE + lane] = bnd;
-#pragma unroll
-        for (int off = 8; off >= 1; off >>= 1) { pn += __shfl_xor(pn, off, 64); const uint32_t om = __shfl_xor(pm, off, 64); pm = om > pm ? om : pm; }
-        wv.sync();
-        double tcx = 0.0, trc = 0.0, tb = 0.0;
-        if (lane == 0) for (int l = 0; l < WAVE; l++) { tcx += red[l]; trc += red[WAVE + l]; tb += red[2 * WAVE + l]; }
-#pragma unroll
-        for (int u = 0; u < 2; u++) {
-            const uint32_t k = lane + (uint32_t)u * WAVE;
-            if (k >= K) continue;
-            st_dev(&a.tact[k], 0);
-            st_host(&a.res->act[k], ta[u]);
-            for (uint32_t i = n_parts; i < (uint32_t)ASLOTS; i++) st_host(&a.res->part_act[(size_t)i * K + k], 0);
-        }
-        if (lane >= n_parts && lane < (uint32_t)ASLOTS) st_host(&a.res->part_cx[lane], 0.0);
-        if (lane == 0) { st_host(&a.res->cx, tcx); st_host(&a.res->rc, trc); st_host(&a.res->bnd, tb); st_host(&a.res->n_budget, pn); st_host(&a.res->max_steps, pm); }
-    }
-    if (lane == 0) st_dev(&a.tickets[0], 0u);
+        if (lane == 0) st_dev(&a.tickets[0], 0u);
+        done = &a.res->seq;
+    }
     if (prof && lane == 0) prof[13] = wv.now();
     __threadfence_system();
     wv.sync();
     if (prof && lane == 0) prof[14] = wv.now();
-    if (lane == 0) __hip_atomic_store(&a.res->seq, a.seq, __ATOMIC_RELEASE, __HIP_MEMORY_SCOPE_SYSTEM);
-}
-
-constexpr size_t SYNC_ACT = 128, SYNC_PACT = SYNC_ACT + (size_t)ASLOTS * ASUB * KMAX * 8, SYNC_PVAL = SYNC_PACT + (size_t)KMAX * 8, SYNC_BYTES = SYNC_PVAL + (size_t)ASLOTS * sizeof(PartVal);
+    if (lane == 0) __hip_atomic_store(done, a.seq, __ATOMIC_RELEASE, __HIP_MEMORY_SCOPE_SYSTEM);
+}
+
+constexpr size_t SYNC_ACT = 128, SYNC_BYTES = SYNC_ACT + (size_t)ASLOTS * ASUB * KMAX * 8;
 
 constexpr int NPROF = 13;
 const int PROF_FROM[NPROF] = {0, 1, 3, 4, 5, 5, 8, 9, 10, 6, 11, 12, 13};
 const int PROF_TO[NPROF]   = {1, 2, 4, 5, 6, 8, 9, 10, 6, 11, 12, 13, 14};
 const char *const PROF_NAME[NPROF] = {"reduced costs + compaction", "dual pool + order + greedy fills", "level lists + root bound", "walk", "results + activities", "[results: zero the sums", "pattern + sums in LDS", "atomics + cost loads", "values]",
-                                      "acknowledgements before the ticket", "part ticket", "part sums + sweep ticket + totals (last block)", "system fence (last block)"};
+                                      "acknowledgements before the ticket", "part ticket", "part values + activities to the host (part's last block)", "system fence (part's last block)"};
 
 size_t al16(size_t v) { return (v + 15) & ~(size_t)15; }
 double now_us() { return std::chrono::duration<double, std::micro>(std::chrono::steady_clock::now().time_since_epoch()).count(); }
@@ -193,7 +139,11 @@
     o_off = 0; o_m = al16(o_off + (size_t)(t.n_blocks + 1) * 4); o_cap = al16(o_m + t.n_blocks); o_cost = al16(o_cap + (size_t)t.n_blocks * MMAX * 8);
     o_a = al16(o_cost + (size_t)t.n_cols * 8); o_ccap = al16(o_a + (size_t)t.n_cols * MMAX * 8); o_woff = al16(o_ccap + (size_t)t.n_cols * 4);
     o_wrow = al16(o_woff + (size_t)(t.n_cols + 1) * 4);
-    if (!h_res.ensure(sizeof(SweepResult) + 64)) return false;
+    if (!h_res.p) {
+        if (!h_res.ensure(sizeof(SweepResult) + 64)) return false;
+        memset(h_res.p, 0, sizeof(SweepResult));
+    }
+    if (!h_blkv.ensure((size_t)t.n_blocks * 28 + 64)) return false;
     if (!h_pin.ensure((size_t)std::min<uint32_t>(max_sweeps, PIN_SWEEPS) * t.n_cols * 2 + 64)) return false;
     in_flight = false;
     return d_pats.ensure((size_t)max_sweeps * t.n_cols * 2) && d_blk.ensure((size_t)t.n_blocks * 28 + 64) && d_sync.ensure(SYNC_BYTES);
@@ -218,8 +168,6 @@
     if (nw) { memcpy(h + o_wrow, t.w_row.data(), nw * 2); memcpy(h + o_wcoef, t.w_coef.data(), nw * 4); }
     if (hipMemcpyAsync(d_tab.p, h, tab_bytes, hipMemcpyHostToDevice, stream) != hipSuccess) return false;
     if (!sync_clean) { if (hipMemsetAsync(d_sync.p, 0, SYNC_BYTES, stream) != hipSuccess) return false; }
-    SweepResult *r = h_res.as<SweepResult>();
-    seq = r->seq;
     return true;
 }
 
@@ -234,7 +182,6 @@
     memset(h + o_woff, 0, o_wrow - o_woff);
     if (hipMemcpyAsync(d_tab.p, h, o_wrow, hipMemcpyHostToDevice, stream) != hipSuccess) return 0;
     if (!sync_clean) { if (hipMemsetAsync(d_sync.p, 0, SYNC_BYTES, stream) != hipSuccess) return 0; }
-    seq = h_res.as<SweepResult>()->seq;
     blocks_only = true;
     return 1;
 }
@@ -283,7 +230,6 @@
 bool DeviceSweeper::sweep_range(const double *pi, uint32_t b0, uint32_t b1, RangeValues &rv) {
     if (!T || b1 > T->n_blocks || b0 > b1) return false;
     const uint32_t nb = T->n_blocks;
-    if (!h_blkv.ensure((size_t)nb * 28 + 64)) return false;
     if (b1 > b0) { if (!launch(pi, b0, b1, true, nullptr)) return false; }
     else {
         if (n_sweeps >= cap_sweeps) return false;
@@ -313,10 +259,9 @@
     uint16_t *xdst = n_sweeps < PIN_SWEEPS ? h_pin.dev<uint16_t>() + (size_t)n_sweeps * t.n_cols : d_pats.as<uint16_t>() + (size_t)n_sweeps * t.n_cols;
     a.out = SweepOut{xdst, (double *)blk, (double *)(blk + (size_t)t.n_blocks * 8), (double *)(blk + (size_t)t.n_blocks * 16),
                      (long long *)(d_sync.as<unsigned char>() + SYNC_ACT), (uint32_t *)(blk + (size_t)t.n_blocks * 24), profile ? d_prof.as<uint64_t>() : nullptr, (uint32_t)ASUB, dbg};
-    a.budget = budget; a.seq = ++seq; a.tickets = d_sync.as<uint32_t>(); a.tact = (long long *)(d_sync.as<unsigned char>() + SYNC_PACT); a.pval = (PartVal *)(d_sync.as<unsigned char>() + SYNC_PVAL); a.res = h_res.dev<SweepResult>();
+    a.budget = budget; a.seq = ++seq; a.tickets = d_sync.as<uint32_t>(); a.res = h_res.dev<SweepResult>();
     a.first = b0; a.local = local ? 1u : 0u;
-    if (local) { unsigned char *lv = h_blkv.dev<unsigned char>(); a.lv_cx = (double *)lv; a.lv_rc = (double *)(lv + (size_t)t.n_blocks * 8); a.lv_bnd = (double *)(lv + (size_t)t.n_blocks * 16); a.lv_steps = (uint32_t *)(lv + (size_t)t.n_blocks * 24); }
-    else { a.lv_cx = a.lv_rc = a.lv_bnd = nullptr; a.lv_steps = nullptr; }
+    { unsigned char *lv = h_blkv.dev<unsigned char>(); a.lv_cx = (double *)lv; a.lv_rc = (double *)(lv + (size_t)t.n_blocks * 8); a.lv_bnd = (double *)(lv + (size_t)t.n_blocks * 16); a.lv_steps = (uint32_t *)(lv + (size_t)t.n_blocks * 24); }
     memset(a.pi, 0, sizeof(a.pi));
     if (K) memcpy(a.pi, pi, (size_t)K * 8);
     const double t0 = now_us();
@@ -330,7 +275,7 @@
 #undef HQ_SWEEP_N
 #undef HQ_SWEEP
     if (hipGetLastError() != hipSuccess) return false;
-    in_flight = true; sync_clean = false; flight_t0 = t0; flight_blocks = b1 - b0; flight_k = K;
+    in_flight = true; sync_clean = false; flight_t0 = t0; flight_blocks = b1 - b0; flight_k = K; flight_local = local;
     return true;
 }
 
@@ -339,12 +284,19 @@
     in_flight = false;
     const HostTables &t = *T;
     const double t0 = flight_t0;
-    volatile SweepResult *r = h_res.as<SweepResult>();
+    SweepResult *r = h_res.as<SweepResult>();
+    const uint32_t per = part_size(t.n_blocks), n_parts = (t.n_blocks + per - 1) / per;
+    uint32_t p_seen = 0;
+    auto done = [&]() {
+        if (flight_local) return __atomic_load_n(&r->seq, __ATOMIC_ACQUIRE) == seq;
+        while (p_seen < n_parts && __atomic_load_n(&r->pseq[p_seen], __ATOMIC_ACQUIRE) == seq) p_seen++;
+        return p_seen == n_parts;
+    };
     for (uint64_t spins = 0;; spins++) {
-        if (__atomic_load_n(&r->seq, __ATOMIC_ACQUIRE) == seq) break;
+        if (done()) break;
         if ((spins & 0xFFFF) == 0xFFFF && now_us() - t0 > 2.0e6) {
             if (hipStreamSynchronize(stream) != hipSuccess) return false;
-            if (__atomic_load_n(&r->seq, __ATOMIC_ACQUIRE) != seq) return false;
+            if (!done()) return false;
             break;
         }
     }
@@ -369,14 +321,11 @@
     total_sweeps++; total_block_solves += flight_blocks; total_us += last_kernel_us;
     n_sweeps++;
     if (!outp) return true;
-    SweepTotals &out = *outp;
-    out.cx = r->cx; out.rc = r->rc; out.bnd = r->bnd; out.n_budget = r->n_budget; out.max_steps = r->max_steps;
     const uint32_t K = flight_k;
-    out.act.resize(K);
-    for (uint32_t k = 0; k < K; k++) out.act[k] = r->act[k];
-    out.part_cx.assign(r->part_cx, r->part_cx + ASLOTS);
-    out.part_act.resize((size_t)ASLOTS * K);
-    for (size_t i = 0; i < (size_t)ASLOTS * K; i++) out.part_act[i] = r->part_act[i];
+    for (uint32_t i = n_parts; i < (uint32_t)ASLOTS && K; i++) memset(&r->part_act[(size_t)i * K], 0, (size_t)K * 8);
+    const unsigned char *h = h_blkv.as<unsigned char>();
+    const size_t nb = t.n_blocks;
+    totals_from_blocks(t.n_blocks, K, (const double *)h, (const double *)(h + nb * 8), (const double *)(h + nb * 16), (const uint32_t *)(h + nb * 24), r->part_act, *outp);
     return true;
 }
 
diff --git a/hyperqueue_amd/csrc/price_dev.h b/hyperqueue_amd/csrc/price_dev.h
--- a/hyperqueue_amd/csrc/price_dev.h
+++ b/hyperqueue_amd/csrc/price_dev.h
@@ -20,6 +20,7 @@
     size_t o_off = 0, o_m = 0, o_cap = 0, o_cost = 0, o_a = 0, o_ccap = 0, o_woff = 0, o_wrow = 0, o_wcoef = 0, tab_bytes = 0;
     bool blocks_only = false;
     uint32_t flight_k = 0;
+    bool flight_local = false;
     size_t wide_room = 0;
     uint32_t n_sweeps = 0, cap_sweeps = 0, seq = 0;
     uint32_t max_block_cols = 0;
diff --git a/include/hqtick_debug.h b/include/hqtick_debug.h
--- a/include/hqtick_debug.h
+++ b/include/hqtick_debug.h
@@ -52,6 +52,10 @@
 void hqtick_debug_last_coupled_digest(uint64_t out[4]);
 void hqtick_debug_set_early_sweep(int on);
 uint32_t hqtick_debug_early_sweeps(void);
+void hqtick_debug_set_deferred_check(int on);
+void hqtick_debug_fail_deferred_checks(uint32_t n);
+uint32_t hqtick_debug_deferred_check_retries(const hqtick_ctx *ctx);
+int hqtick_debug_run_sweeps(hqtick_ctx *ctx, uint32_t n_blocks, uint32_t seed, int early, int abandon, uint32_t n_sweeps, double *out, uint32_t cap);
 void hqtick_debug_capture_first_cut(int on);
 uint32_t hqtick_debug_first_cut(unsigned char *out, uint32_t cap);
 void hqtick_debug_corrupt_block_runs(int on);
```

Measured after the change: 69.24 million. 1.1% lower.
